# yell/boltzmann-machines

Measured on AMD Instinct MI355X. Metric: Gibbs-steps/sec (CD-k, 784x1024 RBM, batch 512), higher is better.
Workload: dtype f32

## Files before the change

boltzmann_machines_amd/csrc/bm_kernels.h:

```cpp
#pragma once
#include <stdio.h>
#include <stdlib.h>
#include <string.h>
#include <type_traits>
#include "bm_gemm.h"
#include "bm_bf3.h"
#include "bm_numerics.h"
#include "bm_rng.h"

namespace bm {

struct MfCtl { unsigned maxdiff; int done; int steps; float resid; };

struct ActArgs {
    Operand P1, Q1; int K1;
    int p_xm;
    Operand P2, Q2; int K2;
    int I, J;
    const float *bias;
    const float *sigma;
    float mult;
    float bmult;
    int kind;
    int sample;
    int lit;
    float *means;
    float *states;
    float *negmeans;
    int ldo;
    PhiloxKey key;
    long long row0;
    const float *prev;
    unsigned *maxdiff;
    float *maxdiff_blk;
    float *rowacc;
    float beta_a, beta_b;
    int rowacc_single;
    float *rowdot_out;
    int ld_part;
    const float *dot_vec;
    const float *dot_mat;
    int ld_dot;
    const float *acc_init;
    int ld_init;
    const int *skip;
    MfCtl *chk_ctl;
    const float *chk_slots; int chk_n; float chk_tol;
    Bf3Range b3;
    uint16_t *states16; int ld16;
    int geo_hint;
    int map_xi;
    float *fe_rowacc2;
    PhiloxKey fe_key;
    double *fe_zero;
    int fe_rm;
    const int *fe_flip;
    const float *fe_x; int fe_ldx;
    const float *fe_w; int fe_ldw;
    const float *clamp_val, *clamp_mask;
    int ld_clamp;
    const float *row_mult;
    float *rowen_out;
    float *sel_out;
    int sel_ld, sel_R, sel_rows;
    float *cr_part;
    const float *cr_U;
    int cr_ldu, cr_C, cr_nslots;
    const int *cb_y;
    const float *cb_U;
    int cb_ldu, cb_C;
    int *cb_bad;
    int bp;
    const float *bp_act;
    int bp_ld;
    int nrelu;
    int sm_k;
#ifdef BM_PROBE
    long long *dbg;
#endif
};
#ifdef BM_PROBE
#define BM_STAMP(n) do { if (a.dbg && threadIdx.x == 0) a.dbg[blockIdx.x * 4 + (n)] = (long long)__builtin_readcyclecounter(); } while (0)
#else
#define BM_STAMP(n) do {} while (0)
#endif

__device__ __forceinline__ int pll_flip_col(const PhiloxKey &key, unsigned long long idx, int V) {
    uint32_t w[4];
    philox_block(key, idx >> 2, w);
    return (int)(w[idx & 3] % (uint32_t)V);
}
#define FE_FLIP_FROM_KEY (reinterpret_cast<const int *>(uintptr_t(1)))
constexpr int BM_MF_SLOTS = 1024;

__device__ __forceinline__ void draw4(const ActArgs &a, const PhiloxKey &key, unsigned long long flat, int ib, int nvalid,
                                      const float *m, float *s, bool aligned) {
    if (aligned) {
        uint32_t wds[4];
        philox_block(key, flat >> 2, wds);
        if (a.kind == 0) {
#pragma unroll
            for (int r = 0; r < 4; ++r) s[r] = (u32_to_uniform(wds[r]) < m[r]) ? 1.f : 0.f;
        } else {
            float n[4];
            box_muller(wds[0], wds[1], n[0], n[1]);
            box_muller(wds[2], wds[3], n[2], n[3]);
#pragma unroll
            for (int r = 0; r < 4; ++r) s[r] = n[r] * a.sigma[ib + r] + m[r];
        }
    } else {
#pragma unroll
        for (int r = 0; r < 4; ++r) {
            if (r >= nvalid) break;
            const unsigned long long idx = flat + r;
            uint32_t wds[4];
            philox_block(key, idx >> 2, wds);
            if (a.kind == 0) {
                s[r] = (u32_to_uniform(wds[idx & 3]) < m[r]) ? 1.f : 0.f;
            } else {
                float n0, n1;
                const int pr = (int)(idx & 3) >> 1;
                box_muller(wds[2 * pr], wds[2 * pr + 1], n0, n1);
                s[r] = ((idx & 1) ? n1 : n0) * a.sigma[ib + r] + m[r];
            }
        }
    }
}

__device__ __forceinline__ float nrelu_state(float t, float n) {
    const float sd = sqrtf(sigmoid(t));
    const float u = __fadd_rn(t, __fmul_rn(n, sd));
    return (u > 0.0f) ? u : 0.0f;
}
__device__ __forceinline__ void nrelu_normals(const PhiloxKey &key, unsigned long long flat, int nvalid, float *n) {
#pragma unroll
    for (int r = 0; r < 4; ++r) {
        n[r] = 0.f;
        if (r >= nvalid) continue;
        const unsigned long long idx = flat + r;
        uint32_t wds[4];
        philox_block(key, idx >> 2, wds);
        float n0, n1;
        const int pr = (int)(idx & 3) >> 1;
        box_muller(wds[2 * pr], wds[2 * pr + 1], n0, n1);
        n[r] = (idx & 1) ? n1 : n0;
    }
}

#ifndef BM_NT_STORES
#define BM_NT_STORES 1
#endif
typedef float f32x2 __attribute__((ext_vector_type(2)));
__device__ __forceinline__ void stream_store4(float *p, float x, float y, float z, float w) {
    if (BM_NT_STORES) __builtin_nontemporal_store((f32x4){x, y, z, w}, reinterpret_cast<f32x4 *>(p));
    else *reinterpret_cast<float4 *>(p) = make_float4(x, y, z, w);
}
__device__ __forceinline__ void stream_store2(float *p, float x, float y) {
    if (BM_NT_STORES) __builtin_nontemporal_store((f32x2){x, y}, reinterpret_cast<f32x2 *>(p));
    else *reinterpret_cast<float2 *>(p) = make_float2(x, y);
}

template <bool CACHED = false>
__device__ __forceinline__ void store4(float *dst, size_t o, const float *v, int nvalid, bool v4) {
    if (v4) {
        if (CACHED) *reinterpret_cast<float4 *>(dst + o) = make_float4(v[0], v[1], v[2], v[3]);
        else stream_store4(dst + o, v[0], v[1], v[2], v[3]);
    } else {
#pragma unroll
        for (int r = 0; r < 4; ++r) if (r < nvalid) dst[o + r] = v[r];
    }
}

template <int MI> struct PhiloxFor { typedef PhiloxPair type; };
template <> struct PhiloxFor<1> { typedef PhiloxOne type; };

__device__ __forceinline__ float wave_max_lane63(float v) {
#define BM_DPP_MAX(ctrl, rmask) v = fmaxf(v, __int_as_float(__builtin_amdgcn_update_dpp(__float_as_int(v), __float_as_int(v), ctrl, rmask, 0xf, false)))
    BM_DPP_MAX(0xb1, 0xf);
    BM_DPP_MAX(0x4e, 0xf);
    BM_DPP_MAX(0x124, 0xf);
    BM_DPP_MAX(0x128, 0xf);
    BM_DPP_MAX(0x142, 0xa);
    BM_DPP_MAX(0x143, 0xc);
#undef BM_DPP_MAX
    return v;
}

template <int E, class Rng, bool MF = false, int NTH = 256> struct ActSide {
    static constexpr bool kFinalSync = false;
    static constexpr bool kSplitFill = false, kCohQ = false, kCanAbort = MF;
    static constexpr bool kMF = MF;
    const float *bias, *sigma;
    const float *prev_row;
    int ib0, I, with_rng;
    float bs[E], sg[E], pv[E];
    Rng rng;
    MfCtl *chk_ctl; const float *chk_slots; int chk_n; float chk_tol; const int *skip; float *s_chk; int aborted, nthreads;

    __device__ __forceinline__ void load_inputs() {
        const float *sp = sigma ? sigma : bias;
        const bool has_sigma = sigma != nullptr;
        if (MF && prev_row) {
            if (E == 4 && ib0 + 3 < I && (((uintptr_t)prev_row & 15u) == 0)) {
                const float4 t = *reinterpret_cast<const float4 *>(prev_row);
                pv[0] = t.x; pv[1] = t.y; pv[2] = t.z; pv[E - 1] = t.w;
            } else {
#pragma unroll
                for (int e = 0; e < E; ++e) pv[e] = (ib0 + e < I) ? prev_row[e] : 0.f;
            }
        }
        if (MF && E == 4 && ib0 + 3 < I && (((uintptr_t)(bias + ib0) & 15u) == 0) && (((uintptr_t)(sp + ib0) & 15u) == 0)) {
            const float4 b = *reinterpret_cast<const float4 *>(bias + ib0), v = *reinterpret_cast<const float4 *>(sp + ib0);
            bs[0] = b.x; bs[1] = b.y; bs[2] = b.z; bs[E - 1] = b.w;
            sg[0] = has_sigma ? v.x : 1.0f; sg[1] = has_sigma ? v.y : 1.0f; sg[2] = has_sigma ? v.z : 1.0f; sg[E - 1] = has_sigma ? v.w : 1.0f;
            return;
        }
#pragma unroll
        for (int e = 0; e < E; ++e) {
            const int i = (ib0 + e < I) ? ib0 + e : I - 1;
            bs[e] = bias[i];
            const float sv = sp[i];
            sg[e] = has_sigma ? sv : 1.0f;
        }
    }
    static constexpr int CHK_MAX = 4096;
    float *s_slots;
    static __device__ __forceinline__ void dma4_lane0(const void *src, float *lds_dst) {
        if ((threadIdx.x & 63) == 0) {
            unsigned keep;
            const unsigned lds_addr = (unsigned)(uintptr_t)(__attribute__((address_space(3))) void *)lds_dst;
            asm volatile("s_mov_b32 %0, m0\n\ts_mov_b32 m0, %2\n\ts_nop 0\n\tglobal_load_lds_dword %1, off\n\ts_mov_b32 m0, %0"
                         : "=&s"(keep) : "v"(src), "s"(__builtin_amdgcn_readfirstlane(lds_addr)) : "memory");
        }
    }
    __device__ __forceinline__ void preload() {
        if constexpr (MF) {
            load_inputs();
            aborted = 0;
            const int w = threadIdx.x >> 6, lane = threadIdx.x & 63;
            if (chk_ctl) {
                for (int p = w; p * 256 < chk_n && p * 256 < CHK_MAX; p += nthreads / 64)
                    dma16(reinterpret_cast<const char *>(chk_slots + 256 * p) + 16 * lane, s_slots + 256 * p);
                if (w == 0) dma4_lane0(&chk_ctl->done, s_slots + CHK_MAX);
            } else if (skip) {
                if (w == 0) dma4_lane0(skip, s_slots + CHK_MAX);
            }
        }
    }
    __device__ __forceinline__ void fill() {
        if (!MF) load_inputs();
        if (with_rng) rng.fill();
    }
    __device__ __forceinline__ void post_fill() {
        if constexpr (MF) {
            if (chk_ctl) {
                constexpr int NR = CHK_MAX / (4 * NTH);
                f32x4 v[NR];
#pragma unroll
                for (int q = 0; q < NR; ++q) {
                    const int e = 4 * ((int)threadIdx.x + q * NTH);
                    v[q] = *reinterpret_cast<const f32x4 *>(s_slots + (e < chk_n ? e : 0));
                }
                float m = 0.f;
#pragma unroll
                for (int q = 0; q < NR; ++q) {
                    const bool in = 4 * ((int)threadIdx.x + q * NTH) < chk_n;
                    m = fmaxf(m, in ? fmaxf(fmaxf(v[q][0], v[q][1]), fmaxf(v[q][2], v[q][3])) : 0.f);
                }
                m = wave_max_lane63(m);
                if ((threadIdx.x & 63) == 63) s_chk[threadIdx.x >> 6] = m;
                wg_barrier();
                m = 0.f;
#pragma unroll
                for (int q = 0; q < NTH / 64; ++q) m = fmaxf(m, s_chk[q]);
                const int was = __float_as_int(s_slots[CHK_MAX]);
                const int done = was || !(m > chk_tol);
                if (blockIdx.x == 0 && threadIdx.x == 0 && !was) { chk_ctl->steps += 1; chk_ctl->done = done; }
                aborted = __builtin_amdgcn_readfirstlane(done);
            } else if (skip) {
                aborted = __builtin_amdgcn_readfirstlane(__float_as_int(s_slots[CHK_MAX]) != 0);
            }
        }
    }
    __device__ __forceinline__ void drain() {}
};

template <class G, int ABL, class SideT, bool HWMATH = false, bool FE = false, bool LIT = false, bool CL = false, bool RT = false,
          bool CR = false, bool CB = false, bool BP = false, bool NR = false, bool SM = false>
__device__ __forceinline__ float act_epilogue(const ActArgs &a, const PhiloxKey &key, const f32x4 (&acc)[G::MI][1], const SideT &side,
                                              int i0, int j0) {
    constexpr int E = G::E, NH = G::MI;
    const int tid = threadIdx.x, lane = tid & 63, w = tid >> 6;
    const int wi = w % G::WI, wj = w / G::WI;
    const int g = lane >> 4, l15 = lane & 15;
    const int ib0 = i0 + wi * (16 * G::MI) + g * E;
    const int j = j0 + wj * 16 + l15;
    const bool rng_fast = ((a.I & 3) == 0);
    const float (&bs)[E] = side.bs;
    const float (&sg)[E] = side.sg;
    const typename PhiloxFor<G::MI>::type &rng = side.rng;

    float cv[NH][4], cm[NH][4];
    (void)cv; (void)cm;
    if constexpr (CL) {
        const bool al_cl = ((a.ld_clamp & 3) == 0) && (((uintptr_t)a.clamp_val & 15u) == 0) && (((uintptr_t)a.clamp_mask & 15u) == 0);
#pragma unroll
        for (int hlf = 0; hlf < NH; ++hlf) {
            const int ib = ib0 + 4 * hlf;
#pragma unroll
            for (int r = 0; r < 4; ++r) { cv[hlf][r] = 0.f; cm[hlf][r] = 0.f; }
            if (j < a.J && ib < a.I) {
                const size_t oc = (size_t)j * a.ld_clamp + ib;
                if (al_cl && ib + 3 < a.I) {
                    const float4 tv = *reinterpret_cast<const float4 *>(a.clamp_val + oc), tm = *reinterpret_cast<const float4 *>(a.clamp_mask + oc);
                    cv[hlf][0] = tv.x; cv[hlf][1] = tv.y; cv[hlf][2] = tv.z; cv[hlf][3] = tv.w;
                    cm[hlf][0] = tm.x; cm[hlf][1] = tm.y; cm[hlf][2] = tm.z; cm[hlf][3] = tm.w;
                } else {
#pragma unroll
                    for (int r = 0; r < 4; ++r)
                        if (ib + r < a.I) { cv[hlf][r] = a.clamp_val[oc + r]; cm[hlf][r] = a.clamp_mask[oc + r]; }
                }
            }
        }
    }
    float rm = 1.f, sv[E];
    (void)rm; (void)sv;
    if constexpr (RT) {
        rm = (j < a.J) ? a.row_mult[j] : 0.f;
#pragma unroll
        for (int e = 0; e < E; ++e) sv[e] = 0.f;
    }
    float cu[NH][4];
    bool cb_ok = false;
    (void)cu; (void)cb_ok;
    if constexpr (CB) {
        const int yj = (j < a.J) ? a.cb_y[j] : -1;
        cb_ok = (unsigned)yj < (unsigned)a.cb_C;
        if (j < a.J && !cb_ok && ib0 == 0) *a.cb_bad = 1;
        const bool al_cb = ((a.cb_ldu & 3) == 0) && (((uintptr_t)a.cb_U & 15u) == 0);
#pragma unroll
        for (int hlf = 0; hlf < NH; ++hlf) {
            const int ib = ib0 + 4 * hlf;
#pragma unroll
            for (int r = 0; r < 4; ++r) cu[hlf][r] = 0.f;
            if (cb_ok && ib < a.I) {
                const float *u = a.cb_U + (size_t)yj * a.cb_ldu + ib;
                if (al_cb && ib + 3 < a.I && (ib & 3) == 0) {
                    const float4 tu = *reinterpret_cast<const float4 *>(u);
                    cu[hlf][0] = tu.x; cu[hlf][1] = tu.y; cu[hlf][2] = tu.z; cu[hlf][3] = tu.w;
                } else {
#pragma unroll
                    for (int r = 0; r < 4; ++r)
                        if (ib + r < a.I) cu[hlf][r] = u[r];
                }
            }
        }
    }
    float ba[NH][4];
    (void)ba;
    if constexpr (BP) {
        const bool al_bp = ((a.bp_ld & 3) == 0) && (((uintptr_t)a.bp_act & 15u) == 0);
#pragma unroll
        for (int hlf = 0; hlf < NH; ++hlf) {
            const int ib = ib0 + 4 * hlf;
#pragma unroll
            for (int r = 0; r < 4; ++r) ba[hlf][r] = 0.f;
            if (a.bp_act && j < a.J && ib < a.I) {
                const float *p = a.bp_act + (size_t)j * a.bp_ld + ib;
                if (al_bp && ib + 3 < a.I) {
                    const float4 t = *reinterpret_cast<const float4 *>(p);
                    ba[hlf][0] = t.x; ba[hlf][1] = t.y; ba[hlf][2] = t.z; ba[hlf][3] = t.w;
                } else {
#pragma unroll
                    for (int r = 0; r < 4; ++r)
                        if (ib + r < a.I) ba[hlf][r] = p[r];
                }
            }
        }
    }
    float z[E];
    lane_outputs<G>(acc, 0, z);
    float dmax = 0.f;
    if (BM_ABL(4)) {
        float zs = 0.f;
#pragma unroll
        for (int e = 0; e < E; ++e) zs += z[e];
        if (j < a.J && ib0 < a.I && a.states) a.states[(size_t)j * a.ldo + ib0] = zs;
    } else if (j < a.J && ib0 < a.I) {
        const bool al_out = ((a.ldo & 3) == 0);
#pragma unroll
        for (int hlf = 0; hlf < NH; ++hlf) {
            const int ib = ib0 + 4 * hlf;
            if (ib >= a.I) break;
            const int nvalid = (a.I - ib < 4) ? a.I - ib : 4;
            float m[4], s[4], nt[4];
            (void)nt;
#pragma unroll
            for (int r = 0; r < 4; ++r) {
                if constexpr (BP) {
                    const float zv = z[4 * hlf + r], av = ba[hlf][r];
                    m[r] = a.bp_act ? __fmul_rn(__fmul_rn(zv, av), __fsub_rn(1.0f, av)) : zv;
                    s[r] = m[r];
                    continue;
                }
                const float x = (RT ? rm : a.mult) * z[4 * hlf + r];
                float bv = bs[4 * hlf + r];
                if constexpr (CB) { if (cb_ok) bv = __fadd_rn(bv, cu[hlf][r]); }
                const float b = (RT ? rm : a.bmult) * bv;
                if constexpr (NR) {
                    nt[r] = x + b;
                    m[r] = (nt[r] > 0.0f) ? nt[r] : 0.0f;
                    s[r] = m[r];
                    continue;
                }
                if constexpr (SM) {
                    nt[r] = x + b;
                    continue;
                }
                m[r] = (a.kind == 0) ? (LIT ? sigmoid_literal(x + b) : (HWMATH ? sigmoid_hw(x + b) : sigmoid(x + b)))
                                     : (a.kind == 1 ? (x * sg[4 * hlf + r] + b) : (a.kind == 3 ? x + b : x));
                s[r] = m[r];
            }
            if constexpr (SM) {
                static_assert(G::MI == 1, "the SM flavour exists for the geometries with one quad per lane");
                const int Ks = a.sm_k, nl = (Ks >= 8) ? (Ks >> 2) : 1, pos = g & (nl - 1);
                float mxa = fmaxf(nt[0], nt[1]), mxb = fmaxf(nt[2], nt[3]);
                if (Ks > 2) {
                    mxa = fmaxf(mxa, mxb);
                    if (Ks >= 8) mxa = fmaxf(mxa, __shfl_xor(mxa, 16));
                    if (Ks == 16) mxa = fmaxf(mxa, __shfl_xor(mxa, 32));
                    mxb = mxa;
                }
                float ev[4], cc[4], cpv[4];
#pragma unroll
                for (int r = 0; r < 4; ++r) {
                    float d = ((r < 2) ? mxa : mxb) - nt[r];
                    if (d > 80.0f) d = 80.0f;
                    ev[r] = exp_neg(d);
                }
                float start = 0.0f;
                for (int step = 0; step < nl; ++step) {
                    if (step > 0) {
                        const float recv = __shfl(cc[3], (lane + 48) & 63);
                        if (pos == step) start = recv;
                    }
                    cpv[0] = start;          cc[0] = start + ev[0];
                    cpv[1] = cc[0];          cc[1] = cc[0] + ev[1];
                    cpv[2] = (Ks == 2) ? 0.0f : cc[1];
                    cc[2] = cpv[2] + ev[2];
                    cpv[3] = cc[2];          cc[3] = cc[2] + ev[3];
                }
                float Sa = cc[3], Sb = cc[3];
                if (Ks == 2) Sa = cc[1];
                if (Ks >= 8) { Sa = __shfl(cc[3], l15 + 16 * (g | (nl - 1))); Sb = Sa; }
#pragma unroll
                for (int r = 0; r < 4; ++r) { m[r] = ev[r] / ((r < 2) ? Sa : Sb); s[r] = m[r]; }
                if (a.sample) {
                    const uint32_t *wds = rng.words(hlf);
                    float ua = u32_to_uniform(wds[0]), ub = (Ks == 2) ? u32_to_uniform(wds[2]) : ua;
                    if (Ks >= 8) { ua = __shfl(ua, l15 + 16 * (g & ~(nl - 1))); ub = ua; }
                    const float ta = ua * Sa, tb = ub * Sb;
#pragma unroll
                    for (int r = 0; r < 4; ++r) {
                        const float t = (r < 2) ? ta : tb;
                        s[r] = (cc[r] > t && !(cpv[r] > t)) ? 1.f : 0.f;
                    }
                }
            }
            if (!BP && !SM && a.sample) {
                if constexpr (NR) {
                    float n[4];
                    if (rng_fast) {
                        const uint32_t *wds = rng.words(hlf);
                        box_muller(wds[0], wds[1], n[0], n[1]);
                        box_muller(wds[2], wds[3], n[2], n[3]);
                    } else {
                        nrelu_normals(key, (unsigned long long)(a.row0 + j) * (unsigned long long)a.I + ib, nvalid, n);
                    }
#pragma unroll
                    for (int r = 0; r < 4; ++r) s[r] = nrelu_state(nt[r], n[r]);
                } else if (rng_fast) {
                    const uint32_t *wds = rng.words(hlf);
                    if (a.kind == 0) {
#pragma unroll
                        for (int r = 0; r < 4; ++r) s[r] = (u32_to_uniform(wds[r]) < m[r]) ? 1.f : 0.f;
                    } else {
                        float n[4];
                        box_muller(wds[0], wds[1], n[0], n[1]);
                        box_muller(wds[2], wds[3], n[2], n[3]);
#pragma unroll
                        for (int r = 0; r < 4; ++r) s[r] = n[r] * sg[4 * hlf + r] + m[r];
                    }
                } else {
                    const unsigned long long flat = (unsigned long long)(a.row0 + j) * (unsigned long long)a.I + ib;
                    draw4(a, key, flat, ib, nvalid, m, s, false);
                }
            }
            if constexpr (CL) {
#pragma unroll
                for (int r = 0; r < 4; ++r)
                    if (cm[hlf][r] != 0.f) { m[r] = cv[hlf][r]; s[r] = cv[hlf][r]; }
            }
            if constexpr (RT) {
#pragma unroll
                for (int r = 0; r < 4; ++r) sv[4 * hlf + r] = s[r];
            }
            const size_t o = (size_t)j * a.ldo + ib;
            if constexpr (SideT::kMF) {
                if (a.prev) {
#pragma unroll
                    for (int r = 0; r < 4; ++r)
                        if (r < nvalid) dmax = fmaxf(dmax, fabsf(m[r] - side.pv[4 * hlf + r]));
                }
            }
            const bool v4 = al_out && nvalid == 4;
            if (a.means) store4<HWMATH>(a.means, o, m, nvalid, v4 && (((uintptr_t)a.means & 15u) == 0));
            if (a.negmeans) {
                float nm[4];
#pragma unroll
                for (int r = 0; r < 4; ++r) nm[r] = -m[r];
                store4<HWMATH>(a.negmeans, o, nm, nvalid, v4 && (((uintptr_t)a.negmeans & 15u) == 0));
            }
            if (a.states) store4<HWMATH>(a.states, o, s, nvalid, v4 && (((uintptr_t)a.states & 15u) == 0));
            if constexpr (RT) {
                if (a.sel_out && rm == 1.0f) {
                    const int c = j / a.sel_R;
                    if (c < a.sel_rows)
                        store4<HWMATH>(a.sel_out, (size_t)c * a.sel_ld + ib, s, nvalid,
                                       nvalid == 4 && ((a.sel_ld & 3) == 0) && (((uintptr_t)a.sel_out & 15u) == 0));
                }
            }
            if (HWMATH && a.states16) {
                uint16_t *d = a.states16 + (size_t)j * a.ld16 + ib;
                if (nvalid == 4 && (ib & 3) == 0) {
                    uint2 pk;
                    pk.x = (__float_as_uint(s[0]) >> 16) | (__float_as_uint(s[1]) & 0xffff0000u);
                    pk.y = (__float_as_uint(s[2]) >> 16) | (__float_as_uint(s[3]) & 0xffff0000u);
                    *reinterpret_cast<uint2 *>(d) = pk;
                } else {
#pragma unroll
                    for (int r = 0; r < 4; ++r) if (r < nvalid) d[r] = (uint16_t)(__float_as_uint(s[r]) >> 16);
                }
            }
        }
    }
    if constexpr (FE) { if (a.fe_zero && i0 == 0 && j0 == 0 && tid < 6) a.fe_zero[tid] = 0.0; }
    bool row_sums = a.rowacc || a.rowdot_out;
    if constexpr (RT) row_sums = row_sums || a.rowen_out;
    if constexpr (BP) row_sums = false;
    if (row_sums) {
        float racc = 0.f, rdot = 0.f, racc2 = 0.f, ren = 0.f;
        (void)ren;
        if (j < a.J) {
            int fc = 0; float delta = 0.f;
            if constexpr (FE) {
                fc = (a.fe_flip == FE_FLIP_FROM_KEY) ? pll_flip_col(a.fe_key, (unsigned long long)(a.row0 + j), a.K1) : a.fe_flip[j];
                delta = 1.0f - 2.0f * a.fe_x[(size_t)j * a.fe_ldx + fc];
            }
#pragma unroll
            for (int hlf = 0; hlf < NH; ++hlf) {
                float qa = 0.f, qd = 0.f, qa2 = 0.f, qe = 0.f;
                (void)qe;
#pragma unroll
                for (int r = 0; r < 4; ++r) {
                    const int e = 4 * hlf + r, i = ib0 + e;
                    if (i >= a.I) break;
                    if (a.rowacc) {
                        if (a.dot_mat) {
                            qa += z[e] * a.dot_mat[(size_t)j * a.ld_dot + i];
                        } else {
                            const float t = z[e] + bs[e];
                            if constexpr (FE) qa2 += softplus(t + delta * a.fe_w[(size_t)fc * a.fe_ldw + i]);
                            if (a.rowacc_single) qa += HWMATH ? softplus_hw(a.beta_b * t) : softplus(a.beta_b * t);
                            else qa += softplus_hw(a.beta_b * t) - softplus_hw(a.beta_a * t);
                        }
                    }
                    if (a.rowdot_out) qd += a.states[(size_t)j * a.ldo + i] * a.dot_vec[i];
                    if constexpr (RT) { if (a.rowen_out) qe += sv[e] * (z[e] + bs[e]); }
                }
                if constexpr (RT) ren = (hlf == 0) ? qe : ren + qe;
                racc = (hlf == 0) ? qa : racc + qa;
                rdot = (hlf == 0) ? qd : rdot + qd;
                racc2 = (hlf == 0) ? qa2 : racc2 + qa2;
            }
        }
        racc += __shfl_xor(racc, 16);
        rdot += __shfl_xor(rdot, 16);
        if (G::MI == 1) { racc += __shfl_xor(racc, 32); rdot += __shfl_xor(rdot, 32); }
        if constexpr (FE) { racc2 += __shfl_xor(racc2, 16); if (G::MI == 1) racc2 += __shfl_xor(racc2, 32); }
        if constexpr (RT) { ren += __shfl_xor(ren, 16); if (G::MI == 1) ren += __shfl_xor(ren, 32); }
        const bool writer = (G::MI == 1) ? (g == 0) : ((g & 1) == 0);
        const int slot = (i0 + wi * (16 * G::MI)) / 16 + ((G::MI == 2) ? (g >> 1) : 0);
        if (writer && j < a.J && slot * 16 < a.I) {
            if constexpr (FE) {
                a.rowacc[(size_t)j * a.fe_rm + slot] = racc;
                a.fe_rowacc2[(size_t)j * a.fe_rm + slot] = racc2;
            } else {
                if (a.rowacc) a.rowacc[(size_t)slot * a.ld_part + j] = racc;
                if (a.rowdot_out) a.rowdot_out[(size_t)slot * a.ld_part + j] = rdot;
                if constexpr (RT) { if (a.rowen_out) a.rowen_out[(size_t)slot * a.ld_part + j] = ren; }
            }
        }
    }
    if constexpr (CR) {
        const bool writer = (G::MI == 1) ? (g == 0) : ((g & 1) == 0);
        const int slot = (i0 + wi * (16 * G::MI)) / 16 + ((G::MI == 2) ? (g >> 1) : 0);
        for (int c = 0; c < a.cr_C; ++c) {
            const float *u = a.cr_U + (size_t)c * a.cr_ldu;
            float racc = 0.f;
            if (j < a.J) {
#pragma unroll
                for (int hlf = 0; hlf < NH; ++hlf) {
                    float qa = 0.f;
#pragma unroll
                    for (int r = 0; r < 4; ++r) {
                        const int e = 4 * hlf + r, i = ib0 + e;
                        if (i >= a.I) break;
                        qa += softplus((z[e] + bs[e]) + u[i]);
                    }
                    racc = (hlf == 0) ? qa : racc + qa;
                }
            }
            racc += __shfl_xor(racc, 16);
            if (G::MI == 1) racc += __shfl_xor(racc, 32);
            if (writer && j < a.J && slot * 16 < a.I) a.cr_part[((size_t)c * a.cr_nslots + slot) * a.ld_part + j] = racc;
        }
    }
    return dmax;
}

template <class G, int MINB, bool SEG2, bool FAST, int ABL = 0, int PL = KM, int STG = STG_DMA, bool FE = false, bool LIT = false, bool MF = false,
          bool CL = false, bool RT = false, bool CR = false, bool CB = false, bool BP = false, bool NR = false, bool SM = false>
BM_KERNEL __launch_bounds__(G::NT, MINB) void act_kernel(ActArgs a, TileMap tmap) {
    __shared__ __attribute__((aligned(16))) float smem[G::SMEM_FLOATS];
    constexpr int E = G::E;
    BM_STAMP(0);
    asm volatile("" :: "s"(a.P1.ptr), "s"(a.Q1.ptr), "s"(a.P1.ld), "s"(a.Q1.ld), "s"(a.P1.nx), "s"(a.Q1.nx),
                       "s"(a.K1), "s"(a.K2), "s"(a.bias), "s"(a.sigma), "s"(a.means), "s"(a.states), "s"(a.ldo),
                       "s"(a.sample), "s"(a.kind), "s"(a.row0), "s"(a.I), "s"(a.J), "s"(a.skip));
    const int tiles_j = (a.J + G::TJ - 1) / G::TJ;
    int ti, tj;
    if (tmap.slab) {
        block_to_tile(tiles_j, ti, tj, 0, 0, a.J > 2 * a.I, (a.I + G::TI - 1) / G::TI);
    } else {
        TILE_WORDS(tmap, (int)blockIdx.x);
        TILE_OF_BLOCK(tmap, (int)blockIdx.x, (int)gridDim.x, ti, tj);
    }
    const int i0 = ti * G::TI, j0 = tj * G::TJ;
    const int tid = threadIdx.x, lane = tid & 63, w = tid >> 6;
    const int wi = w % G::WI, wj = w / G::WI;
    const int g = lane >> 4, l15 = lane & 15;
    const int ib0 = i0 + wi * (16 * G::MI) + g * E;

    KRange kr;
    kr.P1 = a.P1; kr.Q1 = a.Q1; kr.K1 = a.K1;
    kr.P2 = a.P2; kr.Q2 = a.Q2; kr.K2 = a.K2;
    static_assert(G::NJ == 1, "act_kernel: one j sub-tile per wave");
    const int j = j0 + wj * 16 + l15;
    ActSide<E, typename PhiloxFor<G::MI>::type, MF, G::NT> side;
    side.bias = a.bias; side.sigma = a.sigma; side.ib0 = ib0; side.I = a.I; side.with_rng = a.sample;
    side.prev_row = (MF && a.prev && j < a.J && ib0 < a.I) ? a.prev + (size_t)j * a.ldo + ib0 : nullptr;
    const PhiloxKey key = a.key;
    side.rng.init(key, ((unsigned long long)(a.row0 + j) * (unsigned long long)a.I + ib0) >> 2);

    f32x4 acc[G::MI][1];
#pragma unroll
    for (int t = 0; t < G::MI; ++t) acc[t][0] = (f32x4){0.f, 0.f, 0.f, 0.f};
    if constexpr (MF) {
        __shared__ float s_chk[G::NT / 64];
        __shared__ __attribute__((aligned(16))) float s_slots[ActSide<E, typename PhiloxFor<G::MI>::type, true>::CHK_MAX + 4];
        side.s_slots = s_slots;
        side.chk_ctl = a.chk_ctl; side.chk_slots = a.chk_slots; side.chk_n = a.chk_n; side.chk_tol = a.chk_tol;
        side.skip = a.skip; side.s_chk = s_chk; side.nthreads = G::NT; side.aborted = 0;
        if (a.acc_init && j < a.J) {
            const float *src = a.acc_init + (size_t)j * a.ld_init + ib0;
            if (G::MI == 1 && ib0 + 3 < a.I && (((uintptr_t)src & 15u) == 0)) {
                const float4 t4 = *reinterpret_cast<const float4 *>(src);
                acc[0][0] = (f32x4){t4.x, t4.y, t4.z, t4.w};
            } else {
#pragma unroll
                for (int r = 0; r < 4; ++r)
#pragma unroll
                    for (int t = 0; t < G::MI; ++t) {
                        const int i = ib0 + G::MI * r + t;
                        if (i < a.I) acc[t][0][r] = src[G::MI * r + t];
                    }
            }
        }
        side.preload();
    }
#ifdef BM_PROBE
    mainloop<XM, G, FAST, SEG2, ABL, PL, STG>(acc, kr, i0, j0, smem, side, a.dbg ? a.dbg + 2048 + blockIdx.x * 8 : nullptr);
#else
    mainloop<XM, G, FAST, SEG2, ABL, PL, STG>(acc, kr, i0, j0, smem, side);
#endif
    BM_STAMP(1);
    if constexpr (MF) { if (side.aborted) return; }
    float dmax = act_epilogue<G, ABL, decltype(side), false, FE, LIT, CL, RT, CR, CB, BP, NR, SM>(a, key, acc, side, i0, j0);
    if (MF && a.maxdiff) {
        __shared__ float s_wavemax[G::NT / 64];
        dmax = wave_max_lane63(dmax);
        if (lane == 63) s_wavemax[w] = dmax;
        wg_barrier();
        if (tid == 0) {
            float m = 0.f;
#pragma unroll
            for (int q = 0; q < G::NT / 64; ++q) m = fmaxf(m, s_wavemax[q]);
            if (a.maxdiff_blk && gridDim.x <= BM_MF_SLOTS) a.maxdiff_blk[blockIdx.x] = m;
            else if (m > 0.f) atomicMax(a.maxdiff, __float_as_uint(m));
        }
    }
    BM_STAMP(2);
}

struct Bf3Strip { int tiles_i, tiles_j, strips, abl; };

template <class G, bool SEG2, int MINW>
BM_KERNEL __launch_bounds__(G::NT, MINW) void act_bf3_kernel(ActArgs a, Bf3Strip sp) {
    __shared__ __attribute__((aligned(16))) float smem[Bf3Geo<G>::SMEM_FLOATS];
    constexpr int E = G::E;
    const int ti = (int)blockIdx.x / sp.strips, st = (int)blockIdx.x % sp.strips;
    const int per = sp.tiles_j / sp.strips, rem = sp.tiles_j % sp.strips;
    const int tj0 = st * per + (st < rem ? st : rem), tj1 = tj0 + per + (st < rem ? 1 : 0);
    const int i0 = ti * G::TI;
    const int tid = threadIdx.x, lane = tid & 63, w = tid >> 6;
    const int wi = w % G::WI, wj = w / G::WI;
    const int g = lane >> 4, l15 = lane & 15;
    const int ib0 = i0 + wi * (16 * G::MI) + g * E;
    ActSide<E, typename PhiloxFor<G::MI>::type> side;
    side.bias = a.bias; side.sigma = a.sigma; side.ib0 = ib0; side.I = a.I; side.with_rng = 0;
    side.prev_row = nullptr;
    side.fill();
    side.with_rng = a.sample;
    Bf3Pipe<G, SEG2> pipe;
    pipe.setup(a.b3, i0, smem);
    if (tj0 < tj1) { pipe.set_tile(a.b3, tj0 * G::TJ); pipe.prefetch(); }
    for (int tj = tj0; tj < tj1; ++tj) {
        const int j0 = tj * G::TJ, j = j0 + wj * 16 + l15;
        f32x4 acc[G::MI][1];
#pragma unroll
        for (int t = 0; t < G::MI; ++t) acc[t][0] = (f32x4){0.f, 0.f, 0.f, 0.f};
        side.rng.init(a.key, ((unsigned long long)(a.row0 + j) * (unsigned long long)a.I + ib0) >> 2);
        if (a.sample) side.rng.fill();
        if (!(sp.abl & 2)) pipe.run(acc);
        if (tj + 1 < tj1) { pipe.set_tile(a.b3, (tj + 1) * G::TJ); pipe.prefetch(); }
        if (!(sp.abl & 1)) (void)act_epilogue<G, 0, decltype(side), true>(a, a.key, acc, side, i0, j0);
    }
}

struct ColSumJob {
    const float *A, *Bm;
    int lda, ldb, ncols, nrows;
    float *out;
};
constexpr int MAX_COLJOBS = 12;
struct ColSumArgs {
    ColSumJob job[MAX_COLJOBS];
    int first_wave[MAX_COLJOBS + 1];
    int njobs;
};

constexpr int CS_ROWS = 128;
constexpr int CS_LD = 80;
constexpr int CS_SMEM_FLOATS = 2 * CS_ROWS * CS_LD;

constexpr int CS_NV = CS_ROWS * 16 / NT;
struct ColRegs { float4 a[CS_NV], b[CS_NV]; };

__device__ __forceinline__ void cs_fetch(ColRegs &r, const float *A, int lda, const float *Bm, int ldb,
                                         int c0, int ncols, int nrows, int r0, int tid) {
    const int c4 = tid & 15;
    const int cc = min(c0 + 4 * c4, ncols - 4);
#pragma unroll
    for (int n = 0; n < CS_NV; ++n) {
        const int rc = min(r0 + (tid >> 4) + 16 * n, nrows - 1);
        r.a[n] = *reinterpret_cast<const float4 *>(A + (size_t)rc * lda + cc);
        r.b[n] = Bm ? *reinterpret_cast<const float4 *>(Bm + (size_t)rc * ldb + cc) : make_float4(0.f, 0.f, 0.f, 0.f);
    }
}

__device__ __forceinline__ void cs_stash(const ColRegs &r, float *sA, float *sB, int c0, int ncols, int nrows,
                                         int r0, int tid) {
    const int c4 = tid & 15;
#pragma unroll
    for (int n = 0; n < CS_NV; ++n) {
        const int row = (tid >> 4) + 16 * n;
        const bool ok = (r0 + row < nrows) && (c0 + 4 * c4 < ncols);
        float4 va = r.a[n], vb = r.b[n];
        if (!ok) { va = make_float4(0.f, 0.f, 0.f, 0.f); vb = va; }
        *reinterpret_cast<float4 *>(sA + row * CS_LD + 4 * c4) = va;
        *reinterpret_cast<float4 *>(sB + row * CS_LD + 4 * c4) = vb;
    }
}

__device__ __forceinline__ void block_colsum(const float *A, int lda, const float *Bm, int ldb,
                                             int c0, int ncols, int nrows, bool want2,
                                             float *smem, f32x4 &sum1, f32x4 &sum2, bool negB = false) {
    const int tid = threadIdx.x, lane = tid & 63, w = tid >> 6;
    const int g = lane >> 4, l15 = lane & 15;
    float *sA = smem, *sB = smem + CS_ROWS * CS_LD;
    sum1 = (f32x4){0.f, 0.f, 0.f, 0.f};
    sum2 = (f32x4){0.f, 0.f, 0.f, 0.f};
    const bool vec = (((uintptr_t)A & 15u) == 0) && ((lda & 3) == 0) && ((ncols & 3) == 0) &&
                     (!Bm || ((((uintptr_t)Bm & 15u) == 0) && ((ldb & 3) == 0)));
    ColRegs regs;
    if (vec) cs_fetch(regs, A, lda, Bm, ldb, c0, ncols, nrows, 0, tid);
    for (int r0 = 0; r0 < nrows; r0 += CS_ROWS) {
        const int nr = (nrows - r0 < CS_ROWS) ? nrows - r0 : CS_ROWS;
        if (vec) {
            cs_stash(regs, sA, sB, c0, ncols, nrows, r0, tid);
        } else {
            for (int e = tid; e < CS_ROWS * 64; e += NT) {
                const int row = e >> 6, cc = e & 63, c = c0 + cc;
                const bool ok = row < nr && c < ncols;
                sA[row * CS_LD + cc] = ok ? A[(size_t)(r0 + row) * lda + c] : 0.f;
                sB[row * CS_LD + cc] = (ok && Bm) ? Bm[(size_t)(r0 + row) * ldb + c] : 0.f;
            }
        }
        wg_barrier();
        if (vec) cs_fetch(regs, A, lda, Bm, ldb, c0, ncols, nrows, r0 + CS_ROWS, tid);
        const int nsteps = (((nr + 3) / 4) + 7) & ~7;
        const int co = w * 16 + l15;
        for (int s = 0; s < nsteps; s += 8) {
            float d[8], e[8];
#pragma unroll
            for (int u = 0; u < 8; ++u) {
                const int o = (4 * (s + u) + g) * CS_LD + co;
                e[u] = sB[o];
                d[u] = negB ? sA[o] + e[u] : sA[o] - e[u];
            }
#pragma unroll
            for (int u = 0; u < 8; ++u) {
                sum1 = __builtin_amdgcn_mfma_f32_16x16x4f32(d[u], 1.0f, sum1, 0, 0, 0);
                if (want2) sum2 = __builtin_amdgcn_mfma_f32_16x16x4f32(e[u], 1.0f, sum2, 0, 0, 0);
            }
        }
        wg_barrier();
    }
    if (negB) sum2 = -sum2;
}

BM_KERNEL __launch_bounds__(NT) void colsum_kernel(ColSumArgs a) {
    __shared__ __attribute__((aligned(16))) float smem[CS_SMEM_FLOATS];
    const int wv = blockIdx.x, lane = threadIdx.x & 63, w = threadIdx.x >> 6;
    int jb = 0;
    while (jb + 1 < a.njobs && wv >= a.first_wave[jb + 1]) ++jb;
    const ColSumJob J = a.job[jb];
    const int c0 = (wv - a.first_wave[jb]) * 64;
    f32x4 s1, s2;
    block_colsum(J.A, J.lda, J.Bm, J.ldb, c0, J.ncols, J.nrows, false, smem, s1, s2);
    if ((lane & 15) == 0) {
        const int g = lane >> 4;
#pragma unroll
        for (int r = 0; r < 4; ++r) {
            const int cc = c0 + w * 16 + g * 4 + r;
            if (cc < J.ncols) J.out[cc] = s1[r];
        }
    }
}

struct RbmBiasArgs {
    const float *sv, *sh, *sq;
    float *vb, *dvb, *hb, *dhb, *q, *pen;
    int V, H;
    float N, lr, mom, damping, cost, target;
};
BM_KERNEL void rbm_bias_kernel(RbmBiasArgs a) {
    const int c = blockIdx.x * blockDim.x + threadIdx.x;
    if (c < a.V) {
        const float g = a.sv[c] / a.N;
        const float d = a.lr * (a.mom * a.dvb[c] + g);
        a.dvb[c] = d;
        a.vb[c] = a.vb[c] + d;
    } else if (c < a.V + a.H) {
        const int h = c - a.V;
        const float qn = a.damping * a.q[h] + (1.0f - a.damping) * a.sq[h];
        a.q[h] = qn;
        const float pen = a.cost * (qn - a.target);
        a.pen[h] = pen;
        float g = a.sh[h] / a.N;
        g = g - pen;
        const float d = a.lr * (a.mom * a.dhb[h] + g);
        a.dhb[h] = d;
        a.hb[h] = a.hb[h] + d;
    }
}

struct RbmBiasFusedArgs {
    const float *X, *vs, *h0m, *hm;
    int ldx, ldv, ldh0, ldh, B;
    int hm_negated;
    float *raw_tail;
    int raw_only;
    RbmBiasArgs u;
};
__device__ __forceinline__ void rbm_bias_fused_block(const RbmBiasFusedArgs &a, int wv, float *smem) {
    const int lane = threadIdx.x & 63, w = threadIdx.x >> 6, g = lane >> 4;
    const int nv = (a.u.V + 63) / 64;
    f32x4 s1, s2;
    if (wv < nv) {
        const int c0 = wv * 64;
        block_colsum(a.X, a.ldx, a.vs, a.ldv, c0, a.u.V, a.B, false, smem, s1, s2);
        if ((lane & 15) == 0) {
#pragma unroll
            for (int r = 0; r < 4; ++r) {
                const int c = c0 + w * 16 + g * 4 + r;
                if (c < a.u.V) {
                    a.raw_tail[c] = s1[r];
                    if (a.raw_only) continue;
                    const float gr = s1[r] / a.u.N;
                    const float d = a.u.lr * (a.u.mom * a.u.dvb[c] + gr);
                    a.u.dvb[c] = d;
                    a.u.vb[c] = a.u.vb[c] + d;
                }
            }
        }
    } else {
        const int c0 = (wv - nv) * 64;
        block_colsum(a.h0m, a.ldh0, a.hm, a.ldh, c0, a.u.H, a.B, true, smem, s1, s2, a.hm_negated != 0);
        if ((lane & 15) == 0) {
#pragma unroll
            for (int r = 0; r < 4; ++r) {
                const int h = c0 + w * 16 + g * 4 + r;
                if (h < a.u.H) {
                    const float sq = s2[r];
                    a.raw_tail[a.u.V + h] = s1[r];
                    a.raw_tail[a.u.V + a.u.H + h] = sq;
                    if (a.raw_only) continue;
                    const float qn = a.u.damping * a.u.q[h] + (1.0f - a.u.damping) * sq;
                    a.u.q[h] = qn;
                    const float pen = a.u.cost * (qn - a.u.target);
                    a.u.pen[h] = pen;
                    float gr = s1[r] / a.u.N;
                    gr = gr - pen;
                    const float d = a.u.lr * (a.u.mom * a.u.dhb[h] + gr);
                    a.u.dhb[h] = d;
                    a.u.hb[h] = a.u.hb[h] + d;
                }
            }
        }
    }
}

BM_KERNEL __launch_bounds__(NT) void rbm_bias_fused_kernel(RbmBiasFusedArgs a) {
    __shared__ __attribute__((aligned(16))) float smem[CS_SMEM_FLOATS];
    rbm_bias_fused_block(a, blockIdx.x, smem);
}

struct GradArgs {
    Operand Ppos, Qpos; int Kpos;
    Operand Pneg, Qneg; int Kneg;
    int I, J;
    int form;
    int fused;
    float *raw;
    float *raw2;
    float *W, *dW;
    float *Wt;
    int ldw, ldwt;
    const float *pen;
    float N, M, l2, lr, mom;
    int nbias;
    RbmBiasFusedArgs bias;
    int fetch_at_fill;
    int map_xi;
#ifdef BM_PROBE
    long long *dbg;
#endif
};

__device__ __forceinline__ void apply_w_update(float g, float pen, float l2, float lr, float mom,
                                               float &w, float &dw) {
    g = __fsub_rn(g, __fmul_rn(l2, w));
    g = __fsub_rn(g, pen);
    const float d = __fmul_rn(lr, __fadd_rn(__fmul_rn(mom, dw), g));
    dw = d;
    w = __fadd_rn(w, d);
}
__device__ __forceinline__ bool grad_pow2(float N) { return ((__float_as_uint(N) & 0x007fffffu) == 0u) && N >= 1.0f; }
__device__ __forceinline__ float grad_norm1(float r, float N, float invN, bool pow2) {
    return pow2 ? __fmul_rn(r, invN) : __fdiv_rn(r, N);
}
__device__ __forceinline__ float grad_norm2(float r, float r2, float N, float M, float invN, float invM, bool pow2) {
    return pow2 ? __fsub_rn(__fmul_rn(r, invN), __fmul_rn(r2, invM)) : __fsub_rn(__fdiv_rn(r, N), __fdiv_rn(r2, M));
}

struct DivBy {
    float n, inv; bool pow2;
    __device__ __forceinline__ explicit DivBy(float N) : n(N), inv(1.0f / N),
        pow2(grad_pow2(N)) {}
};

template <int NJ> struct GradSide {
    static constexpr bool kFinalSync = true;
    static constexpr bool kSplitFill = false, kCohQ = false, kCanAbort = false;
    const float *W, *dW; int ldw, I, J, ib0, jb[NJ]; bool on, vec8;
    float4 w[NJ][2], d[NJ][2];
    bool at_fill;
    __device__ __forceinline__ void fill() { if (at_fill) fetch(); }
    __device__ __forceinline__ void drain() { if (!at_fill) fetch(); }
    __device__ __forceinline__ void fetch() {
        if (!on || ib0 >= I) return;
#pragma unroll
        for (int n = 0; n < NJ; ++n) {
            if (jb[n] >= J) continue;
            const size_t o = (size_t)jb[n] * ldw + ib0;
            if (vec8) {
                w[n][0] = *reinterpret_cast<const float4 *>(W + o);  w[n][1] = *reinterpret_cast<const float4 *>(W + o + 4);
                d[n][0] = *reinterpret_cast<const float4 *>(dW + o); d[n][1] = *reinterpret_cast<const float4 *>(dW + o + 4);
            } else {
                float tw[8], td[8];
#pragma unroll
                for (int e = 0; e < 8; ++e) {
                    const bool ok = ib0 + e < I;
                    tw[e] = ok ? W[o + e] : 0.f;
                    td[e] = ok ? dW[o + e] : 0.f;
                }
                w[n][0] = make_float4(tw[0], tw[1], tw[2], tw[3]); w[n][1] = make_float4(tw[4], tw[5], tw[6], tw[7]);
                d[n][0] = make_float4(td[0], td[1], td[2], td[3]); d[n][1] = make_float4(td[4], td[5], td[6], td[7]);
            }
        }
    }
};

struct GradCen { const float *oj, *gj, *oi, *gi; };
__device__ __forceinline__ const GradCen &grad_cen_of(const GradCen &c) { return c; }
struct GradFast { float *Wf, *We, *Wet; int ldf, ldet; float fast_lr, fast_decay; };
__device__ __forceinline__ const GradFast &grad_fast_of(const GradFast &f) { return f; }
template <class T, class... P> struct grad_has { static constexpr int value = 0; };
template <class T, class P0, class... P> struct grad_has<T, P0, P...> { static constexpr int value = (std::is_same<T, P0>::value ? 1 : 0) + grad_has<T, P...>::value; };
template <class G, bool FAST, int ABL = 0, int STG = STG_DMA, int MINB = 1, class... CENP>
BM_KERNEL __launch_bounds__(G::NT, MINB) void grad_kernel(GradArgs a, TileMap tmap, CENP... cenp) {
    constexpr int CEN = grad_has<GradCen, CENP...>::value, FW = grad_has<GradFast, CENP...>::value;
    static_assert(sizeof...(CENP) <= 1 && CEN + FW == (int)sizeof...(CENP), "grad_kernel: at most one GradCen or one GradFast");
    constexpr int TI = G::TI, NJ = G::NJ;
    static_assert(G::MI == 2 && G::TI == 64 && G::TJ == 64, "grad_kernel: 64 x 64 tiles, 8 consecutive outputs per lane");
    __shared__ __attribute__((aligned(16))) float smem[G::SMEM_FLOATS];
    constexpr bool kBias = G::SMEM_FLOATS >= CS_SMEM_FLOATS;
    static_assert(G::NT >= NT, "bias path");
    const int ntile_blocks = (int)gridDim.x - a.nbias;
    if ((int)blockIdx.x >= ntile_blocks) {
        if constexpr (kBias) {
            if (G::NT > NT && threadIdx.x >= NT) return;
            rbm_bias_fused_block(a.bias, (int)blockIdx.x - ntile_blocks, smem);
        }
        return;
    }
    asm volatile("" :: "s"(a.Ppos.ptr), "s"(a.Qpos.ptr), "s"(a.Ppos.ld), "s"(a.Qpos.ld), "s"(a.Ppos.nx), "s"(a.Qpos.nx),
                       "s"(a.Pneg.ptr), "s"(a.Qneg.ptr), "s"(a.Pneg.ld), "s"(a.Qneg.ld), "s"(a.Kpos), "s"(a.Kneg),
                       "s"(a.I), "s"(a.J), "s"(a.W), "s"(a.dW), "s"(a.ldw), "s"(a.form), "s"(a.fused));
    constexpr int TJ2 = G::TJ;
    int ti, tj;
    if (tmap.slab) {
        block_to_tile((a.J + TJ2 - 1) / TJ2, ti, tj, 0, a.nbias);
    } else {
        TILE_WORDS(tmap, (int)blockIdx.x);
        TILE_OF_BLOCK(tmap, (int)blockIdx.x, ntile_blocks, ti, tj);
    }
    const int i0 = ti * TI, j0 = tj * TJ2;
    const int tid = threadIdx.x, lane = tid & 63, w = tid >> 6;
    const int wi = w % G::WI, wj = w / G::WI;
    const int g = lane >> 4, l15 = lane & 15;
    const int ib0 = i0 + wi * 32 + g * 8;

#ifdef BM_PROBE
#define BM_GSTAMP(n) do { if (a.dbg && threadIdx.x == 0) a.dbg[blockIdx.x * 4 + (n)] = (long long)__builtin_readcyclecounter(); } while (0)
#else
#define BM_GSTAMP(n) do {} while (0)
#endif
    BM_GSTAMP(0);
    f32x4 pos[2][NJ], neg[2][NJ];
#pragma unroll
    for (int t = 0; t < 2; ++t)
#pragma unroll
        for (int n = 0; n < NJ; ++n) pos[t][n] = neg[t][n] = (f32x4){0.f, 0.f, 0.f, 0.f};
    GradSide<NJ> side;
    side.W = a.W; side.dW = a.dW; side.ldw = a.ldw; side.I = a.I; side.J = a.J; side.ib0 = ib0;
#pragma unroll
    for (int n = 0; n < NJ; ++n) side.jb[n] = j0 + wj * (16 * NJ) + lane_j<KM, G>(l15, n);
    side.vec8 = (ib0 + 7 < a.I) && ((a.ldw & 3) == 0);
    side.at_fill = true;
    side.on = a.fused != 0 && a.fetch_at_fill != 0;
    KRange kr;
    kr.P1 = a.Ppos; kr.Q1 = a.Qpos; kr.K1 = a.Kpos;
    if (a.form == 0) {
        kr.P2 = a.Pneg; kr.Q2 = a.Qneg; kr.K2 = a.Kneg;
        mainloop<KM, G, FAST, true, ABL, KM, STG>(pos, kr, i0, j0, smem, side);
    } else {
        kr.P2 = a.Ppos; kr.Q2 = a.Qpos; kr.K2 = 0;
        mainloop<KM, G, FAST, false, 0, KM, STG>(pos, kr, i0, j0, smem, side);
        kr.P1 = a.Pneg; kr.Q1 = a.Qneg; kr.K1 = a.Kneg;
        mainloop<KM, G, FAST, false, 0, KM, STG>(neg, kr, i0, j0, smem, side);
    }

    BM_GSTAMP(1);
    if (ib0 >= a.I) return;
    if (!a.fetch_at_fill) { side.on = a.fused != 0; side.fetch(); }
    const DivBy divN(a.N), divM(a.M);
    float wt[NJ][8];
    float et[FW ? NJ : 1][FW ? 8 : 1];
    bool jok[NJ];
    float coi[CEN ? 8 : 1], cgi[CEN ? 8 : 1];
    if constexpr (CEN != 0) {
#pragma unroll
        for (int e = 0; e < 8; ++e) {
            const bool ok = ib0 + e < a.I;
            coi[e] = ok ? grad_cen_of(cenp...).oi[ib0 + e] : 0.f;
            cgi[e] = ok ? grad_cen_of(cenp...).gi[ib0 + e] : 0.f;
        }
    }
#pragma unroll
    for (int n = 0; n < NJ; ++n) {
        const int j = side.jb[n];
        jok[n] = j < a.J;
        if (!jok[n]) continue;
        float pv[8], nv[8];
        lane_outputs<G>(pos, n, pv);
        lane_outputs<G>(neg, n, nv);
        const size_t o = (size_t)j * a.ldw + ib0;
        if (!a.fused) {
#pragma unroll
            for (int e = 0; e < 8; ++e) {
                if (ib0 + e >= a.I) break;
                a.raw[o + e] = pv[e];
                if (a.form != 0) a.raw2[o + e] = nv[e];
            }
            continue;
        }
        float wv[8] = {side.w[n][0].x, side.w[n][0].y, side.w[n][0].z, side.w[n][0].w, side.w[n][1].x, side.w[n][1].y, side.w[n][1].z, side.w[n][1].w};
        float dv[8] = {side.d[n][0].x, side.d[n][0].y, side.d[n][0].z, side.d[n][0].w, side.d[n][1].x, side.d[n][1].y, side.d[n][1].z, side.d[n][1].w};
        float pe[8];
#pragma unroll
        for (int e = 0; e < 8; ++e) pe[e] = (a.pen && ib0 + e < a.I) ? a.pen[ib0 + e] : 0.f;
        float gr[8];
        if (divN.pow2 && divM.pow2) {
#pragma unroll
            for (int e = 0; e < 8; ++e) gr[e] = (a.form == 0) ? grad_norm1(pv[e], a.N, divN.inv, true)
                                                              : grad_norm2(pv[e], nv[e], a.N, a.M, divN.inv, divM.inv, true);
        } else {
#pragma unroll
            for (int e = 0; e < 8; ++e) gr[e] = (a.form == 0) ? grad_norm1(pv[e], a.N, 0.f, false)
                                                              : grad_norm2(pv[e], nv[e], a.N, a.M, 0.f, 0.f, false);
        }
        if constexpr (CEN != 0) {
            const float oj = grad_cen_of(cenp...).oj[j], gj = grad_cen_of(cenp...).gj[j];
#pragma unroll
            for (int e = 0; e < 8; ++e) gr[e] = __fsub_rn(gr[e], __fadd_rn(__fmul_rn(oj, cgi[e]), __fmul_rn(gj, coi[e])));
        }
        float fv[FW ? 8 : 1];
        if constexpr (FW != 0) {
            const GradFast &f = grad_fast_of(cenp...);
            const size_t of = (size_t)j * f.ldf + ib0;
            if (side.vec8 && (f.ldf & 3) == 0) {
                const float4 f0 = *reinterpret_cast<const float4 *>(f.Wf + of), f1 = *reinterpret_cast<const float4 *>(f.Wf + of + 4);
                fv[0] = f0.x; fv[1] = f0.y; fv[2] = f0.z; fv[3] = f0.w; fv[4] = f1.x; fv[5] = f1.y; fv[6] = f1.z; fv[7] = f1.w;
            } else {
#pragma unroll
                for (int e = 0; e < 8; ++e) fv[e] = (ib0 + e < a.I) ? f.Wf[of + e] : 0.f;
            }
#pragma unroll
            for (int e = 0; e < 8; ++e) fv[e] = __fadd_rn(__fmul_rn(f.fast_decay, fv[e]), __fmul_rn(f.fast_lr, gr[e]));
        }
#pragma unroll
        for (int e = 0; e < 8; ++e) {
            apply_w_update(gr[e], pe[e], a.l2, a.lr, a.mom, wv[e], dv[e]);
            wt[n][e] = wv[e];
        }
        if (side.vec8) {
            stream_store4(a.W + o, wv[0], wv[1], wv[2], wv[3]);
            stream_store4(a.W + o + 4, wv[4], wv[5], wv[6], wv[7]);
            stream_store4(a.dW + o, dv[0], dv[1], dv[2], dv[3]);
            stream_store4(a.dW + o + 4, dv[4], dv[5], dv[6], dv[7]);
        } else {
#pragma unroll
            for (int e = 0; e < 8; ++e)
                if (ib0 + e < a.I) { a.W[o + e] = wv[e]; a.dW[o + e] = dv[e]; }
        }
        if constexpr (FW != 0) {
            const GradFast &f = grad_fast_of(cenp...);
            const size_t of = (size_t)j * f.ldf + ib0;
#pragma unroll
            for (int e = 0; e < 8; ++e) et[n][e] = __fadd_rn(wv[e], fv[e]);
            if (side.vec8 && (f.ldf & 3) == 0) {
                stream_store4(f.Wf + of, fv[0], fv[1], fv[2], fv[3]);
                stream_store4(f.Wf + of + 4, fv[4], fv[5], fv[6], fv[7]);
                stream_store4(f.We + of, et[n][0], et[n][1], et[n][2], et[n][3]);
                stream_store4(f.We + of + 4, et[n][4], et[n][5], et[n][6], et[n][7]);
            } else {
#pragma unroll
                for (int e = 0; e < 8; ++e)
                    if (ib0 + e < a.I) { f.Wf[of + e] = fv[e]; f.We[of + e] = et[n][e]; }
            }
        }
    }
    if constexpr (FW != 0) {
        const GradFast &f = grad_fast_of(cenp...);
        if (a.fused && f.Wet) {
            const int ja = side.jb[0];
            const bool pair = NJ == 2 && jok[0] && jok[NJ - 1] && ((f.ldet & 1) == 0);
#pragma unroll
            for (int e = 0; e < 8; ++e) {
                if (ib0 + e >= a.I) break;
                float *dst = f.Wet + (size_t)(ib0 + e) * f.ldet + ja;
                if (pair) {
                    stream_store2(dst, et[0][e], et[NJ - 1][e]);
                } else {
                    if (jok[0]) dst[0] = et[0][e];
                    if (NJ == 2 && jok[NJ - 1]) dst[1] = et[NJ - 1][e];
                }
            }
        }
    }
    if (a.fused && a.Wt) {
        const int ja = side.jb[0];
        const bool pair = NJ == 2 && jok[0] && jok[NJ - 1] && ((a.ldwt & 1) == 0);
#pragma unroll
        for (int e = 0; e < 8; ++e) {
            if (ib0 + e >= a.I) break;
            float *dst = a.Wt + (size_t)(ib0 + e) * a.ldwt + ja;
            if (pair) {
                stream_store2(dst, wt[0][e], wt[NJ - 1][e]);
            } else {
                if (jok[0]) dst[0] = wt[0][e];
                if (NJ == 2 && jok[NJ - 1]) dst[1] = wt[NJ - 1][e];
            }
        }
    }
    BM_GSTAMP(2);
}

struct ApplyWArgs {
    const float *raw, *raw2;
    float *W, *dW, *Wt;
    const float *pen;
    int I, J, ldw, ldwt;
    int form;
    float N, M, l2, lr, mom;
};
BM_KERNEL void apply_w_kernel(ApplyWArgs a) {
    const size_t n = (size_t)a.I * a.J;
    for (size_t e = (size_t)blockIdx.x * blockDim.x + threadIdx.x; e < n; e += (size_t)gridDim.x * blockDim.x) {
        const int i = (int)(e % (size_t)a.I), j = (int)(e / (size_t)a.I);
        const size_t o = (size_t)j * a.ldw + i;
        const float gr = (a.form == 0) ? grad_norm1(a.raw[o], a.N, 0.f, false) : grad_norm2(a.raw[o], a.raw2[o], a.N, a.M, 0.f, 0.f, false);
        float wv = a.W[o], dv = a.dW[o];
        apply_w_update(gr, a.pen ? a.pen[i] : 0.f, a.l2, a.lr, a.mom, wv, dv);
        a.W[o] = wv;
        a.dW[o] = dv;
        if (a.Wt) a.Wt[(size_t)i * a.ldwt + j] = wv;
    }
}

__device__ __forceinline__ void rbm_bias_apply(const RbmBiasArgs &a, bool hidden, int c, float g) {
    if (!hidden) {
        const float d = a.lr * (a.mom * a.dvb[c] + g);
        a.dvb[c] = d;
        a.vb[c] = a.vb[c] + d;
    } else {
        const float qn = a.damping * a.q[c] + (1.0f - a.damping) * a.sq[c];
        a.q[c] = qn;
        const float pen = a.cost * (qn - a.target);
        a.pen[c] = pen;
        g = g - pen;
        const float d = a.lr * (a.mom * a.dhb[c] + g);
        a.dhb[c] = d;
        a.hb[c] = a.hb[c] + d;
    }
}
__device__ __forceinline__ void rbm_bias_update(const RbmBiasArgs &a, int c) {
    if (c < a.V) rbm_bias_apply(a, false, c, a.sv[c] / a.N);
    else if (c < a.V + a.H) rbm_bias_apply(a, true, c - a.V, a.sh[c - a.V] / a.N);
}
BM_KERNEL __launch_bounds__(256) void apply_w_tiled_kernel(ApplyWArgs a, RbmBiasArgs b, int nbias) {
    __shared__ float tile[64][65];
    const int ntile = (int)gridDim.x - nbias;
    if ((int)blockIdx.x >= ntile) {
        rbm_bias_update(b, ((int)blockIdx.x - ntile) * 256 + (int)threadIdx.x);
        return;
    }
    const int tiles_i = (a.I + 63) / 64;
    const int i0 = ((int)blockIdx.x % tiles_i) * 64, j0 = ((int)blockIdx.x / tiles_i) * 64;
    const int tid = threadIdx.x, c4 = tid & 15, r0 = tid >> 4;
    const bool pow2 = grad_pow2(a.N) && grad_pow2(a.M);
    const float invN = 1.0f / a.N, invM = 1.0f / a.M;
    const int i = i0 + 4 * c4;
    float4 pe = make_float4(0.f, 0.f, 0.f, 0.f);
    if (a.pen && i < a.I) pe = *reinterpret_cast<const float4 *>(a.pen + i);
#pragma unroll
    for (int p = 0; p < 4; ++p) {
        const int jl = r0 + 16 * p, j = j0 + jl;
        if (j < a.J && i < a.I) {
            const size_t o = (size_t)j * a.ldw + i;
            const float4 r = *reinterpret_cast<const float4 *>(a.raw + o);
            float4 wv = *reinterpret_cast<const float4 *>(a.W + o), dv = *reinterpret_cast<const float4 *>(a.dW + o);
            float4 g;
            if (a.form == 0) {
                g = make_float4(grad_norm1(r.x, a.N, invN, pow2), grad_norm1(r.y, a.N, invN, pow2),
                                grad_norm1(r.z, a.N, invN, pow2), grad_norm1(r.w, a.N, invN, pow2));
            } else {
                const float4 r2 = *reinterpret_cast<const float4 *>(a.raw2 + o);
                g = make_float4(grad_norm2(r.x, r2.x, a.N, a.M, invN, invM, pow2), grad_norm2(r.y, r2.y, a.N, a.M, invN, invM, pow2),
                                grad_norm2(r.z, r2.z, a.N, a.M, invN, invM, pow2), grad_norm2(r.w, r2.w, a.N, a.M, invN, invM, pow2));
            }
            apply_w_update(g.x, pe.x, a.l2, a.lr, a.mom, wv.x, dv.x);
            apply_w_update(g.y, pe.y, a.l2, a.lr, a.mom, wv.y, dv.y);
            apply_w_update(g.z, pe.z, a.l2, a.lr, a.mom, wv.z, dv.z);
            apply_w_update(g.w, pe.w, a.l2, a.lr, a.mom, wv.w, dv.w);
            *reinterpret_cast<float4 *>(a.W + o) = wv;
            *reinterpret_cast<float4 *>(a.dW + o) = dv;
            tile[jl][4 * c4] = wv.x; tile[jl][4 * c4 + 1] = wv.y; tile[jl][4 * c4 + 2] = wv.z; tile[jl][4 * c4 + 3] = wv.w;
        }
    }
    if (!a.Wt) return;
    __syncthreads();
    const int jq = j0 + 4 * c4;
#pragma unroll
    for (int p = 0; p < 4; ++p) {
        const int il = r0 + 16 * p, ii = i0 + il;
        if (ii >= a.I || jq >= a.J) continue;
        float *dst = a.Wt + (size_t)ii * a.ldwt + jq;
        if (jq + 3 < a.J) {
            *reinterpret_cast<float4 *>(dst) = make_float4(tile[4 * c4][il], tile[4 * c4 + 1][il], tile[4 * c4 + 2][il], tile[4 * c4 + 3][il]);
        } else {
            for (int e = 0; e < 4; ++e) if (jq + e < a.J) dst[e] = tile[4 * c4 + e][il];
        }
    }
}
struct SmArgs {
    float *L; int ld, I, J, M, sample;
    float *states, *negmeans;
    int ld_states;
    PhiloxKey key; long long row0;
    const float *prev; int ld_prev; unsigned *maxdiff;
    const int *skip;
};
BM_KERNEL __launch_bounds__(64) void softmax_multinomial_kernel(SmArgs a) {
    extern __shared__ float sm_dyn[];
    float *c = sm_dyn, *e = sm_dyn + a.I;
    const int row = blockIdx.x, lane = threadIdx.x;
    if (a.skip && *a.skip) return;
    float *l = a.L + (size_t)row * a.ld;
    const int lds = a.ld_states ? a.ld_states : a.ld;
    float mx = -3.402823466e38f;
    for (int i = lane; i < a.I; i += 64) mx = fmaxf(mx, l[i]);
#pragma unroll
    for (int off = 32; off > 0; off >>= 1) mx = fmaxf(mx, __shfl_xor(mx, off));
    for (int i = lane; i < a.I; i += 64) {
        float d = mx - l[i];
        if (d > 80.0f) d = 80.0f;
        e[i] = exp_neg(d);
    }
    __syncthreads();
    if (lane == 0) {
        float run = 0.0f;
        int i = 0;
        for (; i + 8 <= a.I; i += 8) {
            float t[8];
#pragma unroll
            for (int u = 0; u < 8; ++u) t[u] = e[i + u];
#pragma unroll
            for (int u = 0; u < 8; ++u) { run = run + t[u]; c[i + u] = run; }
        }
        for (; i < a.I; ++i) { run = run + e[i]; c[i] = run; }
    }
    __syncthreads();
    const float S = c[a.I - 1], Mf = (float)a.M;
    float dmax = 0.f;
    for (int i = lane; i < a.I; i += 64) {
        const float m = Mf * (e[i] / S);
        if (a.prev) dmax = fmaxf(dmax, fabsf(m - a.prev[(size_t)row * a.ld_prev + i]));
        l[i] = m;
        if (a.negmeans) a.negmeans[(size_t)row * lds + i] = -m;
        if (a.states && !a.sample) a.states[(size_t)row * lds + i] = m;
    }
    if (a.maxdiff) {
#pragma unroll
        for (int off = 32; off > 0; off >>= 1) dmax = fmaxf(dmax, __shfl_xor(dmax, off));
        if (lane == 0 && dmax > 0.f) atomicMax(a.maxdiff, __float_as_uint(dmax));
    }
    if (!a.states || !a.sample) return;
    __syncthreads();
    int *cnt = reinterpret_cast<int *>(e);
    for (int i = lane; i < a.I; i += 64) cnt[i] = 0;
    __syncthreads();
    for (int d = lane; d < a.M; d += 64) {
        const float u = philox_uniform_at(a.key, (unsigned long long)(a.row0 + row) * (unsigned long long)a.M + (unsigned long long)d);
        const float t = u * S;
        int lo = 0, hi = a.I - 1;
        while (lo < hi) {
            const int mid = (lo + hi) >> 1;
            if (c[mid] > t) hi = mid; else lo = mid + 1;
        }
        atomicAdd(cnt + lo, 1);
    }
    __syncthreads();
    for (int i = lane; i < a.I; i += 64) a.states[(size_t)row * lds + i] = (float)cnt[i];
}

BM_KERNEL void mn_hhat_kernel(float *hhat, int K, int M, PhiloxKey k0, PhiloxKey k1, PhiloxKey k2) {
    const int d = blockIdx.x * blockDim.x + threadIdx.x;
    if (d >= M) return;
    const PhiloxKey keys[3] = {k0, k1, k2};
#pragma unroll
    for (int t = 0; t < 3; ++t) {
        int idx = (int)(philox_uniform_at(keys[t], (unsigned long long)d) * (float)K);
        if (idx > K - 1) idx = K - 1;
        atomicAdd(hhat + (size_t)t * K + idx, 1.0f);
    }
}

BM_KERNEL void dropout_kernel(const float *X, int ldx, float *Y, int ldy, int rows, int cols, float keep,
                               PhiloxKey key, unsigned long long flat0) {
    const size_t n = (size_t)rows * cols;
    for (size_t e = (size_t)blockIdx.x * blockDim.x + threadIdx.x; e < n; e += (size_t)gridDim.x * blockDim.x) {
        const size_t r = e / (size_t)cols, c = e % (size_t)cols;
        const float u = philox_uniform_at(key, flat0 + e);
        Y[r * ldy + c] = (X[r * ldx + c] / keep) * floorf(keep + u);
    }
}

BM_KERNEL void div_cols_kernel(const float *X, int ldx, const float *sigma, float *Y, int ldy, int rows, int cols) {
    const size_t n = (size_t)rows * cols;
    for (size_t e = (size_t)blockIdx.x * blockDim.x + threadIdx.x; e < n; e += (size_t)gridDim.x * blockDim.x) {
        const size_t r = e / (size_t)cols, c = e % (size_t)cols;
        Y[r * ldy + c] = X[r * ldx + c] / sigma[c];
    }
}

BM_KERNEL void copy2d_kernel(const float *X, int ldx, float *Y, int ldy, int rows, int cols) {
    const size_t n = (size_t)rows * cols;
    for (size_t e = (size_t)blockIdx.x * blockDim.x + threadIdx.x; e < n; e += (size_t)gridDim.x * blockDim.x) {
        const size_t r = e / (size_t)cols, c = e % (size_t)cols;
        Y[r * ldy + c] = X[r * ldx + c];
    }
}

BM_KERNEL void clamp_apply_kernel(float *X, int ldx, const float *val, const float *mask, int ldc, int rows, int cols) {
    const size_t n = (size_t)rows * cols;
    for (size_t e = (size_t)blockIdx.x * blockDim.x + threadIdx.x; e < n; e += (size_t)gridDim.x * blockDim.x) {
        const size_t r = e / (size_t)cols, c = e % (size_t)cols;
        if (mask[r * ldc + c] != 0.f) X[r * ldx + c] = val[r * ldc + c];
    }
}

BM_KERNEL __launch_bounds__(256) void transpose_kernel(const float *A, int lda, float *T, int ldt, int rows, int cols) {
    __shared__ float t[32][33];
    const int tiles_c = (cols + 31) / 32;
    const int r0 = ((int)blockIdx.x / tiles_c) * 32, c0 = ((int)blockIdx.x % tiles_c) * 32;
    const int tx = threadIdx.x & 31, ty = threadIdx.x >> 5;
    for (int r = ty; r < 32; r += 8)
        if (r0 + r < rows && c0 + tx < cols) t[r][tx] = A[(size_t)(r0 + r) * lda + c0 + tx];
    __syncthreads();
    for (int c = ty; c < 32; c += 8)
        if (c0 + c < cols && r0 + tx < rows) T[(size_t)(c0 + c) * ldt + r0 + tx] = t[tx][c];
}

__device__ __forceinline__ double wave_sum(double v) {
#pragma unroll
    for (int off = 32; off > 0; off >>= 1) v += __shfl_xor(v, off);
    return v;
}

BM_KERNEL void sqdiff_kernel(const float *A, int lda, const float *B, int ldb, int rows, int cols, double *out) {
    const size_t n = (size_t)rows * cols;
    double s = 0.0;
    for (size_t e = (size_t)blockIdx.x * blockDim.x + threadIdx.x; e < n; e += (size_t)gridDim.x * blockDim.x) {
        const size_t r = e / (size_t)cols, c = e % (size_t)cols;
        const float d = B ? (A[r * lda + c] - B[r * ldb + c]) : A[r * lda + c];
        s += (double)d * (double)d;
    }
    s = wave_sum(s);
    if ((threadIdx.x & 63) == 0) atomicAdd(out, s);
}

struct MetricsPrepArgs {
    double *scal; float *rowacc; int n_rowacc; int *flip; int B, V; PhiloxKey key; unsigned long long row0;
};
BM_KERNEL __launch_bounds__(256) void metrics_prep_kernel(MetricsPrepArgs a) {
    const int t = blockIdx.x * blockDim.x + threadIdx.x, nt = gridDim.x * blockDim.x;
    if (t < 6) a.scal[t] = 0.0;
    for (int e = t; e < a.n_rowacc; e += nt) a.rowacc[e] = 0.f;
    for (int b = t; b < a.B; b += nt) {
        a.flip[b] = pll_flip_col(a.key, a.row0 + b, a.V);
    }
}
struct SqJob { const float *A; int lda; const float *B; int ldb; int rows, cols; double *out; };
__device__ __forceinline__ void sqdiff2_body(const SqJob &j0, const SqJob &j1, int blk, int nblk) {
    const int half = nblk >> 1;
    const bool second = blk >= half;
    const SqJob &j = second ? j1 : j0;
    const int nb = second ? nblk - half : half, b = second ? blk - half : blk;
    const int lane = threadIdx.x & 63, wv = b * (blockDim.x >> 6) + (threadIdx.x >> 6), nwv = nb * (blockDim.x >> 6);
    double s = 0.0;
    const bool vec = (j.lda & 3) == 0 && (((uintptr_t)j.A) & 15u) == 0 && (!j.B || ((j.ldb & 3) == 0 && (((uintptr_t)j.B) & 15u) == 0));
    for (int r = wv; r < j.rows; r += nwv) {
        const float *pa = j.A + (size_t)r * j.lda, *pb = j.B ? j.B + (size_t)r * j.ldb : nullptr;
        int c = 0;
        if (vec) {
            const int c4n = j.cols >> 2;
            for (int g0 = 0; g0 < c4n; g0 += 256) {
                float4 x[4], y[4];
#pragma unroll
                for (int u = 0; u < 4; ++u) {
                    const int g = g0 + u * 64 + lane;
                    const int gc = g < c4n ? g : c4n - 1;
                    x[u] = *reinterpret_cast<const float4 *>(pa + 4 * gc);
                    y[u] = pb ? *reinterpret_cast<const float4 *>(pb + 4 * gc) : make_float4(0.f, 0.f, 0.f, 0.f);
                }
#pragma unroll
                for (int u = 0; u < 4; ++u) {
                    if (g0 + u * 64 + lane < c4n) {
                        const float d0 = x[u].x - y[u].x, d1 = x[u].y - y[u].y, d2 = x[u].z - y[u].z, d3 = x[u].w - y[u].w;
                        s += (double)d0 * (double)d0 + (double)d1 * (double)d1 + (double)d2 * (double)d2 + (double)d3 * (double)d3;
                    }
                }
            }
            c = 4 * c4n;
        }
        for (c += lane; c < j.cols; c += 64) {
            const float d = pb ? (pa[c] - pb[c]) : pa[c];
            s += (double)d * (double)d;
        }
    }
    __shared__ double s_part[4];
    s = wave_sum(s);
    if (lane == 0) s_part[threadIdx.x >> 6] = s;
    __syncthreads();
    if (threadIdx.x == 0 && j.rows > 0) atomicAdd(j.out, (s_part[0] + s_part[1]) + (s_part[2] + s_part[3]));
}
BM_KERNEL __launch_bounds__(256) void sqdiff2_kernel(SqJob j0, SqJob j1) { sqdiff2_body(j0, j1, (int)blockIdx.x, (int)gridDim.x); }
BM_KERNEL void scal_to_host_kernel(const double *scal, double *dst) {
    if (threadIdx.x < 6) dst[threadIdx.x] = scal[threadIdx.x];
}

struct FeArgs {
    Operand P, Q; int K;
    int I, J;
    const float *hb;
    float *rowacc;
    float *rowacc2;
    const int *flip_col;
    const float *hvec;
    float *rowacc3;
};
template <bool FAST>
BM_KERNEL __launch_bounds__(NT, 1) void fe_hidden_kernel(FeArgs a) {
    using G = GeoAct;
    constexpr int TI = G::TI, TJ = G::TJ;
    __shared__ __attribute__((aligned(16))) float smem[G::SMEM_FLOATS];
    const int tiles_j = (a.J + TJ - 1) / TJ;
    int ti, tj;
    block_to_tile(tiles_j, ti, tj);
    const int i0 = ti * TI, j0 = tj * TJ;
    f32x4 acc[2][1];
    acc[0][0] = acc[1][0] = (f32x4){0.f, 0.f, 0.f, 0.f};
    NoSide none;
    KRange kr;
    kr.P1 = a.P; kr.Q1 = a.Q; kr.K1 = a.K;
    kr.P2 = a.P; kr.Q2 = a.Q; kr.K2 = 0;
    mainloop<XM, G, FAST, false>(acc, kr, i0, j0, smem, none);
    const int tid = threadIdx.x, lane = tid & 63, w = tid >> 6;
    const int wi = w & 1, wj = w >> 1;
    const int g = lane >> 4, l15 = lane & 15;
    const int j = j0 + wj * 16 + l15;
    float s = 0.f, s2 = 0.f, s3 = 0.f;
    if (j < a.J) {
        float delta = 0.f; int fc = -1;
        if (a.flip_col) {
            fc = a.flip_col[j];
            delta = 1.0f - 2.0f * a.Q.ptr[(size_t)j * a.Q.ld + fc];
        }
        float zz[8];
        lane_outputs<G>(acc, 0, zz);
#pragma unroll
        for (int e = 0; e < 8; ++e) {
            const int i = i0 + wi * 32 + g * 8 + e;
            if (i < a.I) {
                if (a.hvec) {
                    s += zz[e] * a.hvec[i];
                    s3 += zz[e] * a.hvec[a.I + i];
                    if (fc >= 0) s2 += (zz[e] + delta * a.P.ptr[(size_t)fc * a.P.ld + i]) * a.hvec[2 * (size_t)a.I + i];
                } else {
                    const float z = zz[e] + a.hb[i];
                    s += softplus(z);
                    if (fc >= 0) s2 += softplus(z + delta * a.P.ptr[(size_t)fc * a.P.ld + i]);
                }
            }
        }
    }
    s += __shfl_xor(s, 16);  s += __shfl_xor(s, 32);
    s2 += __shfl_xor(s2, 16); s2 += __shfl_xor(s2, 32);
    s3 += __shfl_xor(s3, 16); s3 += __shfl_xor(s3, 32);
    if (g == 0 && j < a.J) {
        atomicAdd(a.rowacc + j, s);
        if (a.rowacc2) atomicAdd(a.rowacc2 + j, s2);
        if (a.rowacc3) atomicAdd(a.rowacc3 + j, s3);
    }
}

struct FeRowArgs {
    const float *X; int ld, V, B;
    const float *vb, *sigma;
    const float *rowacc, *rowacc2, *rowacc3;
    const int *flip_col;
    double *out;
    int nslot, ld_part;
    int has_key; PhiloxKey key; unsigned long long row0;
};
constexpr int FE_ROWS_PER_WG = 8;
__device__ __forceinline__ void fe_row_body(const FeRowArgs &a, int blk) {
    const int lane = threadIdx.x & 63, wv = threadIdx.x >> 6;
    double s0 = 0.0, s1 = 0.0, s2 = 0.0;
    for (int q = 0; q < FE_ROWS_PER_WG / 4; ++q) {
        const int row = blk * FE_ROWS_PER_WG + q * 4 + wv;
        if (row >= a.B) break;
        const float *x = a.X + (size_t)row * a.ld;
        const int fc = a.flip_col ? a.flip_col[row] : (a.has_key ? pll_flip_col(a.key, a.row0 + row, a.V) : -1);
        double t = 0.0, t2 = 0.0;
        int c = lane;
        if (!a.sigma && (a.ld & 3) == 0 && (((uintptr_t)a.X | (uintptr_t)a.vb) & 15u) == 0) {
            const int c4n = a.V >> 2;
            for (int g0 = 0; g0 < c4n; g0 += 256) {
                float4 xv[4], bv[4];
#pragma unroll
                for (int u = 0; u < 4; ++u) {
                    const int g = g0 + u * 64 + lane, gc = g < c4n ? g : c4n - 1;
                    xv[u] = *reinterpret_cast<const float4 *>(x + 4 * gc);
                    bv[u] = *reinterpret_cast<const float4 *>(a.vb + 4 * gc);
                }
#pragma unroll
                for (int u = 0; u < 4; ++u) {
                    const int g = g0 + u * 64 + lane;
                    if (g < c4n) {
                        const float xs[4] = {xv[u].x, xv[u].y, xv[u].z, xv[u].w}, bs4[4] = {bv[u].x, bv[u].y, bv[u].z, bv[u].w};
#pragma unroll
                        for (int r = 0; r < 4; ++r) {
                            const float xf = (4 * g + r == fc) ? 1.0f - xs[r] : xs[r];
                            t -= (double)(xs[r] * bs4[r]);
                            t2 -= (double)(xf * bs4[r]);
                        }
                    }
                }
            }
            c = 4 * c4n + lane;
        }
        for (; c < a.V; c += 64) {
            const float xv = x[c];
            const float xf = (c == fc) ? 1.0f - xv : xv;
            if (a.sigma) {
                const float mu = a.vb[c] / a.sigma[c];
                t += 0.5 * (double)((xv - mu) * (xv - mu));
                t2 += 0.5 * (double)((xf - mu) * (xf - mu));
            } else {
                t -= (double)(xv * a.vb[c]);
                t2 -= (double)(xf * a.vb[c]);
            }
        }
        t = wave_sum(t);
        t2 = wave_sum(t2);
        double h1 = 0.0, h2 = 0.0;
        if (a.nslot > 0) {
            for (int q = lane; q < a.nslot; q += 64) {
                h1 += (double)a.rowacc[(size_t)row * a.ld_part + q];
                h2 += (double)a.rowacc2[(size_t)row * a.ld_part + q];
            }
            h1 = wave_sum(h1); h2 = wave_sum(h2);
        } else {
            h1 = (double)a.rowacc[row];
            if (a.rowacc2) h2 = (double)a.rowacc2[row];
        }
        s0 += t - h1;
        if (a.rowacc2) s1 += t2 - h2;
        if (a.rowacc3) s2 += t - (double)a.rowacc3[row];
    }
    __shared__ double s_part[3][4];
    if (lane == 0) { s_part[0][wv] = s0; s_part[1][wv] = s1; s_part[2][wv] = s2; }
    __syncthreads();
    if (threadIdx.x < 3) {
        const double v = (s_part[threadIdx.x][0] + s_part[threadIdx.x][1]) + (s_part[threadIdx.x][2] + s_part[threadIdx.x][3]);
        if (threadIdx.x == 0 || (threadIdx.x == 1 && a.rowacc2) || (threadIdx.x == 2 && a.rowacc3)) atomicAdd(a.out + threadIdx.x, v);
    }
}
BM_KERNEL __launch_bounds__(256) void fe_row_kernel(FeRowArgs a) { fe_row_body(a, (int)blockIdx.x); }
BM_KERNEL __launch_bounds__(256) void metrics_tail_kernel(SqJob j0, SqJob j1, FeRowArgs r, int nb_sq) {
    if ((int)blockIdx.x < nb_sq) sqdiff2_body(j0, j1, (int)blockIdx.x, nb_sq);
    else fe_row_body(r, (int)blockIdx.x - nb_sq);
}

BM_KERNEL void pll_index_kernel(int *out, int B, int V, PhiloxKey key, unsigned long long row0) {
    const int b = blockIdx.x * blockDim.x + threadIdx.x;
    if (b >= B) return;
    const unsigned long long idx = row0 + b;
    uint32_t w[4];
    philox_block(key, idx >> 2, w);
    out[b] = (int)(w[idx & 3] % (uint32_t)V);
}

struct DbmBiasArgs {
    const float *s_pos, *s_neg;
    float *b, *db;
    float *q, *mm, *pen;
    int n, layer;
    float N, M, lr, mom, damping, cost, target;
};
__device__ __forceinline__ void dbm_bias_apply(const DbmBiasArgs &a, int c, float g) {
    if (a.q) {
        const float qn = a.damping * a.q[c] + (1.0f - a.damping) * a.s_neg[a.layer];
        const float mn = a.damping * a.mm[c] + (1.0f - a.damping) * a.s_pos[a.layer];
        a.q[c] = qn;
        a.mm[c] = mn;
        const float p1 = a.cost * (qn - a.target);
        const float p2 = a.cost * (mn - a.target);
        const float pen = p1 + p2;
        a.pen[c] = pen;
        g = g - pen;
    }
    const float d = a.lr * (a.mom * a.db[c] + g);
    a.db[c] = d;
    a.b[c] = a.b[c] + d;
}
__device__ __forceinline__ void dbm_bias_update(const DbmBiasArgs &a, int c) {
    dbm_bias_apply(a, c, a.s_pos[c] / a.N - a.s_neg[c] / a.M);
}
BM_KERNEL void dbm_bias_kernel(DbmBiasArgs a) {
    const int c = blockIdx.x * blockDim.x + threadIdx.x;
    if (c < a.n) dbm_bias_update(a, c);
}
constexpr int DBM_BIAS_JOBS = 1 + 4;
struct DbmBiasMulti { DbmBiasArgs job[DBM_BIAS_JOBS]; };
BM_KERNEL void dbm_bias_multi_kernel(DbmBiasMulti m) {
    const DbmBiasArgs &a = m.job[blockIdx.y];
    const int c = blockIdx.x * blockDim.x + threadIdx.x;
    if (c < a.n) dbm_bias_update(a, c);
}

struct MaxNormArgs {
    float *W, *Wt;
    int I, J, ldw, ldwt;
    float max_norm;
    float *norm_out;
    float *num, *den;
    int c_first, c_end;
};
constexpr int MN_CH = 256;
constexpr int MN_COLS = 16;
constexpr int MN_NV = MN_CH * (MN_COLS / 4) / NT;
struct MnRegs { float4 v[MN_NV]; };
__device__ __forceinline__ void maxnorm_load(const MaxNormArgs &a, int c0, int r0, bool full, MnRegs &r) {
    const int tid = threadIdx.x;
    if (full) {
#pragma unroll
        for (int n = 0; n < MN_NV; ++n) {
            const int f = tid + n * NT, row = r0 + (f >> 2), c = c0 + 4 * (f & 3);
            const int rc = row < a.J ? row : a.J - 1;
            r.v[n] = *reinterpret_cast<const float4 *>(a.W + (size_t)rc * a.ldw + c);
        }
    } else {
#pragma unroll
        for (int n = 0; n < MN_NV; ++n) {
            const int f = tid + n * NT, row = r0 + (f >> 2), c = c0 + 4 * (f & 3);
            const int rc = row < a.J ? row : a.J - 1;
            const float *src = a.W + (size_t)rc * a.ldw;
            const int last = a.I - 1;
            r.v[n] = make_float4(src[c < last ? c : last], src[c + 1 < last ? c + 1 : last], src[c + 2 < last ? c + 2 : last],
                                 src[c + 3 < last ? c + 3 : last]);
        }
    }
}
__device__ __forceinline__ void maxnorm_store(const MaxNormArgs &a, int c0, int r0, float *buf, MnRegs &r) {
    const int tid = threadIdx.x;
#pragma unroll
    for (int n = 0; n < MN_NV; ++n) {
        const int f = tid + n * NT, row = f >> 2, c4 = f & 3, c = c0 + 4 * c4;
        const bool rok = r0 + row < a.J;
        float4 v = r.v[n];
        v.x = (rok && c < a.I) ? v.x : 0.f;
        v.y = (rok && c + 1 < a.I) ? v.y : 0.f;
        v.z = (rok && c + 2 < a.I) ? v.z : 0.f;
        v.w = (rok && c + 3 < a.I) ? v.w : 0.f;
        *reinterpret_cast<float4 *>(buf + row * 16 + 4 * c4) = v;
    }
}
BM_KERNEL __launch_bounds__(NT) void maxnorm_kernel(MaxNormArgs a) {
    static_assert(NT == 256 && MN_NV >= 1 && MN_NV * NT == MN_CH * (MN_COLS / 4), "loader split");
    __shared__ __attribute__((aligned(16))) float sA[2][MN_CH * 16];
    const int tid = threadIdx.x, lane = tid & 63, w = tid >> 6;
    const int g = lane >> 4, l15 = lane & 15;
    const int c0 = a.c_first + blockIdx.x * MN_COLS;
    const bool full = (a.ldw & 3) == 0 && (((uintptr_t)a.W) & 15u) == 0 && c0 + MN_COLS <= a.I;
    f32x4 acc = (f32x4){0.f, 0.f, 0.f, 0.f};
    const int nch = (a.J + MN_CH - 1) / MN_CH;
    MnRegs R0, R1, R2;
    maxnorm_load(a, c0, 0, full, R0);
    if (nch > 1) maxnorm_load(a, c0, MN_CH, full, R1);
    if (nch > 2) maxnorm_load(a, c0, 2 * MN_CH, full, R2);
#define BM_MN_STEP(R, CH)                                                                         \
    if ((CH) < nch) {                                                                             \
        maxnorm_store(a, c0, (CH) * MN_CH, sA[(CH) & 1], R);                                      \
        if ((CH) + 3 < nch) maxnorm_load(a, c0, ((CH) + 3) * MN_CH, full, R);                     \
        wg_barrier();           \
        if (w == 0) {                                                                             \
            const float *img = sA[(CH) & 1];                                                      \
            _Pragma("unroll 2")                                                                   \
            for (int s = 0; s < MN_CH / 4; s += 8) {       \
                float d[8];                                                                       \
                _Pragma("unroll")                                                                 \
                for (int u = 0; u < 8; ++u) d[u] = img[(4 * (s + u) + g) * 16 + l15];             \
                _Pragma("unroll")                                                                 \
                for (int u = 0; u < 8; ++u) acc = __builtin_amdgcn_mfma_f32_16x16x4f32(d[u], d[u], acc, 0, 0, 0); \
            }                                                                                     \
        }                                                                                         \
    }
    for (int ch = 0; ch < nch; ch += 3) {
        BM_MN_STEP(R0, ch)
        BM_MN_STEP(R1, ch + 1)
        BM_MN_STEP(R2, ch + 2)
    }
#undef BM_MN_STEP
    const int c = c0 + l15;
    if (w == 0 && (l15 >> 2) == g && c < a.I) {
        const float nrm = sqrtf(acc[l15 & 3]);
        a.num[c] = fminf(nrm, a.max_norm);
        a.den[c] = fmaxf(nrm, 1e-8f);
        if (a.norm_out) a.norm_out[c] = nrm;
    }
}
BM_KERNEL __launch_bounds__(256) void maxnorm_scale_kernel(MaxNormArgs a) {
    __shared__ float t[32][33];
    const int tx = threadIdx.x & 31, ty = threadIdx.x >> 5;
    const int tiles_c = (a.c_end - a.c_first + 31) / 32;
    const int c0 = a.c_first + (blockIdx.x % tiles_c) * 32, j0 = (blockIdx.x / tiles_c) * 32;
    const int c = c0 + tx;
    const float num = c < a.I ? a.num[c] : 0.f, den = c < a.I ? a.den[c] : 1.f;
#pragma unroll
    for (int r = ty; r < 32; r += 8) {
        const int j = j0 + r;
        float wn = 0.f;
        if (j < a.J && c < a.I) {
            const size_t o = (size_t)j * a.ldw + c;
            wn = (a.W[o] * num) / den;
            a.W[o] = wn;
        }
        t[r][tx] = wn;
    }
    if (!a.Wt) return;
    __syncthreads();
#pragma unroll
    for (int r = ty; r < 32; r += 8) {
        const int cc = c0 + r, j = j0 + tx;
        if (cc < a.I && j < a.J) a.Wt[(size_t)cc * a.ldwt + j] = t[tx][r];
    }
}

BM_KERNEL __launch_bounds__(256) void mf_ctl_kernel(MfCtl *c, float tol, int init, float *blk, int nblk) {
    __shared__ float s_m[4];
    float m = 0.f;
    for (int e = threadIdx.x; e < nblk; e += 256) { m = fmaxf(m, blk[e]); blk[e] = 0.f; }
#pragma unroll
    for (int off = 32; off > 0; off >>= 1) m = fmaxf(m, __shfl_xor(m, off));
    if ((threadIdx.x & 63) == 0) s_m[threadIdx.x >> 6] = m;
    __syncthreads();
    if (threadIdx.x != 0) return;
    const float resid = fmaxf(fmaxf(fmaxf(s_m[0], s_m[1]), fmaxf(s_m[2], s_m[3])), __uint_as_float(c->maxdiff));
    if (init) {
        c->steps = 0;
        c->done = !(resid > tol);
    } else if (!c->done) {
        c->steps += 1;
        c->done = !(resid > tol);
    }
    c->maxdiff = 0u;
}

BM_KERNEL __launch_bounds__(256) void mf_resid_kernel(MfCtl *c, float *blk, int nblk) {
    __shared__ float s_m[4];
    float m = 0.f;
    for (int e = threadIdx.x; e < nblk; e += 256) { m = fmaxf(m, blk[e]); blk[e] = 0.f; }
#pragma unroll
    for (int off = 32; off > 0; off >>= 1) m = fmaxf(m, __shfl_xor(m, off));
    if ((threadIdx.x & 63) == 0) s_m[threadIdx.x >> 6] = m;
    __syncthreads();
    if (threadIdx.x != 0) return;
    c->resid = fmaxf(fmaxf(fmaxf(s_m[0], s_m[1]), fmaxf(s_m[2], s_m[3])), __uint_as_float(c->maxdiff));
    c->maxdiff = 0u;
}
BM_KERNEL void mf_latch_kernel(MfCtl *c, float tol, int init) {
    if (threadIdx.x != 0 || blockIdx.x != 0) return;
    if (init) {
        c->steps = 0;
        c->done = !(c->resid > tol);
    } else if (!c->done) {
        c->steps += 1;
        c->done = !(c->resid > tol);
    }
}

BM_KERNEL __launch_bounds__(256) void maxabsdiff_kernel(const float *A, int lda, const float *B, int ldb, int rows, int cols, unsigned *out) {
    __shared__ float s_m[4];
    float m = 0.f;
    const bool vec = ((lda | ldb) & 3) == 0 && ((((uintptr_t)A) | ((uintptr_t)B)) & 15u) == 0;
    if (vec) {
        const int c4n = cols >> 2;
        const long long n = (long long)rows * c4n;
        const long long stride = (long long)gridDim.x * 256;
        long long e = (long long)blockIdx.x * 256 + threadIdx.x;
        for (; e + 3 * stride < n; e += 4 * stride) {
            float4 x[4], y[4];
#pragma unroll
            for (int u = 0; u < 4; ++u) {
                const long long f = e + u * stride;
                const int r = (int)(f / c4n), c = 4 * (int)(f % c4n);
                x[u] = *reinterpret_cast<const float4 *>(A + (size_t)r * lda + c);
                y[u] = *reinterpret_cast<const float4 *>(B + (size_t)r * ldb + c);
            }
#pragma unroll
            for (int u = 0; u < 4; ++u)
                m = fmaxf(m, fmaxf(fmaxf(fabsf(x[u].x - y[u].x), fabsf(x[u].y - y[u].y)), fmaxf(fabsf(x[u].z - y[u].z), fabsf(x[u].w - y[u].w))));
        }
        for (; e < n; e += stride) {
            const int r = (int)(e / c4n), c = 4 * (int)(e % c4n);
            const float4 x = *reinterpret_cast<const float4 *>(A + (size_t)r * lda + c), y = *reinterpret_cast<const float4 *>(B + (size_t)r * ldb + c);
            m = fmaxf(m, fmaxf(fmaxf(fabsf(x.x - y.x), fabsf(x.y - y.y)), fmaxf(fabsf(x.z - y.z), fabsf(x.w - y.w))));
        }
        for (int r = blockIdx.x; r < rows; r += gridDim.x)
            for (int c = 4 * c4n + threadIdx.x; c < cols; c += 256) m = fmaxf(m, fabsf(A[(size_t)r * lda + c] - B[(size_t)r * ldb + c]));
    } else {
        for (int r = blockIdx.x; r < rows; r += gridDim.x) {
            const float *pa = A + (size_t)r * lda, *pb = B + (size_t)r * ldb;
            for (int c = threadIdx.x; c < cols; c += 256) m = fmaxf(m, fabsf(pa[c] - pb[c]));
        }
    }
#pragma unroll
    for (int off = 32; off > 0; off >>= 1) m = fmaxf(m, __shfl_xor(m, off));
    if ((threadIdx.x & 63) == 0) s_m[threadIdx.x >> 6] = m;
    __syncthreads();
    if (threadIdx.x == 0) {
        m = fmaxf(fmaxf(s_m[0], s_m[1]), fmaxf(s_m[2], s_m[3]));
        if (m > 0.f) atomicMax(out, __float_as_uint(m));
    }
}

BM_KERNEL __launch_bounds__(256) void mf_init0_kernel(const float *Z, int ldz, const float *bias, const float *prev, int ldp,
                                                       float *out, int ldo, int rows, int cols, float mult, float bmult, int lit,
                                                       unsigned *maxdiff, float *blk) {
    __shared__ float s_m[4];
    float dm = 0.f;
    for (int r = blockIdx.x; r < rows; r += gridDim.x) {
        const float *z = Z + (size_t)r * ldz, *p = prev + (size_t)r * ldp;
        float *o = out + (size_t)r * ldo;
        for (int c = threadIdx.x; c < cols; c += 256) {
            const float x = mult * z[c];
            const float b = bmult * bias[c];
            const float m = lit ? sigmoid_literal(x + b) : sigmoid(x + b);
            dm = fmaxf(dm, fabsf(m - p[c]));
            o[c] = m;
        }
    }
#pragma unroll
    for (int off = 32; off > 0; off >>= 1) dm = fmaxf(dm, __shfl_xor(dm, off));
    if ((threadIdx.x & 63) == 0) s_m[threadIdx.x >> 6] = dm;
    __syncthreads();
    if (threadIdx.x == 0) {
        dm = fmaxf(fmaxf(s_m[0], s_m[1]), fmaxf(s_m[2], s_m[3]));
        if (blk && gridDim.x <= BM_MF_SLOTS) blk[blockIdx.x] = dm;
        else if (dm > 0.f) atomicMax(maxdiff, __float_as_uint(dm));
    }
}

struct AisScoreArgs {
    const float *pe[3]; int ne_slots[3]; int ne;
    const float *po[2]; int no_slots[2]; int no;
};

BM_KERNEL __launch_bounds__(256) void ais_score_kernel(double *logw, int J, int ld, AisScoreArgs p, float dbeta) {
    __shared__ double s_s[8][32], s_d[8][32];
    const int c = threadIdx.x & 31, t = threadIdx.x >> 5;
    const int j = blockIdx.x * 32 + c;
    double s = 0.0, d = 0.0;
    if (j < J) {
#pragma unroll
        for (int e = 0; e < 3; ++e)
            if (e < p.ne) for (int q = t; q < p.ne_slots[e]; q += 8) s += (double)p.pe[e][(size_t)q * ld + j];
#pragma unroll
        for (int o = 0; o < 2; ++o)
            if (o < p.no) for (int q = t; q < p.no_slots[o]; q += 8) d += (double)p.po[o][(size_t)q * ld + j];
    }
    s_s[t][c] = s; s_d[t][c] = d;
    __syncthreads();
    if (t == 0 && j < J) {
        const double ss = ((s_s[0][c] + s_s[1][c]) + (s_s[2][c] + s_s[3][c])) + ((s_s[4][c] + s_s[5][c]) + (s_s[6][c] + s_s[7][c]));
        const double dd = ((s_d[0][c] + s_d[1][c]) + (s_d[2][c] + s_d[3][c])) + ((s_d[4][c] + s_d[5][c]) + (s_d[6][c] + s_d[7][c]));
        logw[j] += ss + (double)dbeta * dd;
    }
}


}

#include "bm_launch.h"
```

boltzmann_machines_amd/csrc/bm_xchg.hip:

```cpp
#include "../../include/bm355.h"
#include "bm_common.h"

#include <unistd.h>

namespace bmx {

constexpr int MAXR = 8;
constexpr int NTX = 256;
enum : int { F_READY = 0, F_DONE = MAXR, F_STATUS = 2 * MAXR, F_WORDS = 2 * MAXR + 8 };

typedef float f32x4 __attribute__((ext_vector_type(4)));
typedef unsigned u32x4 __attribute__((ext_vector_type(4)));

struct Blob {
    hipIpcMemHandle_t h_buf, h_red, h_flags;
    uint64_t off_buf;
    int32_t pid, device, rank, pad;
    uint64_t count;
    char fill[256 - 3 * 64 - 8 - 16 - 8];
};
static_assert(sizeof(Blob) == 256, "blob layout");

struct Args {
    float *buf, *red;
    unsigned long long count, chunk;
    unsigned long long red_cap;
    int rank, n;
    unsigned epoch;
    const float *pbuf[MAXR], *pred[MAXR];
    unsigned *pflags[MAXR];
    unsigned *flags;
    unsigned *ctr;
    int grid;
    long long timeout_ticks;
};

__device__ __forceinline__ __amdgpu_buffer_rsrc_t rsrc(const void *p, unsigned long long bytes) {
    const unsigned n = bytes > 0xfffffff0ull ? 0xfffffff0u : (unsigned)bytes;
    return __builtin_amdgcn_make_buffer_rsrc(const_cast<void *>(p), 0, (int)n, 0x00020000);
}
__device__ __forceinline__ f32x4 load_sys(__amdgpu_buffer_rsrc_t r, unsigned byte_off) {
    return __builtin_bit_cast(f32x4, __builtin_amdgcn_raw_buffer_load_b128(r, (int)byte_off, 0, 17));
}
__device__ __forceinline__ void store_sys(__amdgpu_buffer_rsrc_t r, unsigned byte_off, f32x4 v) {
    __builtin_amdgcn_raw_buffer_store_b128(__builtin_bit_cast(u32x4, v), r, (int)byte_off, 0, 17);
}

__device__ __forceinline__ bool wait_all(const Args &a, int base, int code) {
    const int tid = threadIdx.x;
    int bad = 0;
    if (tid < a.n) {
        const long long t0 = wall_clock64();
        while ((int)(__hip_atomic_load(a.flags + base + tid, __ATOMIC_RELAXED, __HIP_MEMORY_SCOPE_SYSTEM) - a.epoch) < 0) {
            __builtin_amdgcn_s_sleep(4);
            if (wall_clock64() - t0 > a.timeout_ticks) { bad = 1; break; }
        }
        if (bad) __hip_atomic_store(a.flags + F_STATUS, (unsigned)(code * 16 + tid + 1), __ATOMIC_RELAXED, __HIP_MEMORY_SCOPE_SYSTEM);
    }
    bad = __syncthreads_or(bad);
    if (!bad && __hip_atomic_load(a.flags + F_STATUS, __ATOMIC_RELAXED, __HIP_MEMORY_SCOPE_SYSTEM) != 0u) bad = 1;
    __atomic_thread_fence(__ATOMIC_ACQUIRE);
    return !bad;
}

__global__ __launch_bounds__(NTX) void allreduce_kernel(Args a) {
    const int tid = threadIdx.x, me = a.rank, n = a.n;
    if (blockIdx.x == 0 && tid < n)
        __hip_atomic_store(a.pflags[tid] + F_READY + me, a.epoch, __ATOMIC_RELEASE, __HIP_MEMORY_SCOPE_SYSTEM);
    const bool ok1 = wait_all(a, F_READY, 1);
    const float qnan = __builtin_nanf("");
    const unsigned long long base = (unsigned long long)me * a.chunk;
    const unsigned long long len = base < a.count ? (a.count - base < a.chunk ? a.count - base : a.chunk) : 0ull;
    const unsigned long long len4 = (len + 3) / 4;
    {
        __amdgpu_buffer_rsrc_t rs[MAXR];
#pragma unroll
        for (int r = 0; r < MAXR; ++r) rs[r] = rsrc(r < n ? a.pbuf[r] + base : a.buf, r < n ? len4 * 16 : 0);
        __amdgpu_buffer_rsrc_t rred = rsrc(a.red, len4 * 16);
        for (unsigned long long e = (unsigned long long)blockIdx.x * NTX + tid; e < len4; e += (unsigned long long)a.grid * NTX) {
            const unsigned off = (unsigned)(e * 16);
            f32x4 v[MAXR];
#pragma unroll
            for (int r = 0; r < MAXR; ++r) if (r < n) v[r] = load_sys(rs[r], off);
            f32x4 s = v[0];
#pragma unroll
            for (int r = 1; r < MAXR; ++r) if (r < n) s = s + v[r];
            if (!ok1) s = (f32x4){qnan, qnan, qnan, qnan};
            *reinterpret_cast<f32x4 *>(a.buf + base + e * 4) = s;
            store_sys(rred, off, s);
        }
    }
    __threadfence_system();
    __syncthreads();
    if (tid == 0) {
        const unsigned old = __hip_atomic_fetch_add(a.ctr, 1u, __ATOMIC_ACQ_REL, __HIP_MEMORY_SCOPE_AGENT);
        if (old + 1u == (unsigned)a.grid * a.epoch) {
            __threadfence_system();
            for (int r = 0; r < n; ++r)
                __hip_atomic_store(a.pflags[r] + F_DONE + me, a.epoch, __ATOMIC_RELEASE, __HIP_MEMORY_SCOPE_SYSTEM);
        }
    }
    if (n == 1) return;
    const bool ok2 = wait_all(a, F_DONE, 2);
    for (int d = 1; d < n; ++d) {
        if (!ok2) {
            const unsigned long long bq = (unsigned long long)((me + d) % n) * a.chunk;
            const unsigned long long lq = bq < a.count ? (a.count - bq < a.chunk ? a.count - bq : a.chunk) : 0ull;
            for (unsigned long long e = (unsigned long long)blockIdx.x * NTX + tid; e < (lq + 3) / 4; e += (unsigned long long)a.grid * NTX)
                *reinterpret_cast<f32x4 *>(a.buf + bq + e * 4) = (f32x4){qnan, qnan, qnan, qnan};
            continue;
        }
        const int q = (me + d) % n;
        const unsigned long long bq = (unsigned long long)q * a.chunk;
        const unsigned long long lq = bq < a.count ? (a.count - bq < a.chunk ? a.count - bq : a.chunk) : 0ull;
        const unsigned long long lq4 = (lq + 3) / 4;
        __amdgpu_buffer_rsrc_t rq = rsrc(a.pred[q], lq4 * 16);
        unsigned long long e = (unsigned long long)blockIdx.x * NTX + tid;
        const unsigned long long st = (unsigned long long)a.grid * NTX;
        for (; e + st < lq4; e += 2 * st) {
            const f32x4 v0 = load_sys(rq, (unsigned)(e * 16)), v1 = load_sys(rq, (unsigned)((e + st) * 16));
            *reinterpret_cast<f32x4 *>(a.buf + bq + e * 4) = v0;
            *reinterpret_cast<f32x4 *>(a.buf + bq + (e + st) * 4) = v1;
        }
        if (e < lq4) *reinterpret_cast<f32x4 *>(a.buf + bq + e * 4) = load_sys(rq, (unsigned)(e * 16));
    }
}

struct RbmApply {
    float *W, *dW;
    unsigned long long countW, chunkW;
    int I, ldw, V, H;
    float N, l2, lr, mom, damping, cost, target;
    float *vb, *dvb, *hb, *dhb, *q, *pen;
    float *tail_red;
    unsigned *tail_flag;
    int dw_only;
};

__global__ __launch_bounds__(NTX) void exchange_apply_kernel(Args a, RbmApply p) {
    const int tid = threadIdx.x, me = a.rank, n = a.n;
    const float qnan = __builtin_nanf("");
    if (blockIdx.x == 0 && tid < n)
        __hip_atomic_store(a.pflags[tid] + F_READY + me, a.epoch, __ATOMIC_RELEASE, __HIP_MEMORY_SCOPE_SYSTEM);
    const bool ok1 = wait_all(a, F_READY, 1);
    const unsigned long long base = (unsigned long long)me * p.chunkW;
    const unsigned long long len = base < p.countW ? (p.countW - base < p.chunkW ? p.countW - base : p.chunkW) : 0ull;
    const unsigned long long len4 = len / 4;
    __amdgpu_buffer_rsrc_t rred = rsrc(a.red, len4 * 16);
    if (!p.dw_only) {
        if (blockIdx.x == gridDim.x - 1) {
            const int T = p.V + 2 * p.H, T4 = (T + 3) / 4;
            __amdgpu_buffer_rsrc_t rt[MAXR];
#pragma unroll
            for (int r = 0; r < MAXR; ++r) rt[r] = rsrc(r < n ? a.pbuf[r] + p.countW : a.buf, r < n ? (unsigned long long)T4 * 16 : 0);
            for (int c4 = tid; c4 < T4; c4 += NTX) {
                f32x4 v[MAXR];
#pragma unroll
                for (int r = 0; r < MAXR; ++r) if (r < n) v[r] = load_sys(rt[r], (unsigned)c4 * 16u);
                f32x4 s = v[0];
#pragma unroll
                for (int r = 1; r < MAXR; ++r) if (r < n) s = s + v[r];
                if (!ok1) s = (f32x4){qnan, qnan, qnan, qnan};
                *reinterpret_cast<f32x4 *>(p.tail_red + 4 * c4) = s;
            }
            __syncthreads();
            const float *sv = p.tail_red, *sh = p.tail_red + p.V, *sq = p.tail_red + p.V + p.H;
            for (int c = tid; c < p.V + p.H; c += NTX) {
                if (c < p.V) {
                    const float g = sv[c] / p.N;
                    const float d = p.lr * (p.mom * p.dvb[c] + g);
                    p.dvb[c] = d;
                    p.vb[c] = p.vb[c] + d;
                } else {
                    const int h = c - p.V;
                    const float qn = p.damping * p.q[h] + (1.0f - p.damping) * sq[h];
                    p.q[h] = qn;
                    const float pen = p.cost * (qn - p.target);
                    p.pen[h] = pen;
                    float g = sh[h] / p.N;
                    g = g - pen;
                    const float d = p.lr * (p.mom * p.dhb[h] + g);
                    p.dhb[h] = d;
                    p.hb[h] = p.hb[h] + d;
                }
            }
            __threadfence();
            __syncthreads();
            if (tid == 0) __hip_atomic_store(p.tail_flag, a.epoch, __ATOMIC_RELEASE, __HIP_MEMORY_SCOPE_AGENT);
        }
        bool okp = true;
        if (p.cost != 0.f) {
            int bad = 0;
            if (tid == 0) {
                const long long t0 = wall_clock64();
                while ((int)(__hip_atomic_load(p.tail_flag, __ATOMIC_ACQUIRE, __HIP_MEMORY_SCOPE_AGENT) - a.epoch) < 0) {
                    __builtin_amdgcn_s_sleep(2);
                    if (wall_clock64() - t0 > a.timeout_ticks) { bad = 1; break; }
                }
                if (bad) __hip_atomic_store(a.flags + F_STATUS, (unsigned)(4 * 16 + me + 1), __ATOMIC_RELAXED, __HIP_MEMORY_SCOPE_SYSTEM);
            }
            okp = !__syncthreads_or(bad);
        }
        const bool pow2 = bm::grad_pow2(p.N);
        const float invN = 1.0f / p.N;
        __amdgpu_buffer_rsrc_t rs[MAXR];
#pragma unroll
        for (int r = 0; r < MAXR; ++r) rs[r] = rsrc(r < n ? a.pbuf[r] + base : a.buf, r < n ? len4 * 16 : 0);
        for (unsigned long long e = (unsigned long long)blockIdx.x * NTX + tid; e < len4; e += (unsigned long long)a.grid * NTX) {
            const unsigned off = (unsigned)(e * 16);
            f32x4 v[MAXR];
#pragma unroll
            for (int r = 0; r < MAXR; ++r) if (r < n) v[r] = load_sys(rs[r], off);
            f32x4 s = v[0];
#pragma unroll
            for (int r = 1; r < MAXR; ++r) if (r < n) s = s + v[r];
            const unsigned long long flat = base + e * 4;
            const int i = (int)(flat % (unsigned long long)p.ldw);
            f32x4 wv = *reinterpret_cast<const f32x4 *>(p.W + flat), dv = *reinterpret_cast<const f32x4 *>(p.dW + flat);
            if (i < p.I) {
                f32x4 pe = (f32x4){0.f, 0.f, 0.f, 0.f};
                if (p.cost != 0.f) pe = *reinterpret_cast<const f32x4 *>(p.pen + i);
#pragma unroll
                for (int c = 0; c < 4; ++c) {
                    const float g = bm::grad_norm1(s[c], p.N, invN, pow2);
                    float w = wv[c], d = dv[c];
                    bm::apply_w_update(g, pe[c], p.l2, p.lr, p.mom, w, d);
                    wv[c] = w; dv[c] = d;
                }
                if (!ok1 || !okp) wv = dv = (f32x4){qnan, qnan, qnan, qnan};
                *reinterpret_cast<f32x4 *>(p.W + flat) = wv;
                *reinterpret_cast<f32x4 *>(p.dW + flat) = dv;
            }
            store_sys(rred, off, wv);
        }
    } else {
        for (unsigned long long e = (unsigned long long)blockIdx.x * NTX + tid; e < len4; e += (unsigned long long)a.grid * NTX)
            store_sys(rred, (unsigned)(e * 16), *reinterpret_cast<const f32x4 *>(p.dW + base + e * 4));
    }
    __threadfence_system();
    __syncthreads();
    if (tid == 0) {
        const unsigned old = __hip_atomic_fetch_add(a.ctr, 1u, __ATOMIC_ACQ_REL, __HIP_MEMORY_SCOPE_AGENT);
        if (old + 1u == (unsigned)a.grid * a.epoch) {
            __threadfence_system();
            for (int r = 0; r < n; ++r)
                __hip_atomic_store(a.pflags[r] + F_DONE + me, a.epoch, __ATOMIC_RELEASE, __HIP_MEMORY_SCOPE_SYSTEM);
        }
    }
    if (n == 1) return;
    const bool ok2 = wait_all(a, F_DONE, 2);
    float *dst = p.dw_only ? p.dW : p.W;
    for (int d = 1; d < n; ++d) {
        const int q = (me + d) % n;
        const unsigned long long bq = (unsigned long long)q * p.chunkW;
        const unsigned long long lq = bq < p.countW ? (p.countW - bq < p.chunkW ? p.countW - bq : p.chunkW) : 0ull;
        const unsigned long long lq4 = lq / 4;
        __amdgpu_buffer_rsrc_t rq = rsrc(a.pred[q], lq4 * 16);
        const unsigned long long st = (unsigned long long)a.grid * NTX;
        unsigned long long e = (unsigned long long)blockIdx.x * NTX + tid;
        if (!ok2) {
            for (; e < lq4; e += st) *reinterpret_cast<f32x4 *>(dst + bq + e * 4) = (f32x4){qnan, qnan, qnan, qnan};
            continue;
        }
        for (; e + st < lq4; e += 2 * st) {
            const f32x4 v0 = load_sys(rq, (unsigned)(e * 16)), v1 = load_sys(rq, (unsigned)((e + st) * 16));
            *reinterpret_cast<f32x4 *>(dst + bq + e * 4) = v0;
            *reinterpret_cast<f32x4 *>(dst + bq + (e + st) * 4) = v1;
        }
        if (e < lq4) *reinterpret_cast<f32x4 *>(dst + bq + e * 4) = load_sys(rq, (unsigned)(e * 16));
    }
}

struct DbmLayerX {
    float *W, *dW, *Wt, *wnorm;
    const float *pen;
    unsigned long long off_pos, off_neg;
    unsigned long long red_off;
    int I, J, ldw, ldwt, sw;
};
struct DbmApply {
    int L, mode, do_ready;
    DbmLayerX lay[BM_DBM_MAX_LAYERS];
    bm::DbmBiasArgs bias[BM_DBM_MAX_LAYERS + 1];
    unsigned long long off_sums; int n_sums;
    float N, M, l2, lr, mom;
    float *tail_red; unsigned *tail_flag;
};

__global__ __launch_bounds__(NTX) void dbm_exchange_apply_kernel(Args a, DbmApply p) {
    const int tid = threadIdx.x, me = a.rank, n = a.n;
    const float qnan = __builtin_nanf("");
    if (blockIdx.x == 0 && tid < n)
        __hip_atomic_store(a.pflags[tid] + F_READY + me, a.epoch, __ATOMIC_RELEASE, __HIP_MEMORY_SCOPE_SYSTEM);
    const bool ok1 = wait_all(a, F_READY, 1);
    __amdgpu_buffer_rsrc_t rs[MAXR];
#pragma unroll
    for (int r = 0; r < MAXR; ++r) rs[r] = rsrc(r < n ? a.pbuf[r] : a.buf, r < n ? ((a.count + 3) & ~3ull) * 4 : 0);
    if (blockIdx.x == gridDim.x - 1) {
        const int T4 = (p.n_sums + 3) / 4;
        for (int c4 = tid; c4 < T4; c4 += NTX) {
            const unsigned off = (unsigned)((p.off_sums + 4ull * c4) * 4);
            f32x4 v[MAXR];
#pragma unroll
            for (int r = 0; r < MAXR; ++r) if (r < n) v[r] = load_sys(rs[r], off);
            f32x4 s = v[0];
#pragma unroll
            for (int r = 1; r < MAXR; ++r) if (r < n) s = s + v[r];
            if (!ok1) s = (f32x4){qnan, qnan, qnan, qnan};
            *reinterpret_cast<f32x4 *>(p.tail_red + 4 * c4) = s;
        }
        __syncthreads();
        for (int v = 0; v <= p.L; ++v)
            for (int c = tid; c < p.bias[v].n; c += NTX) bm::dbm_bias_update(p.bias[v], c);
        __threadfence();
        __syncthreads();
        if (tid == 0) __hip_atomic_store(p.tail_flag, a.epoch, __ATOMIC_RELEASE, __HIP_MEMORY_SCOPE_AGENT);
    }
    bool okp = true;
    {
        int bad = 0;
        if (tid == 0) {
            const long long t0 = wall_clock64();
            while ((int)(__hip_atomic_load(p.tail_flag, __ATOMIC_ACQUIRE, __HIP_MEMORY_SCOPE_AGENT) - a.epoch) < 0) {
                __builtin_amdgcn_s_sleep(2);
                if (wall_clock64() - t0 > a.timeout_ticks) { bad = 1; break; }
            }
            if (bad) __hip_atomic_store(a.flags + F_STATUS, (unsigned)(4 * 16 + me + 1), __ATOMIC_RELAXED, __HIP_MEMORY_SCOPE_SYSTEM);
        }
        okp = !__syncthreads_or(bad);
    }
    const bool pow2 = bm::grad_pow2(p.N) && bm::grad_pow2(p.M);
    const float invN = 1.0f / p.N, invM = 1.0f / p.M;
    for (int i = 0; i < p.L; ++i) {
        const DbmLayerX &y = p.lay[i];
        const int c0 = me * y.sw, c1 = (c0 + y.sw < y.I) ? c0 + y.sw : y.I;
        if (c1 <= c0) continue;
        const unsigned w4 = (unsigned)(c1 - c0) / 4u;
        const unsigned long long n4 = (unsigned long long)y.J * w4;
        for (unsigned long long e = (unsigned long long)blockIdx.x * NTX + tid; e < n4; e += (unsigned long long)a.grid * NTX) {
            const int j = (int)(e / w4), c = c0 + 4 * (int)(e % w4);
            const unsigned long long o = (unsigned long long)j * y.ldw + c;
            const unsigned bp = (unsigned)((y.off_pos + o) * 4), bn = (unsigned)((y.off_neg + o) * 4);
            f32x4 vp[MAXR], vn[MAXR];
#pragma unroll
            for (int r = 0; r < MAXR; ++r) if (r < n) { vp[r] = load_sys(rs[r], bp); vn[r] = load_sys(rs[r], bn); }
            f32x4 sp = vp[0], sn = vn[0];
#pragma unroll
            for (int r = 1; r < MAXR; ++r) if (r < n) { sp = sp + vp[r]; sn = sn + vn[r]; }
            f32x4 wv = *reinterpret_cast<const f32x4 *>(y.W + o), dv = *reinterpret_cast<const f32x4 *>(y.dW + o);
            const f32x4 pe = *reinterpret_cast<const f32x4 *>(y.pen + c);
#pragma unroll
            for (int q = 0; q < 4; ++q) {
                const float g = bm::grad_norm2(sp[q], sn[q], p.N, p.M, invN, invM, pow2);
                float w = wv[q], d = dv[q];
                bm::apply_w_update(g, pe[q], p.l2, p.lr, p.mom, w, d);
                wv[q] = w; dv[q] = d;
            }
            if (!ok1 || !okp) wv = dv = (f32x4){qnan, qnan, qnan, qnan};
            *reinterpret_cast<f32x4 *>(y.W + o) = wv;
            *reinterpret_cast<f32x4 *>(y.dW + o) = dv;
        }
    }
}

__global__ __launch_bounds__(NTX) void dbm_exchange_gather_kernel(Args a, DbmApply p) {
    __shared__ float t[32][33];
    const int tid = threadIdx.x, me = a.rank, n = a.n;
    const float qnan = __builtin_nanf("");
    if (p.do_ready) {
        if (blockIdx.x == 0 && tid < n)
            __hip_atomic_store(a.pflags[tid] + F_READY + me, a.epoch, __ATOMIC_RELEASE, __HIP_MEMORY_SCOPE_SYSTEM);
        (void)wait_all(a, F_READY, 1);
    }
    __amdgpu_buffer_rsrc_t rred = rsrc(a.red, a.red_cap * 4);
    for (int i = 0; i < p.L; ++i) {
        const DbmLayerX &y = p.lay[i];
        const int c0 = me * y.sw, c1 = (c0 + y.sw < y.I) ? c0 + y.sw : y.I;
        if (c1 <= c0) continue;
        const float *src = p.mode ? y.dW : y.W;
        const unsigned w4 = (unsigned)(c1 - c0) / 4u;
        const unsigned long long n4 = (unsigned long long)y.J * w4;
        for (unsigned long long e = (unsigned long long)blockIdx.x * NTX + tid; e < n4; e += (unsigned long long)a.grid * NTX) {
            const int j = (int)(e / w4), cc = 4 * (int)(e % w4);
            store_sys(rred, (unsigned)((y.red_off + (unsigned long long)j * y.sw + cc) * 4),
                      *reinterpret_cast<const f32x4 *>(src + (unsigned long long)j * y.ldw + c0 + cc));
        }
        if (!p.mode && blockIdx.x == 0)
            for (unsigned e = tid; e < w4; e += NTX)
                store_sys(rred, (unsigned)((y.red_off + (unsigned long long)y.J * y.sw + 4 * e) * 4),
                          *reinterpret_cast<const f32x4 *>(y.wnorm + c0 + 4 * e));
    }
    __threadfence_system();
    __syncthreads();
    if (tid == 0) {
        const unsigned old = __hip_atomic_fetch_add(a.ctr, 1u, __ATOMIC_ACQ_REL, __HIP_MEMORY_SCOPE_AGENT);
        if (old + 1u == (unsigned)a.grid * a.epoch) {
            __threadfence_system();
            for (int r = 0; r < n; ++r)
                __hip_atomic_store(a.pflags[r] + F_DONE + me, a.epoch, __ATOMIC_RELEASE, __HIP_MEMORY_SCOPE_SYSTEM);
        }
    }
    if (n == 1) return;
    const bool ok2 = wait_all(a, F_DONE, 2);
    for (int i = 0; i < p.L; ++i) {
        const DbmLayerX &y = p.lay[i];
        float *dst = p.mode ? y.dW : y.W;
        for (int d = 1; d < n; ++d) {
            const int q = (me + d) % n;
            const int q0 = q * y.sw, q1 = (q0 + y.sw < y.I) ? q0 + y.sw : y.I;
            if (q1 <= q0) continue;
            __amdgpu_buffer_rsrc_t rq = rsrc(a.pred[q], a.red_cap * 4);
            const int tiles_c = (q1 - q0 + 31) / 32, tiles_j = (y.J + 31) / 32;
            for (int tile = blockIdx.x; tile < tiles_c * tiles_j; tile += a.grid) {
                const int cb = (tile % tiles_c) * 32, j0 = (tile / tiles_c) * 32;
                const int r = tid >> 3, c4 = tid & 7;
                const int j = j0 + r, c = q0 + cb + 4 * c4;
                f32x4 v = (f32x4){0.f, 0.f, 0.f, 0.f};
                if (j < y.J && c < q1) {
                    v = ok2 ? load_sys(rq, (unsigned)((y.red_off + (unsigned long long)j * y.sw + cb + 4 * c4) * 4))
                            : (f32x4){qnan, qnan, qnan, qnan};
                    *reinterpret_cast<f32x4 *>(dst + (unsigned long long)j * y.ldw + c) = v;
                }
                if (!p.mode) {
                    t[r][4 * c4] = v[0]; t[r][4 * c4 + 1] = v[1]; t[r][4 * c4 + 2] = v[2]; t[r][4 * c4 + 3] = v[3];
                    __syncthreads();
                    const int cc = q0 + cb + r, jq = j0 + 4 * c4;
                    if (cc < q1 && jq < y.J) {
                        float *wt = y.Wt + (unsigned long long)cc * y.ldwt + jq;
                        if (jq + 3 < y.J) *reinterpret_cast<f32x4 *>(wt) = (f32x4){t[4 * c4][r], t[4 * c4 + 1][r], t[4 * c4 + 2][r], t[4 * c4 + 3][r]};
                        else for (int e = 0; e < 4; ++e) if (jq + e < y.J) wt[e] = t[4 * c4 + e][r];
                    }
                    __syncthreads();
                }
            }
            if (!p.mode && blockIdx.x == 0)
                for (int e = tid; e < (q1 - q0) / 4; e += NTX)
                    *reinterpret_cast<f32x4 *>(y.wnorm + q0 + 4 * e) =
                        ok2 ? load_sys(rq, (unsigned)((y.red_off + (unsigned long long)y.J * y.sw + 4 * e) * 4)) : (f32x4){qnan, qnan, qnan, qnan};
        }
    }
}

struct MaxArgs {
    float *val;
    unsigned long long *slots;
    unsigned long long *pslots[MAXR];
    unsigned *flags;
    int rank, n;
    unsigned epoch;
    long long timeout_ticks;
};
__global__ __launch_bounds__(64) void max1_kernel(MaxArgs a) {
    const int tid = threadIdx.x;
    const unsigned par = a.epoch & 1u;
    const float mine = *a.val;
    float got = 0.f;
    if (tid < a.n) {
        const unsigned long long word = ((unsigned long long)a.epoch << 32) | (unsigned long long)__float_as_uint(mine);
        __hip_atomic_store(a.pslots[tid] + par * MAXR + a.rank, word, __ATOMIC_RELAXED, __HIP_MEMORY_SCOPE_SYSTEM);
        const long long t0 = wall_clock64();
        unsigned long long w;
        bool ok = true;
        while ((unsigned)((w = __hip_atomic_load(a.slots + par * MAXR + tid, __ATOMIC_RELAXED, __HIP_MEMORY_SCOPE_SYSTEM)) >> 32) != a.epoch) {
            __builtin_amdgcn_s_sleep(2);
            if (wall_clock64() - t0 > a.timeout_ticks) { ok = false; break; }
        }
        if (ok) got = __uint_as_float((unsigned)w);
        else __hip_atomic_store(a.flags + F_STATUS, (unsigned)(3 * 16 + tid + 1), __ATOMIC_RELAXED, __HIP_MEMORY_SCOPE_SYSTEM);
    }
#pragma unroll
    for (int off = 32; off > 0; off >>= 1) got = fmaxf(got, __shfl_xor(got, off));
    if (tid == 0) *a.val = got;
}

__global__ __launch_bounds__(256) void mf_ctl_max1_kernel(MaxArgs a, bm::MfCtl *c, float *blk, int nblk, float tol, int init) {
    __shared__ float s_m[4];
    __shared__ float s_resid;
    const int tid = threadIdx.x;
    float m = 0.f;
    for (int e = tid; e < nblk; e += 256) { m = fmaxf(m, blk[e]); blk[e] = 0.f; }
#pragma unroll
    for (int off = 32; off > 0; off >>= 1) m = fmaxf(m, __shfl_xor(m, off));
    if ((tid & 63) == 0) s_m[tid >> 6] = m;
    __syncthreads();
    if (tid == 0) {
        s_resid = fmaxf(fmaxf(fmaxf(s_m[0], s_m[1]), fmaxf(s_m[2], s_m[3])), __uint_as_float(c->maxdiff));
        c->maxdiff = 0u;
    }
    __syncthreads();
    if (tid >= 64) return;
    const unsigned par = a.epoch & 1u;
    const float mine = s_resid;
    float got = 0.f;
    if (tid < a.n) {
        const unsigned long long word = ((unsigned long long)a.epoch << 32) | (unsigned long long)__float_as_uint(mine);
        __hip_atomic_store(a.pslots[tid] + par * MAXR + a.rank, word, __ATOMIC_RELAXED, __HIP_MEMORY_SCOPE_SYSTEM);
        const long long t0 = wall_clock64();
        unsigned long long w;
        bool ok = true;
        while ((unsigned)((w = __hip_atomic_load(a.slots + par * MAXR + tid, __ATOMIC_RELAXED, __HIP_MEMORY_SCOPE_SYSTEM)) >> 32) != a.epoch) {
            __builtin_amdgcn_s_sleep(2);
            if (wall_clock64() - t0 > a.timeout_ticks) { ok = false; break; }
        }
        if (ok) got = __uint_as_float((unsigned)w);
        else __hip_atomic_store(a.flags + F_STATUS, (unsigned)(3 * 16 + tid + 1), __ATOMIC_RELAXED, __HIP_MEMORY_SCOPE_SYSTEM);
    }
#pragma unroll
    for (int off = 32; off > 0; off >>= 1) got = fmaxf(got, __shfl_xor(got, off));
    if (tid != 0) return;
    c->resid = got;
    if (init) {
        c->steps = 0;
        c->done = !(got > tol);
    } else if (!c->done) {
        c->steps += 1;
        c->done = !(got > tol);
    }
}

}

struct bm_xchg {
    int rank = 0, nranks = 1, device = 0;
    float *buf = nullptr, *red = nullptr;
    size_t count = 0, chunk = 0, red_cap = 0;
    unsigned *flags = nullptr, *ctr = nullptr;
    unsigned long long *slots = nullptr;
    const float *pbuf[bmx::MAXR], *pred[bmx::MAXR];
    unsigned *pflags[bmx::MAXR];
    void *opened[3 * bmx::MAXR];
    int n_opened = 0;
    bool attached = false;
    unsigned epoch = 0, epoch_max = 0;
    int grid = 1;
    long long timeout_ticks = 0;
    float *tail_red = nullptr;
    unsigned *tail_flag = nullptr;
    size_t tail_n = 0;
    bool dw_stale = false;
    bm_xchg **user = nullptr;
};

static int xchg_alloc_flags(bm_xchg *x) {
    const size_t bytes = bmx::F_WORDS * sizeof(unsigned) + 2 * bmx::MAXR * sizeof(unsigned long long);
    void *p = nullptr;
    hipError_t e = hipExtMallocWithFlags(&p, bytes, hipDeviceMallocUncached);
    if (e != hipSuccess) { (void)hipGetLastError(); e = hipExtMallocWithFlags(&p, bytes, hipDeviceMallocFinegrained); }
    BM_HIP(e);
    BM_HIP(hipMemset(p, 0, bytes));
    x->flags = (unsigned *)p;
    x->slots = (unsigned long long *)((char *)p + bmx::F_WORDS * sizeof(unsigned));
    return 0;
}

static int xchg_check_status(bm_xchg *x) {
    if (!x) return 0;
    unsigned s = 0;
    BM_HIP(hipMemcpy(&s, x->flags + bmx::F_STATUS, sizeof(s), hipMemcpyDeviceToHost));
    BM_CHECK(s == 0, "bm_xchg: a wait for rank %u expired in phase %u (1 READY, 2 DONE, 3 max, 4 penalty): the results of "
                     "this exchange are NaN-poisoned, the job is lost", (s & 15u) - 1u, s >> 4);
    return 0;
}

static void xchg_bind_user(bm_xchg *x, bm_xchg **slot) { if (x) x->user = slot; }
static void xchg_dw_replaced(bm_xchg *x) { if (x) x->dw_stale = false; }

static int xchg_mf_ctl_step(bm_xchg *x, bm::MfCtl *ctl, float *blk, int nblk, float tol, int init, hipStream_t stream) {
    BM_CHECK(x && x->attached && ctl, "exchange not attached / null argument");
    bmx::MaxArgs a;
    memset(&a, 0, sizeof(a));
    a.val = &ctl->resid; a.slots = x->slots; a.flags = x->flags; a.rank = x->rank; a.n = x->nranks;
    a.epoch = ++x->epoch_max; a.timeout_ticks = x->timeout_ticks;
    for (int r = 0; r < bmx::MAXR; ++r)
        a.pslots[r] = (unsigned long long *)((char *)x->pflags[r] + bmx::F_WORDS * sizeof(unsigned));
    hipLaunchKernelGGL(bmx::mf_ctl_max1_kernel, dim3(1), dim3(256), 0, stream, a, ctl, blk, nblk, tol, init);
    BM_HIP(hipGetLastError());
    return 0;
}

extern "C" {

static int xchg_create(int32_t rank, int32_t nranks, float *buf_dev, size_t count, size_t min_red, bm_xchg **out) {
    BM_CHECK(out && buf_dev, "null argument");
    BM_CHECK(nranks >= 1 && nranks <= bmx::MAXR && rank >= 0 && rank < nranks, "bad rank %d of %d (at most %d ranks)", rank, nranks, bmx::MAXR);
    BM_CHECK(((uintptr_t)buf_dev & 15u) == 0, "the exchanged buffer must be 16-byte aligned");
    bm_xchg *x = new bm_xchg();
    x->rank = rank; x->nranks = nranks; x->buf = buf_dev; x->count = count;
    x->chunk = (((count + nranks - 1) / nranks) + 3) & ~(size_t)3;
    x->red_cap = ((x->chunk > min_red ? x->chunk : min_red) + 3) & ~(size_t)3;
    auto fail = [&]() { if (x->red) (void)hipFree(x->red); if (x->ctr) (void)hipFree(x->ctr); if (x->flags) (void)hipFree(x->flags); delete x; return 1; };
    if (hipGetDevice(&x->device) != hipSuccess ||
        hipMalloc((void **)&x->red, (x->red_cap ? x->red_cap : 4) * sizeof(float)) != hipSuccess ||
        hipMalloc((void **)&x->ctr, 64) != hipSuccess || hipMemset(x->ctr, 0, 64) != hipSuccess) {
        bm::set_error("bm_xchg_create: device allocation failed: %s", hipGetErrorString(hipGetLastError()));
        return fail();
    }
    if (xchg_alloc_flags(x)) return fail();
    int ncu = 0, per_cu = 0;
    {
        hipDeviceProp_t pr;
        if (hipGetDeviceProperties(&pr, x->device) == hipSuccess) ncu = pr.multiProcessorCount;
        if (hipOccupancyMaxActiveBlocksPerMultiprocessor(&per_cu, bmx::dbm_exchange_gather_kernel, bmx::NTX, 0) != hipSuccess) { (void)hipGetLastError(); per_cu = 0; }
    }
    if (ncu < 1 || per_cu < 1) { bm::set_error("bm_xchg_create: cannot establish a co-resident launch width (CUs %d, workgroups per CU %d)", ncu, per_cu); return fail(); }
    const size_t f4 = (x->chunk / 4 + bmx::NTX - 1) / bmx::NTX;
    x->grid = (int)(f4 < 1 ? 1 : (f4 > (size_t)ncu ? (size_t)ncu : f4));
    const char *t = getenv("BM_XCHG_TIMEOUT_S");
    x->timeout_ticks = (long long)((t ? atof(t) : 20.0) * 1e8);
    for (int r = 0; r < bmx::MAXR; ++r) { x->pbuf[r] = x->buf; x->pred[r] = x->red; x->pflags[r] = x->flags; }
    x->attached = nranks == 1;
    *out = x;
    return 0;
}

int bm_xchg_create(int32_t rank, int32_t nranks, float *buf_dev, size_t count, bm_xchg **out) {
    return xchg_create(rank, nranks, buf_dev, count, 0, out);
}

int bm_xchg_blob_bytes(void) { return (int)sizeof(bmx::Blob); }

int bm_xchg_export(bm_xchg *x, void *out_blob256) {
    BM_CHECK(x && out_blob256, "null argument");
    bmx::Blob b;
    memset(&b, 0, sizeof(b));
    void *base = nullptr; size_t sz = 0;
    BM_HIP(hipMemGetAddressRange((hipDeviceptr_t *)&base, &sz, (hipDeviceptr_t)x->buf));
    BM_CHECK((char *)x->buf + ((x->count + 3) & ~(size_t)3) * sizeof(float) <= (char *)base + sz,
             "the exchanged buffer's allocation must cover its length rounded up to 16 bytes");
    b.off_buf = (uint64_t)((char *)x->buf - (char *)base);
    BM_HIP(hipIpcGetMemHandle(&b.h_buf, base));
    BM_HIP(hipIpcGetMemHandle(&b.h_red, x->red));
    BM_HIP(hipIpcGetMemHandle(&b.h_flags, x->flags));
    b.pid = (int32_t)getpid(); b.device = x->device; b.rank = x->rank; b.count = x->count;
    memcpy(out_blob256, &b, sizeof(b));
    return 0;
}

int bm_xchg_attach(bm_xchg *x, const void *all_blobs) {
    BM_CHECK(x && all_blobs, "null argument");
    BM_CHECK(!x->attached || x->nranks == 1, "already attached");
    const bmx::Blob *bl = (const bmx::Blob *)all_blobs;
    for (int r = 0; r < x->nranks; ++r) {
        BM_CHECK(bl[r].rank == r, "blob %d carries rank %d: the blobs must be ordered by rank", r, bl[r].rank);
        BM_CHECK(bl[r].count == x->count, "rank %d exchanges %llu floats, this rank %zu", r, (unsigned long long)bl[r].count, x->count);
        if (r == x->rank) continue;
        BM_CHECK(bl[r].pid != (int32_t)getpid(), "rank %d lives in this process: one process per rank", r);
        void *pb = nullptr, *pr = nullptr, *pf = nullptr;
        BM_HIP(hipIpcOpenMemHandle(&pb, bl[r].h_buf, hipIpcMemLazyEnablePeerAccess));
        x->opened[x->n_opened++] = pb;
        BM_HIP(hipIpcOpenMemHandle(&pr, bl[r].h_red, hipIpcMemLazyEnablePeerAccess));
        x->opened[x->n_opened++] = pr;
        BM_HIP(hipIpcOpenMemHandle(&pf, bl[r].h_flags, hipIpcMemLazyEnablePeerAccess));
        x->opened[x->n_opened++] = pf;
        x->pbuf[r] = (const float *)((char *)pb + bl[r].off_buf);
        x->pred[r] = (const float *)pr;
        x->pflags[r] = (unsigned *)pf;
    }
    x->attached = true;
    return 0;
}

int bm_xchg_destroy(bm_xchg *x) {
    if (!x) return 0;
    (void)hipDeviceSynchronize();
    if (x->user) *x->user = nullptr;
    for (int i = 0; i < x->n_opened; ++i) (void)hipIpcCloseMemHandle(x->opened[i]);
    if (x->red) (void)hipFree(x->red);
    if (x->tail_red) (void)hipFree(x->tail_red);
    if (x->tail_flag) (void)hipFree(x->tail_flag);
    if (x->ctr) (void)hipFree(x->ctr);
    if (x->flags) (void)hipFree(x->flags);
    delete x;
    return 0;
}

int bm_xchg_allreduce_sum(bm_xchg *x, void *stream) {
    BM_CHECK(x && x->attached, "exchange not attached (bm_xchg_export -> gather the blobs -> bm_xchg_attach)");
    bmx::Args a;
    memset(&a, 0, sizeof(a));
    a.buf = x->buf; a.red = x->red; a.count = x->count; a.chunk = x->chunk;
    a.rank = x->rank; a.n = x->nranks; a.epoch = ++x->epoch;
    for (int r = 0; r < bmx::MAXR; ++r) { a.pbuf[r] = x->pbuf[r]; a.pred[r] = x->pred[r]; a.pflags[r] = x->pflags[r]; }
    a.flags = x->flags; a.ctr = x->ctr; a.grid = x->grid; a.timeout_ticks = x->timeout_ticks;
    hipLaunchKernelGGL(bmx::allreduce_kernel, dim3(x->grid), dim3(bmx::NTX), 0, (hipStream_t)stream, a);
    BM_HIP(hipGetLastError());
    return 0;
}

int bm_xchg_allreduce_max1(bm_xchg *x, float *val_dev, void *stream) {
    BM_CHECK(x && x->attached && val_dev, "exchange not attached / null argument");
    bmx::MaxArgs a;
    memset(&a, 0, sizeof(a));
    a.val = val_dev; a.slots = x->slots; a.flags = x->flags; a.rank = x->rank; a.n = x->nranks;
    a.epoch = ++x->epoch_max; a.timeout_ticks = x->timeout_ticks;
    for (int r = 0; r < bmx::MAXR; ++r)
        a.pslots[r] = (unsigned long long *)((char *)x->pflags[r] + bmx::F_WORDS * sizeof(unsigned));
    hipLaunchKernelGGL(bmx::max1_kernel, dim3(1), dim3(64), 0, (hipStream_t)stream, a);
    BM_HIP(hipGetLastError());
    return 0;
}

int bm_xchg_status(bm_xchg *x, int32_t *out_status) {
    BM_CHECK(x && out_status, "null argument");
    BM_HIP(hipDeviceSynchronize());
    unsigned s = 0;
    BM_HIP(hipMemcpy(&s, x->flags + bmx::F_STATUS, sizeof(s), hipMemcpyDeviceToHost));
    *out_status = (int32_t)s;
    if (s) bm::set_error("bm_xchg: wait for rank %u timed out in phase %u (1 READY, 2 DONE, 3 max)", (s & 15u) - 1u, s >> 4);
    return 0;
}

int bm_xchg_set_timeout(bm_xchg *x, double seconds) {
    BM_CHECK(x && seconds > 0.0, "bad argument");
    x->timeout_ticks = (long long)(seconds * 1e8);
    return 0;
}

int bm_xchg_set_max_workgroups(bm_xchg *x, int32_t n) {
    BM_CHECK(x && n >= 1, "bad argument");
    BM_CHECK(x->epoch == 0, "bm_xchg_set_max_workgroups: call it before the first exchange");
    if (x->grid > n) x->grid = n;
    return 0;
}

int bm_xchg_info(bm_xchg *x, int32_t *out_rank, int32_t *out_nranks, size_t *out_count) {
    BM_CHECK(x, "null argument");
    if (out_rank) *out_rank = x->rank;
    if (out_nranks) *out_nranks = x->nranks;
    if (out_count) *out_count = x->count;
    return 0;
}

static int xchg_launch_apply(bm_rbm *h, bm_xchg *x, float N_global, float lr, float mom, int dw_only) {
    void *p = nullptr; size_t n = 0;
    BM_TRY(bm_rbm_dev_ptr(h, "grad", &p, &n));
    BM_CHECK(x->attached && p == (void *)x->buf && n == x->count, "the exchange was created for another buffer (gradient slots are not supported)");
    BM_CHECK(h->H % 4 == 0 && h->W.ld % 4 == 0 && h->W.ld == h->dW.ld, "the fused exchange needs n_hidden % 4 == 0");
    const size_t tail = (size_t)h->V + 2 * (size_t)h->H;
    if (!x->tail_red || x->tail_n < tail) {
        if (x->tail_red) (void)hipFree(x->tail_red);
        BM_HIP(hipMalloc((void **)&x->tail_red, (tail + 4) * sizeof(float)));
        x->tail_n = tail;
    }
    if (!x->tail_flag) {
        BM_HIP(hipMalloc((void **)&x->tail_flag, 64));
        BM_HIP(hipMemsetAsync(x->tail_flag, 0, 64, h->stream));
    }
    bmx::Args a;
    memset(&a, 0, sizeof(a));
    a.buf = x->buf; a.red = x->red; a.count = x->count; a.chunk = x->chunk;
    a.rank = x->rank; a.n = x->nranks; a.epoch = ++x->epoch;
    for (int r = 0; r < bmx::MAXR; ++r) { a.pbuf[r] = x->pbuf[r]; a.pred[r] = x->pred[r]; a.pflags[r] = x->pflags[r]; }
    a.flags = x->flags; a.ctr = x->ctr; a.grid = x->grid; a.timeout_ticks = x->timeout_ticks;
    bmx::RbmApply q;
    memset(&q, 0, sizeof(q));
    q.W = h->W.p; q.dW = h->dW.p;
    h->wt_valid = false;
    h->eff_valid = false;
    q.countW = (unsigned long long)h->V * h->W.ld;
    q.chunkW = (((q.countW + x->nranks - 1) / x->nranks) + 3) & ~3ull;
    BM_CHECK(q.chunkW <= x->chunk, "staging slice too small");
    q.I = h->H; q.ldw = h->W.ld; q.V = h->V; q.H = h->H;
    q.N = N_global; q.l2 = h->cfg.l2; q.lr = lr; q.mom = mom;
    q.damping = h->cfg.sparsity_damping; q.cost = h->cfg.sparsity_cost; q.target = h->cfg.sparsity_target;
    q.vb = h->vb.p; q.dvb = h->dvb.p; q.hb = h->hb.p; q.dhb = h->dhb.p; q.q = h->q.p; q.pen = h->pen.p;
    q.tail_red = x->tail_red; q.tail_flag = x->tail_flag; q.dw_only = dw_only;
    hipLaunchKernelGGL(bmx::exchange_apply_kernel, dim3(x->grid), dim3(bmx::NTX), 0, h->stream, a, q);
    BM_HIP(hipGetLastError());
    h->xchg_used = x; x->user = &h->xchg_used;
    return 0;
}

int bm_rbm_exchange_apply_direct(bm_rbm *h, bm_xchg *x, int32_t B_global, float lr, float mom) {
    BM_CHECK(!h || !h->cen_on, "bm_rbm_exchange_apply_direct: the exchange's fused apply has no centred form; switch centering off");
    BM_TRY(refuse_nrelu(h, "bm_rbm_exchange_apply_direct"));
    BM_CHECK(h && x, "null argument");
    BM_CHECK(B_global > 0, "bm_rbm_exchange_apply_direct: B_global = %d must be positive", B_global);
    BM_TRY(xchg_launch_apply(h, x, (float)B_global, lr, mom, 0));
    x->dw_stale = x->nranks > 1;
    h->dw_sharded = x->dw_stale;
    return 0;
}
int bm_rbm_exchange_gather_dw(bm_rbm *h, bm_xchg *x) {
    BM_CHECK(h && x, "null argument");
    BM_TRY(refuse_nrelu(h, "bm_rbm_exchange_gather_dw"));
    if (x->nranks == 1 || (!x->dw_stale && !(h->H % 4 == 0 && h->W.ld % 4 == 0 && h->W.ld == h->dW.ld))) {
        x->dw_stale = false; h->dw_sharded = false; return 0;
    }
    BM_TRY(xchg_launch_apply(h, x, 1.f, 0.f, 0.f, 1));
    x->dw_stale = false;
    h->dw_sharded = false;
    return 0;
}

int bm_rbm_xchg_create(bm_rbm *h, int32_t rank, int32_t nranks, bm_xchg **out) {
    BM_CHECK(h && out, "null argument");
    BM_TRY(refuse_nrelu(h, "bm_rbm_xchg_create"));
    void *p = nullptr; size_t n = 0;
    BM_TRY(bm_rbm_dev_ptr(h, "grad", &p, &n));
    return bm_xchg_create(rank, nranks, (float *)p, n, out);
}
static int dbm_slice_width(int I, int nranks) { return 32 * ((I + 32 * nranks - 1) / (32 * nranks)); }
static size_t dbm_staging_floats(const bm_dbm *h, int nranks) {
    size_t need = 0;
    for (int i = 0; i < h->L; ++i) need += ((size_t)h->n[i] + 1) * (size_t)dbm_slice_width(h->n[i + 1], nranks);
    return need;
}
int bm_dbm_xchg_create(bm_dbm *h, int32_t rank, int32_t nranks, bm_xchg **out) {
    BM_CHECK(h && out, "null argument");
    void *p = nullptr; size_t n = 0;
    BM_TRY(bm_dbm_dev_ptr(h, "grad", &p, &n));
    return xchg_create(rank, nranks, (float *)p, n, nranks >= 1 ? dbm_staging_floats(h, nranks) : 0, out);
}

static bool dbm_fused_ok(const bm_dbm *h, const bm_xchg *x) {
    if (!x->attached || x->buf != h->grad.p || x->count != h->grad.n) return false;
    if (((x->count + 3) & ~(size_t)3) * sizeof(float) >= 0xfffffff0ull || x->red_cap * sizeof(float) >= 0xfffffff0ull) return false;
    if (dbm_staging_floats(h, x->nranks) > x->red_cap) return false;
    for (int i = 0; i < h->L; ++i)
        if (h->n[i + 1] % 4 != 0 || h->W[i].ld % 4 != 0 || h->Wt[i].ld % 4 != 0 || h->W[i].ld != h->dW[i].ld) return false;
    return true;
}
int bm_dbm_exchange_apply_ok(bm_dbm *h, bm_xchg *x, int32_t *out_ok) {
    BM_CHECK(h && x && out_ok, "null argument");
    *out_ok = dbm_fused_ok(h, x) ? 1 : 0;
    return 0;
}

static int dbm_fill_exchange(bm_dbm *h, bm_xchg *x, bmx::Args &a, bmx::DbmApply &q, bool new_epoch) {
    memset(&a, 0, sizeof(a));
    a.buf = x->buf; a.red = x->red; a.count = x->count; a.chunk = x->chunk; a.red_cap = x->red_cap;
    a.rank = x->rank; a.n = x->nranks; a.epoch = new_epoch ? ++x->epoch : x->epoch;
    for (int r = 0; r < bmx::MAXR; ++r) { a.pbuf[r] = x->pbuf[r]; a.pred[r] = x->pred[r]; a.pflags[r] = x->pflags[r]; }
    a.flags = x->flags; a.ctr = x->ctr; a.grid = x->grid; a.timeout_ticks = x->timeout_ticks;
    memset(&q, 0, sizeof(q));
    q.L = h->L;
    size_t roff = 0;
    for (int i = 0; i < h->L; ++i) {
        bmx::DbmLayerX &y = q.lay[i];
        y.W = h->W[i].p; y.dW = h->dW[i].p; y.Wt = h->Wt[i].p; y.wnorm = h->wnorm[i].p; y.pen = h->pen[i].p;
        y.off_pos = h->raw_off[i][0]; y.off_neg = h->raw_off[i][1];
        y.I = h->n[i + 1]; y.J = h->n[i]; y.ldw = h->W[i].ld; y.ldwt = h->Wt[i].ld;
        y.sw = dbm_slice_width(y.I, x->nranks);
        y.red_off = roff;
        roff += ((size_t)y.J + 1) * (size_t)y.sw;
    }
    return 0;
}

int bm_dbm_exchange_apply_direct(bm_dbm *h, bm_xchg *x, int32_t N_global, int32_t M_global, float lr, float mom) {
    BM_CHECK(!h || !h->cen_on, "bm_dbm_exchange_apply_direct: the exchange's fused apply has no centred form; switch centering off");
    BM_CHECK(h && x, "null argument");
    BM_CHECK(N_global > 0 && M_global > 0, "bm_dbm_exchange_apply_direct: N_global = %d and M_global = %d must be positive", N_global, M_global);
    BM_CHECK(!h->failed, "an earlier launch of this engine failed");
    BM_CHECK(dbm_fused_ok(h, x), "the fused DBM exchange needs an attached exchange created by bm_dbm_xchg_create for this "
                                 "engine and layer widths that are multiples of 4 (bm_dbm_exchange_apply_ok)");
    const size_t nsums = h->grad.n - (size_t)(h->sums_p - h->grad.p);
    if (!x->tail_red || x->tail_n < nsums) {
        if (x->tail_red) (void)hipFree(x->tail_red);
        BM_HIP(hipMalloc((void **)&x->tail_red, (nsums + 4) * sizeof(float)));
        x->tail_n = nsums;
    }
    if (!x->tail_flag) {
        BM_HIP(hipMalloc((void **)&x->tail_flag, 64));
        BM_HIP(hipMemsetAsync(x->tail_flag, 0, 64, h->stream));
    }
    bmx::Args a; bmx::DbmApply q;
    BM_TRY(dbm_fill_exchange(h, x, a, q, true));
    q.off_sums = (unsigned long long)(h->sums_p - h->grad.p); q.n_sums = (int)nsums;
    q.N = (float)N_global; q.M = (float)M_global; q.l2 = h->cfg.l2; q.lr = lr; q.mom = mom;
    q.tail_red = x->tail_red; q.tail_flag = x->tail_flag;
    {
        DbmBiasArgs &b = q.bias[0];
        b.s_pos = x->tail_red + sums_off(h, 0); b.s_neg = x->tail_red + sums_off(h, 1);
        b.b = h->vb.p; b.db = h->dvb.p; b.n = h->V; b.N = q.N; b.M = q.M; b.lr = lr; b.mom = mom;
        for (int i = 0; i < h->L; ++i) {
            DbmBiasArgs &c = q.bias[1 + i];
            c.s_pos = x->tail_red + sums_off(h, 2 + 2 * i); c.s_neg = x->tail_red + sums_off(h, 3 + 2 * i);
            c.b = h->hb[i].p; c.db = h->dhb[i].p; c.q = h->q[i].p; c.mm = h->mm[i].p; c.pen = h->pen[i].p;
            c.n = h->n[i + 1]; c.layer = i; c.N = q.N; c.M = q.M; c.lr = lr; c.mom = mom;
            c.damping = h->cfg.sparsity_damping; c.cost = h->cfg.sparsity_cost[i]; c.target = h->cfg.sparsity_target[i];
        }
    }
    hipLaunchKernelGGL(bmx::dbm_exchange_apply_kernel, dim3(x->grid), dim3(bmx::NTX), 0, h->stream, a, q);
    for (int i = 0; i < h->L; ++i) {
        const int c0 = x->rank * q.lay[i].sw;
        const int c1 = c0 + q.lay[i].sw < q.lay[i].I ? c0 + q.lay[i].sw : q.lay[i].I;
        launch_dbm_maxnorm(h, i, c0, c1 > c0 ? c1 : c0);
    }
    hipLaunchKernelGGL(bmx::dbm_exchange_gather_kernel, dim3(x->grid), dim3(bmx::NTX), 0, h->stream, a, q);
    BM_HIP(hipGetLastError());
    h->xchg_used = x; x->user = &h->xchg_used;
    x->dw_stale = x->nranks > 1;
    h->dw_sharded = x->dw_stale;
    h->dw_set_mask = 0;
    BM_CHECK(!h->failed, "a launch helper of this update could not allocate");
    return 0;
}
int bm_dbm_exchange_gather_dw(bm_dbm *h, bm_xchg *x) {
    BM_CHECK(h && x, "null argument");
    if (x->nranks == 1 || (!x->dw_stale && !dbm_fused_ok(h, x))) { x->dw_stale = false; h->dw_sharded = false; return 0; }
    BM_CHECK(dbm_fused_ok(h, x), "the exchange does not belong to this engine");
    bmx::Args a; bmx::DbmApply q;
    BM_TRY(dbm_fill_exchange(h, x, a, q, true));
    q.mode = 1; q.do_ready = 1;
    hipLaunchKernelGGL(bmx::dbm_exchange_gather_kernel, dim3(x->grid), dim3(bmx::NTX), 0, h->stream, a, q);
    BM_HIP(hipGetLastError());
    h->xchg_used = x; x->user = &h->xchg_used;
    x->dw_stale = false;
    h->dw_sharded = false;
    return 0;
}
static int xchg_allreduce_prefix(bm_xchg *x, size_t n, hipStream_t stream) {
    BM_CHECK(x && x->attached && n >= 1 && n <= x->count, "exchange not attached / bad prefix length");
    bmx::Args a;
    memset(&a, 0, sizeof(a));
    a.buf = x->buf; a.red = x->red; a.count = n;
    a.chunk = (((n + x->nranks - 1) / x->nranks) + 3) & ~(size_t)3;
    BM_CHECK(a.chunk <= x->red_cap, "staging slice too small");
    a.rank = x->rank; a.n = x->nranks; a.epoch = ++x->epoch;
    for (int r = 0; r < bmx::MAXR; ++r) { a.pbuf[r] = x->pbuf[r]; a.pred[r] = x->pred[r]; a.pflags[r] = x->pflags[r]; }
    a.flags = x->flags; a.ctr = x->ctr; a.grid = x->grid; a.timeout_ticks = x->timeout_ticks;
    hipLaunchKernelGGL(bmx::allreduce_kernel, dim3(x->grid), dim3(bmx::NTX), 0, stream, a);
    BM_HIP(hipGetLastError());
    return 0;
}

__global__ void ais_window_kernel(const double *logw, float *win, int lo, int n_win, int a, int b, double logZ0, int literal, int fail) {
    const int e = blockIdx.x * blockDim.x + threadIdx.x;
    if (e >= n_win) return;
    const int c = lo + e;
    float v = 0.f;
    if (c >= a && c < b) v = fail ? __builtin_nanf("") : (literal ? (float)logw[c - a] + (float)logZ0 : (float)(logw[c - a] + logZ0));
    win[e] = v;
}

int bm_dbm_ais_sharded_direct(bm_dbm *h, bm_xchg *x, int32_t n_betas, int32_t n_runs_total, int32_t k, uint64_t seed,
                              float *values_host) {
    BM_CHECK(h && x && values_host, "null argument");
    BM_CHECK(x->attached, "exchange not attached");
    BM_CHECK(n_runs_total >= 1, "bad AIS arguments");
    void *gp = nullptr; size_t gn = 0;
    BM_TRY(bm_dbm_dev_ptr(h, "grad", &gp, &gn));
    BM_CHECK(gp == (void *)x->buf && gn == x->count, "the exchange was created for another buffer");
    BM_CHECK(!h->dw_sharded, "the momentum buffers are sharded (bm_dbm_exchange_gather_dw first)");
    const int rank = x->rank, world = x->nranks;
    const int q = n_runs_total / world, rem = n_runs_total % world;
    const int a = rank * q + (rank < rem ? rank : rem), b = a + q + (rank < rem ? 1 : 0);
    std::string first_err;
    int rc = 0;
    if (b > a) rc = ais_core(h, n_betas, b - a, k, seed, a);
    if (rc) { first_err = bm_last_error(); (void)hipGetLastError(); }
    const double z0 = ais_log_Z0(h, h->ais_literal != 0);
    h->xchg_used = x; x->user = &h->xchg_used;
    int rc_x = 0, rc_m = 0;
    for (size_t lo = 0; lo < (size_t)n_runs_total && !rc_x && !rc_m; lo += x->count) {
        const size_t nw = (size_t)n_runs_total - lo < x->count ? (size_t)n_runs_total - lo : x->count;
        hipLaunchKernelGGL(ais_window_kernel, dim3((unsigned)((nw + 255) / 256)), dim3(256), 0, h->stream,
                           (const double *)h->alogw.p, x->buf, (int)lo, (int)nw, a, b, z0, h->ais_literal, rc ? 1 : 0);
        rc_x = xchg_allreduce_prefix(x, nw, h->stream);
        if (rc_x) { if (first_err.empty()) first_err = bm_last_error(); break; }
        if (hipMemcpyAsync(values_host + lo, x->buf, nw * sizeof(float), hipMemcpyDeviceToHost, h->stream) != hipSuccess) rc_m = 1;
        if (hipStreamSynchronize(h->stream) != hipSuccess) rc_m = 1;
    }
    if (rc || rc_x) { bm::set_error("bm_dbm_ais_sharded_direct (rank %d): %s", rank, first_err.c_str()); return rc ? rc : rc_x; }
    if (rc_m) { bm::set_error("bm_dbm_ais_sharded_direct: device copy / synchronisation failed"); return 1; }
    BM_TRY(xchg_check_status(x));
    for (int e = 0; e < n_runs_total; ++e)
        BM_CHECK(values_host[e] == values_host[e], "bm_dbm_ais_sharded_direct: another rank's AIS sweep failed (chain %d arrived as NaN)", e);
    return 0;
}

int bm_rbm_allreduce_grads_direct(bm_rbm *h, bm_xchg *x) {
    BM_CHECK(h && x, "null argument");
    BM_TRY(refuse_nrelu(h, "bm_rbm_allreduce_grads_direct"));
    void *p = nullptr, *st = nullptr; size_t n = 0;
    BM_TRY(bm_rbm_dev_ptr(h, "grad", &p, &n));
    BM_CHECK(p == (void *)x->buf && n == x->count, "the exchange was created for another buffer (gradient slots are not supported)");
    BM_TRY(bm_rbm_stream(h, &st));
    h->xchg_used = x; x->user = &h->xchg_used;
    return bm_xchg_allreduce_sum(x, st);
}
int bm_dbm_allreduce_grads_direct(bm_dbm *h, bm_xchg *x) {
    BM_CHECK(h && x, "null argument");
    void *p = nullptr, *st = nullptr; size_t n = 0;
    BM_TRY(bm_dbm_dev_ptr(h, "grad", &p, &n));
    BM_CHECK(p == (void *)x->buf && n == x->count, "the exchange was created for another buffer");
    BM_TRY(bm_dbm_stream(h, &st));
    h->xchg_used = x; x->user = &h->xchg_used;
    return bm_xchg_allreduce_sum(x, st);
}

}
```

Before: 15870.

## Relax exchange fences, unroll cross-rank loads, and template kernels on fence mode

Templates the multi-GPU exchange kernels on a FENCES flag. By default they use relaxed atomics and s_waitcnt drains in place of system-scope fences and release/acquire orderings. Loops that load from several ranks are unrolled to keep more loads in flight, the local rank is read with device-coherent rather than system-coherent loads, and the bias-update tail batches its loads. This targets synchronization and latency cost in the gradient exchange, but risks memory-ordering bugs across devices. The metric is single-device Gibbs steps/sec, where these exchange paths probably do not run at all.

```diff
diff --git a/boltzmann_machines_amd/csrc/bm_kernels.h b/boltzmann_machines_amd/csrc/bm_kernels.h
--- a/boltzmann_machines_amd/csrc/bm_kernels.h
+++ b/boltzmann_machines_amd/csrc/bm_kernels.h
@@ -1703,6 +1703,7 @@
     int n, layer;
     float N, M, lr, mom, damping, cost, target;
 };
+template <bool PEN_WT = false>
 __device__ __forceinline__ void dbm_bias_apply(const DbmBiasArgs &a, int c, float g) {
     if (a.q) {
         const float qn = a.damping * a.q[c] + (1.0f - a.damping) * a.s_neg[a.layer];
@@ -1712,15 +1713,17 @@
         const float p1 = a.cost * (qn - a.target);
         const float p2 = a.cost * (mn - a.target);
         const float pen = p1 + p2;
-        a.pen[c] = pen;
+        if (PEN_WT) __hip_atomic_store(a.pen + c, pen, __ATOMIC_RELAXED, __HIP_MEMORY_SCOPE_AGENT);
+        else a.pen[c] = pen;
         g = g - pen;
     }
     const float d = a.lr * (a.mom * a.db[c] + g);
     a.db[c] = d;
     a.b[c] = a.b[c] + d;
 }
+template <bool PEN_WT = false>
 __device__ __forceinline__ void dbm_bias_update(const DbmBiasArgs &a, int c) {
-    dbm_bias_apply(a, c, a.s_pos[c] / a.N - a.s_neg[c] / a.M);
+    dbm_bias_apply<PEN_WT>(a, c, a.s_pos[c] / a.N - a.s_neg[c] / a.M);
 }
 BM_KERNEL void dbm_bias_kernel(DbmBiasArgs a) {
     const int c = blockIdx.x * blockDim.x + threadIdx.x;
diff --git a/boltzmann_machines_amd/csrc/bm_xchg.hip b/boltzmann_machines_amd/csrc/bm_xchg.hip
--- a/boltzmann_machines_amd/csrc/bm_xchg.hip
+++ b/boltzmann_machines_amd/csrc/bm_xchg.hip
@@ -46,6 +46,22 @@
     __builtin_amdgcn_raw_buffer_store_b128(__builtin_bit_cast(u32x4, v), r, (int)byte_off, 0, 17);
 }
 
+template <bool DEV>
+__device__ __forceinline__ f32x4 load_dev(__amdgpu_buffer_rsrc_t r, unsigned byte_off) {
+    return __builtin_bit_cast(f32x4, __builtin_amdgcn_raw_buffer_load_b128(r, (int)byte_off, 0, DEV ? 16 : 0));
+}
+__device__ __forceinline__ void drain_stores() { asm volatile("s_waitcnt vmcnt(0)" ::: "memory"); }
+
+template <bool FENCES>
+__device__ __forceinline__ void post_ready(const Args &a) {
+    if (blockIdx.x == 0 && (int)threadIdx.x < a.n) {
+        unsigned *f = a.pflags[threadIdx.x] + F_READY + a.rank;
+        if (FENCES) __hip_atomic_store(f, a.epoch, __ATOMIC_RELEASE, __HIP_MEMORY_SCOPE_SYSTEM);
+        else __hip_atomic_store(f, a.epoch, __ATOMIC_RELAXED, __HIP_MEMORY_SCOPE_SYSTEM);
+    }
+}
+
+template <bool FENCES>
 __device__ __forceinline__ bool wait_all(const Args &a, int base, int code) {
     const int tid = threadIdx.x;
     int bad = 0;
@@ -56,73 +72,145 @@
             if (wall_clock64() - t0 > a.timeout_ticks) { bad = 1; break; }
         }
         if (bad) __hip_atomic_store(a.flags + F_STATUS, (unsigned)(code * 16 + tid + 1), __ATOMIC_RELAXED, __HIP_MEMORY_SCOPE_SYSTEM);
+    } else if (tid == a.n) {
+        if (__hip_atomic_load(a.flags + F_STATUS, __ATOMIC_RELAXED, __HIP_MEMORY_SCOPE_SYSTEM) != 0u) bad = 1;
     }
     bad = __syncthreads_or(bad);
-    if (!bad && __hip_atomic_load(a.flags + F_STATUS, __ATOMIC_RELAXED, __HIP_MEMORY_SCOPE_SYSTEM) != 0u) bad = 1;
-    __atomic_thread_fence(__ATOMIC_ACQUIRE);
+    if (FENCES) __atomic_thread_fence(__ATOMIC_ACQUIRE);
+    else asm volatile("" ::: "memory");
     return !bad;
 }
 
+template <bool FENCES>
+__device__ __forceinline__ void publish_done(const Args &a) {
+    if (FENCES) __threadfence_system();
+    else drain_stores();
+    __syncthreads();
+    if (threadIdx.x == 0) {
+        unsigned old;
+        if (FENCES) old = __hip_atomic_fetch_add(a.ctr, 1u, __ATOMIC_ACQ_REL, __HIP_MEMORY_SCOPE_AGENT);
+        else old = __hip_atomic_fetch_add(a.ctr, 1u, __ATOMIC_RELAXED, __HIP_MEMORY_SCOPE_AGENT);
+        if (old + 1u == (unsigned)a.grid * a.epoch) {
+            if (FENCES) __threadfence_system();
+            for (int r = 0; r < a.n; ++r) {
+                unsigned *f = a.pflags[r] + F_DONE + a.rank;
+                if (FENCES) __hip_atomic_store(f, a.epoch, __ATOMIC_RELEASE, __HIP_MEMORY_SCOPE_SYSTEM);
+                else __hip_atomic_store(f, a.epoch, __ATOMIC_RELAXED, __HIP_MEMORY_SCOPE_SYSTEM);
+            }
+        }
+    }
+}
+
+template <bool FENCES>
+__device__ __forceinline__ void post_tail(unsigned *tail_flag, unsigned epoch) {
+    if (FENCES) __threadfence();
+    else drain_stores();
+    __syncthreads();
+    if (threadIdx.x == 0) {
+        if (FENCES) __hip_atomic_store(tail_flag, epoch, __ATOMIC_RELEASE, __HIP_MEMORY_SCOPE_AGENT);
+        else __hip_atomic_store(tail_flag, epoch, __ATOMIC_RELAXED, __HIP_MEMORY_SCOPE_AGENT);
+    }
+}
+template <bool FENCES>
+__device__ __forceinline__ bool wait_tail(const Args &a, const unsigned *tail_flag) {
+    int bad = 0;
+    if (threadIdx.x == 0) {
+        const long long t0 = wall_clock64();
+        for (;;) {
+            const unsigned f = FENCES ? __hip_atomic_load(tail_flag, __ATOMIC_ACQUIRE, __HIP_MEMORY_SCOPE_AGENT)
+                                      : __hip_atomic_load(tail_flag, __ATOMIC_RELAXED, __HIP_MEMORY_SCOPE_AGENT);
+            if ((int)(f - a.epoch) >= 0) break;
+            __builtin_amdgcn_s_sleep(2);
+            if (wall_clock64() - t0 > a.timeout_ticks) { bad = 1; break; }
+        }
+        if (bad) __hip_atomic_store(a.flags + F_STATUS, (unsigned)(4 * 16 + a.rank + 1), __ATOMIC_RELAXED, __HIP_MEMORY_SCOPE_SYSTEM);
+    }
+    bad = __syncthreads_or(bad);
+    asm volatile("" ::: "memory");
+    return !bad;
+}
+constexpr unsigned OOB = 0xfffffff0u;
+constexpr int UNROLL = 2;
+constexpr int DBM_UNROLL = 2;
+constexpr int TAIL_UNROLL = 4, BIAS_UNROLL = 8;
+__device__ __forceinline__ void store_dev(__amdgpu_buffer_rsrc_t r, unsigned byte_off, f32x4 v) {
+    __builtin_amdgcn_raw_buffer_store_b128(__builtin_bit_cast(u32x4, v), r, (int)byte_off, 0, 0);
+}
+__device__ __forceinline__ void load_ranks(f32x4 (&v)[MAXR], const __amdgpu_buffer_rsrc_t (&rs)[MAXR], unsigned off, int n, int me) {
+#pragma unroll
+    for (int r = 0; r < MAXR; ++r)
+        if (r < n) v[r] = r == me ? load_dev<false>(rs[r], off) : load_sys(rs[r], off);
+}
+__device__ __forceinline__ f32x4 sum_ranks(const f32x4 (&v)[MAXR], int n) {
+    f32x4 s = v[0];
+#pragma unroll
+    for (int r = 1; r < MAXR; ++r) if (r < n) s = s + v[r];
+    return s;
+}
+__device__ __forceinline__ void pull_slice(const float *src, float *dst, unsigned long long len4, unsigned long long st, bool ok) {
+    const __amdgpu_buffer_rsrc_t rq = rsrc(src, len4 * 16), rd = rsrc(dst, len4 * 16);
+    const float qnan = __builtin_nanf("");
+    for (unsigned long long e0 = (unsigned long long)blockIdx.x * NTX + threadIdx.x; e0 < len4; e0 += 4 * st) {
+        unsigned off[4];
+        f32x4 v[4];
+#pragma unroll
+        for (int u = 0; u < 4; ++u) {
+            const unsigned long long e = e0 + u * st;
+            off[u] = e < len4 ? (unsigned)(e * 16) : OOB;
+            v[u] = ok ? load_sys(rq, off[u]) : (f32x4){qnan, qnan, qnan, qnan};
+        }
+#pragma unroll
+        for (int u = 0; u < 4; ++u) store_dev(rd, off[u], v[u]);
+    }
+}
+
+template <bool FENCES>
+__device__ __forceinline__ void store_pen(float *p, float v) {
+    if (FENCES) *p = v;
+    else __hip_atomic_store(p, v, __ATOMIC_RELAXED, __HIP_MEMORY_SCOPE_AGENT);
+}
+
+template <bool FENCES>
 __global__ __launch_bounds__(NTX) void allreduce_kernel(Args a) {
     const int tid = threadIdx.x, me = a.rank, n = a.n;
-    if (blockIdx.x == 0 && tid < n)
-        __hip_atomic_store(a.pflags[tid] + F_READY + me, a.epoch, __ATOMIC_RELEASE, __HIP_MEMORY_SCOPE_SYSTEM);
-    const bool ok1 = wait_all(a, F_READY, 1);
+    post_ready<FENCES>(a);
+    const bool ok1 = wait_all<FENCES>(a, F_READY, 1);
     const float qnan = __builtin_nanf("");
     const unsigned long long base = (unsigned long long)me * a.chunk;
     const unsigned long long len = base < a.count ? (a.count - base < a.chunk ? a.count - base : a.chunk) : 0ull;
     const unsigned long long len4 = (len + 3) / 4;
+    const unsigned long long st = (unsigned long long)a.grid * NTX;
     {
         __amdgpu_buffer_rsrc_t rs[MAXR];
 #pragma unroll
         for (int r = 0; r < MAXR; ++r) rs[r] = rsrc(r < n ? a.pbuf[r] + base : a.buf, r < n ? len4 * 16 : 0);
-        __amdgpu_buffer_rsrc_t rred = rsrc(a.red, len4 * 16);
-        for (unsigned long long e = (unsigned long long)blockIdx.x * NTX + tid; e < len4; e += (unsigned long long)a.grid * NTX) {
-            const unsigned off = (unsigned)(e * 16);
-            f32x4 v[MAXR];
-#pragma unroll
-            for (int r = 0; r < MAXR; ++r) if (r < n) v[r] = load_sys(rs[r], off);
-            f32x4 s = v[0];
-#pragma unroll
-            for (int r = 1; r < MAXR; ++r) if (r < n) s = s + v[r];
-            if (!ok1) s = (f32x4){qnan, qnan, qnan, qnan};
-            *reinterpret_cast<f32x4 *>(a.buf + base + e * 4) = s;
-            store_sys(rred, off, s);
-        }
-    }
-    __threadfence_system();
-    __syncthreads();
-    if (tid == 0) {
-        const unsigned old = __hip_atomic_fetch_add(a.ctr, 1u, __ATOMIC_ACQ_REL, __HIP_MEMORY_SCOPE_AGENT);
-        if (old + 1u == (unsigned)a.grid * a.epoch) {
-            __threadfence_system();
-            for (int r = 0; r < n; ++r)
-                __hip_atomic_store(a.pflags[r] + F_DONE + me, a.epoch, __ATOMIC_RELEASE, __HIP_MEMORY_SCOPE_SYSTEM);
-        }
-    }
+        const __amdgpu_buffer_rsrc_t rown = rsrc(a.buf + base, len4 * 16), rred = rsrc(a.red, len4 * 16);
+        for (unsigned long long e0 = (unsigned long long)blockIdx.x * NTX + tid; e0 < len4; e0 += UNROLL * st) {
+            unsigned off[UNROLL];
+            f32x4 v[UNROLL][MAXR];
+#pragma unroll
+            for (int u = 0; u < UNROLL; ++u) {
+                const unsigned long long e = e0 + u * st;
+                off[u] = e < len4 ? (unsigned)(e * 16) : OOB;
+                load_ranks(v[u], rs, off[u], n, me);
+            }
+#pragma unroll
+            for (int u = 0; u < UNROLL; ++u) {
+                f32x4 s = sum_ranks(v[u], n);
+                if (!ok1) s = (f32x4){qnan, qnan, qnan, qnan};
+                store_dev(rown, off[u], s);
+                if (n > 1) store_sys(rred, off[u], s);
+            }
+        }
+    }
+    publish_done<FENCES>(a);
     if (n == 1) return;
-    const bool ok2 = wait_all(a, F_DONE, 2);
+    const bool ok2 = wait_all<FENCES>(a, F_DONE, 2);
     for (int d = 1; d < n; ++d) {
-        if (!ok2) {
-            const unsigned long long bq = (unsigned long long)((me + d) % n) * a.chunk;
-            const unsigned long long lq = bq < a.count ? (a.count - bq < a.chunk ? a.count - bq : a.chunk) : 0ull;
-            for (unsigned long long e = (unsigned long long)blockIdx.x * NTX + tid; e < (lq + 3) / 4; e += (unsigned long long)a.grid * NTX)
-                *reinterpret_cast<f32x4 *>(a.buf + bq + e * 4) = (f32x4){qnan, qnan, qnan, qnan};
-            continue;
-        }
         const int q = (me + d) % n;
         const unsigned long long bq = (unsigned long long)q * a.chunk;
         const unsigned long long lq = bq < a.count ? (a.count - bq < a.chunk ? a.count - bq : a.chunk) : 0ull;
-        const unsigned long long lq4 = (lq + 3) / 4;
-        __amdgpu_buffer_rsrc_t rq = rsrc(a.pred[q], lq4 * 16);
-        unsigned long long e = (unsigned long long)blockIdx.x * NTX + tid;
-        const unsigned long long st = (unsigned long long)a.grid * NTX;
-        for (; e + st < lq4; e += 2 * st) {
-            const f32x4 v0 = load_sys(rq, (unsigned)(e * 16)), v1 = load_sys(rq, (unsigned)((e + st) * 16));
-            *reinterpret_cast<f32x4 *>(a.buf + bq + e * 4) = v0;
-            *reinterpret_cast<f32x4 *>(a.buf + bq + (e + st) * 4) = v1;
-        }
-        if (e < lq4) *reinterpret_cast<f32x4 *>(a.buf + bq + e * 4) = load_sys(rq, (unsigned)(e * 16));
+        pull_slice(a.pred[q], a.buf + bq, (lq + 3) / 4, st, ok2);
     }
 }
 
@@ -137,15 +225,16 @@
     int dw_only;
 };
 
+template <bool FENCES>
 __global__ __launch_bounds__(NTX) void exchange_apply_kernel(Args a, RbmApply p) {
     const int tid = threadIdx.x, me = a.rank, n = a.n;
     const float qnan = __builtin_nanf("");
-    if (blockIdx.x == 0 && tid < n)
-        __hip_atomic_store(a.pflags[tid] + F_READY + me, a.epoch, __ATOMIC_RELEASE, __HIP_MEMORY_SCOPE_SYSTEM);
-    const bool ok1 = wait_all(a, F_READY, 1);
+    post_ready<FENCES>(a);
+    const bool ok1 = wait_all<FENCES>(a, F_READY, 1);
     const unsigned long long base = (unsigned long long)me * p.chunkW;
     const unsigned long long len = base < p.countW ? (p.countW - base < p.chunkW ? p.countW - base : p.chunkW) : 0ull;
     const unsigned long long len4 = len / 4;
+    const unsigned long long st = (unsigned long long)a.grid * NTX;
     __amdgpu_buffer_rsrc_t rred = rsrc(a.red, len4 * 16);
     if (!p.dw_only) {
         if (blockIdx.x == gridDim.x - 1) {
@@ -153,121 +242,112 @@
             __amdgpu_buffer_rsrc_t rt[MAXR];
 #pragma unroll
             for (int r = 0; r < MAXR; ++r) rt[r] = rsrc(r < n ? a.pbuf[r] + p.countW : a.buf, r < n ? (unsigned long long)T4 * 16 : 0);
-            for (int c4 = tid; c4 < T4; c4 += NTX) {
-                f32x4 v[MAXR];
-#pragma unroll
-                for (int r = 0; r < MAXR; ++r) if (r < n) v[r] = load_sys(rt[r], (unsigned)c4 * 16u);
-                f32x4 s = v[0];
-#pragma unroll
-                for (int r = 1; r < MAXR; ++r) if (r < n) s = s + v[r];
-                if (!ok1) s = (f32x4){qnan, qnan, qnan, qnan};
-                *reinterpret_cast<f32x4 *>(p.tail_red + 4 * c4) = s;
+            for (int c0 = tid; c0 < T4; c0 += TAIL_UNROLL * NTX) {
+                f32x4 v[TAIL_UNROLL][MAXR];
+#pragma unroll
+                for (int u = 0; u < TAIL_UNROLL; ++u) {
+                    const int c4 = c0 + u * NTX;
+                    load_ranks(v[u], rt, c4 < T4 ? (unsigned)c4 * 16u : OOB, n, me);
+                }
+#pragma unroll
+                for (int u = 0; u < TAIL_UNROLL; ++u) {
+                    const int c4 = c0 + u * NTX;
+                    f32x4 s = sum_ranks(v[u], n);
+                    if (!ok1) s = (f32x4){qnan, qnan, qnan, qnan};
+                    if (c4 < T4) *reinterpret_cast<f32x4 *>(p.tail_red + 4 * c4) = s;
+                }
             }
             __syncthreads();
             const float *sv = p.tail_red, *sh = p.tail_red + p.V, *sq = p.tail_red + p.V + p.H;
-            for (int c = tid; c < p.V + p.H; c += NTX) {
-                if (c < p.V) {
-                    const float g = sv[c] / p.N;
-                    const float d = p.lr * (p.mom * p.dvb[c] + g);
-                    p.dvb[c] = d;
-                    p.vb[c] = p.vb[c] + d;
-                } else {
-                    const int h = c - p.V;
-                    const float qn = p.damping * p.q[h] + (1.0f - p.damping) * sq[h];
-                    p.q[h] = qn;
-                    const float pen = p.cost * (qn - p.target);
-                    p.pen[h] = pen;
-                    float g = sh[h] / p.N;
-                    g = g - pen;
-                    const float d = p.lr * (p.mom * p.dhb[h] + g);
-                    p.dhb[h] = d;
-                    p.hb[h] = p.hb[h] + d;
+            for (int c0 = tid; c0 < p.V + p.H; c0 += BIAS_UNROLL * NTX) {
+                float s0[BIAS_UNROLL], s1[BIAS_UNROLL], x0[BIAS_UNROLL], x1[BIAS_UNROLL], x2[BIAS_UNROLL];
+#pragma unroll
+                for (int u = 0; u < BIAS_UNROLL; ++u) {
+                    const int c = c0 + u * NTX, h = c - p.V;
+                    s0[u] = s1[u] = x0[u] = x1[u] = x2[u] = 0.f;
+                    if (c < p.V) { s0[u] = sv[c]; x0[u] = p.dvb[c]; x1[u] = p.vb[c]; }
+                    else if (h < p.H) { s0[u] = sh[h]; s1[u] = sq[h]; x0[u] = p.dhb[h]; x1[u] = p.hb[h]; x2[u] = p.q[h]; }
+                }
+#pragma unroll
+                for (int u = 0; u < BIAS_UNROLL; ++u) {
+                    const int c = c0 + u * NTX, h = c - p.V;
+                    if (c < p.V) {
+                        const float g = s0[u] / p.N;
+                        const float d = p.lr * (p.mom * x0[u] + g);
+                        p.dvb[c] = d;
+                        p.vb[c] = x1[u] + d;
+                    } else if (h < p.H) {
+                        const float qn = p.damping * x2[u] + (1.0f - p.damping) * s1[u];
+                        p.q[h] = qn;
+                        const float pen = p.cost * (qn - p.target);
+                        store_pen<FENCES>(p.pen + h, pen);
+                        float g = s0[u] / p.N;
+                        g = g - pen;
+                        const float d = p.lr * (p.mom * x0[u] + g);
+                        p.dhb[h] = d;
+                        p.hb[h] = x1[u] + d;
+                    }
                 }
             }
-            __threadfence();
-            __syncthreads();
-            if (tid == 0) __hip_atomic_store(p.tail_flag, a.epoch, __ATOMIC_RELEASE, __HIP_MEMORY_SCOPE_AGENT);
+            post_tail<FENCES>(p.tail_flag, a.epoch);
         }
         bool okp = true;
-        if (p.cost != 0.f) {
-            int bad = 0;
-            if (tid == 0) {
-                const long long t0 = wall_clock64();
-                while ((int)(__hip_atomic_load(p.tail_flag, __ATOMIC_ACQUIRE, __HIP_MEMORY_SCOPE_AGENT) - a.epoch) < 0) {
-                    __builtin_amdgcn_s_sleep(2);
-                    if (wall_clock64() - t0 > a.timeout_ticks) { bad = 1; break; }
-                }
-                if (bad) __hip_atomic_store(a.flags + F_STATUS, (unsigned)(4 * 16 + me + 1), __ATOMIC_RELAXED, __HIP_MEMORY_SCOPE_SYSTEM);
-            }
-            okp = !__syncthreads_or(bad);
-        }
+        if (p.cost != 0.f) okp = wait_tail<FENCES>(a, p.tail_flag);
         const bool pow2 = bm::grad_pow2(p.N);
         const float invN = 1.0f / p.N;
+        __amdgpu_buffer_rsrc_t rpen = rsrc(p.pen, (unsigned long long)p.I * 4);
         __amdgpu_buffer_rsrc_t rs[MAXR];
 #pragma unroll
         for (int r = 0; r < MAXR; ++r) rs[r] = rsrc(r < n ? a.pbuf[r] + base : a.buf, r < n ? len4 * 16 : 0);
-        for (unsigned long long e = (unsigned long long)blockIdx.x * NTX + tid; e < len4; e += (unsigned long long)a.grid * NTX) {
-            const unsigned off = (unsigned)(e * 16);
-            f32x4 v[MAXR];
-#pragma unroll
-            for (int r = 0; r < MAXR; ++r) if (r < n) v[r] = load_sys(rs[r], off);
-            f32x4 s = v[0];
-#pragma unroll
-            for (int r = 1; r < MAXR; ++r) if (r < n) s = s + v[r];
-            const unsigned long long flat = base + e * 4;
-            const int i = (int)(flat % (unsigned long long)p.ldw);
-            f32x4 wv = *reinterpret_cast<const f32x4 *>(p.W + flat), dv = *reinterpret_cast<const f32x4 *>(p.dW + flat);
-            if (i < p.I) {
-                f32x4 pe = (f32x4){0.f, 0.f, 0.f, 0.f};
-                if (p.cost != 0.f) pe = *reinterpret_cast<const f32x4 *>(p.pen + i);
-#pragma unroll
-                for (int c = 0; c < 4; ++c) {
-                    const float g = bm::grad_norm1(s[c], p.N, invN, pow2);
-                    float w = wv[c], d = dv[c];
-                    bm::apply_w_update(g, pe[c], p.l2, p.lr, p.mom, w, d);
-                    wv[c] = w; dv[c] = d;
+        const __amdgpu_buffer_rsrc_t rW = rsrc(p.W + base, len4 * 16), rdW = rsrc(p.dW + base, len4 * 16);
+        const unsigned nw = a.grid > 1 ? (unsigned)a.grid - 1u : 1u;
+        const unsigned long long sw = (unsigned long long)nw * NTX;
+        for (unsigned long long e0 = blockIdx.x < nw ? (unsigned long long)blockIdx.x * NTX + tid : len4; e0 < len4; e0 += UNROLL * sw) {
+            unsigned off[UNROLL], offu[UNROLL];
+            f32x4 v[UNROLL][MAXR], wv[UNROLL], dv[UNROLL], pe[UNROLL];
+#pragma unroll
+            for (int u = 0; u < UNROLL; ++u) {
+                const unsigned long long e = e0 + u * sw;
+                off[u] = e < len4 ? (unsigned)(e * 16) : OOB;
+                load_ranks(v[u], rs, off[u], n, me);
+                wv[u] = load_dev<false>(rW, off[u]);
+                dv[u] = load_dev<false>(rdW, off[u]);
+                const int i = (int)((base + e * 4) % (unsigned long long)p.ldw);
+                offu[u] = i < p.I ? off[u] : OOB;
+                pe[u] = (f32x4){0.f, 0.f, 0.f, 0.f};
+                if (p.cost != 0.f) pe[u] = load_dev<!FENCES>(rpen, offu[u] != OOB ? (unsigned)i * 4u : OOB);
+            }
+#pragma unroll
+            for (int u = 0; u < UNROLL; ++u) {
+                const f32x4 s = sum_ranks(v[u], n);
+                if (offu[u] != OOB) {
+#pragma unroll
+                    for (int c = 0; c < 4; ++c) {
+                        const float g = bm::grad_norm1(s[c], p.N, invN, pow2);
+                        float w = wv[u][c], d = dv[u][c];
+                        bm::apply_w_update(g, pe[u][c], p.l2, p.lr, p.mom, w, d);
+                        wv[u][c] = w; dv[u][c] = d;
+                    }
+                    if (!ok1 || !okp) wv[u] = dv[u] = (f32x4){qnan, qnan, qnan, qnan};
                 }
-                if (!ok1 || !okp) wv = dv = (f32x4){qnan, qnan, qnan, qnan};
-                *reinterpret_cast<f32x4 *>(p.W + flat) = wv;
-                *reinterpret_cast<f32x4 *>(p.dW + flat) = dv;
+                store_dev(rW, offu[u], wv[u]);
+                store_dev(rdW, offu[u], dv[u]);
+                if (n > 1) store_sys(rred, off[u], wv[u]);
             }
-            store_sys(rred, off, wv);
         }
     } else {
         for (unsigned long long e = (unsigned long long)blockIdx.x * NTX + tid; e < len4; e += (unsigned long long)a.grid * NTX)
             store_sys(rred, (unsigned)(e * 16), *reinterpret_cast<const f32x4 *>(p.dW + base + e * 4));
     }
-    __threadfence_system();
-    __syncthreads();
-    if (tid == 0) {
-        const unsigned old = __hip_atomic_fetch_add(a.ctr, 1u, __ATOMIC_ACQ_REL, __HIP_MEMORY_SCOPE_AGENT);
-        if (old + 1u == (unsigned)a.grid * a.epoch) {
-            __threadfence_system();
-            for (int r = 0; r < n; ++r)
-                __hip_atomic_store(a.pflags[r] + F_DONE + me, a.epoch, __ATOMIC_RELEASE, __HIP_MEMORY_SCOPE_SYSTEM);
-        }
-    }
+    publish_done<FENCES>(a);
     if (n == 1) return;
-    const bool ok2 = wait_all(a, F_DONE, 2);
+    const bool ok2 = wait_all<FENCES>(a, F_DONE, 2);
     float *dst = p.dw_only ? p.dW : p.W;
     for (int d = 1; d < n; ++d) {
         const int q = (me + d) % n;
         const unsigned long long bq = (unsigned long long)q * p.chunkW;
         const unsigned long long lq = bq < p.countW ? (p.countW - bq < p.chunkW ? p.countW - bq : p.chunkW) : 0ull;
-        const unsigned long long lq4 = lq / 4;
-        __amdgpu_buffer_rsrc_t rq = rsrc(a.pred[q], lq4 * 16);
-        const unsigned long long st = (unsigned long long)a.grid * NTX;
-        unsigned long long e = (unsigned long long)blockIdx.x * NTX + tid;
-        if (!ok2) {
-            for (; e < lq4; e += st) *reinterpret_cast<f32x4 *>(dst + bq + e * 4) = (f32x4){qnan, qnan, qnan, qnan};
-            continue;
-        }
-        for (; e + st < lq4; e += 2 * st) {
-            const f32x4 v0 = load_sys(rq, (unsigned)(e * 16)), v1 = load_sys(rq, (unsigned)((e + st) * 16));
-            *reinterpret_cast<f32x4 *>(dst + bq + e * 4) = v0;
-            *reinterpret_cast<f32x4 *>(dst + bq + (e + st) * 4) = v1;
-        }
-        if (e < lq4) *reinterpret_cast<f32x4 *>(dst + bq + e * 4) = load_sys(rq, (unsigned)(e * 16));
+        pull_slice(a.pred[q], dst + bq, lq / 4, st, ok2);
     }
 }
 
@@ -287,12 +367,12 @@
     float *tail_red; unsigned *tail_flag;
 };
 
+template <bool FENCES>
 __global__ __launch_bounds__(NTX) void dbm_exchange_apply_kernel(Args a, DbmApply p) {
     const int tid = threadIdx.x, me = a.rank, n = a.n;
     const float qnan = __builtin_nanf("");
-    if (blockIdx.x == 0 && tid < n)
-        __hip_atomic_store(a.pflags[tid] + F_READY + me, a.epoch, __ATOMIC_RELEASE, __HIP_MEMORY_SCOPE_SYSTEM);
-    const bool ok1 = wait_all(a, F_READY, 1);
+    post_ready<FENCES>(a);
+    const bool ok1 = wait_all<FENCES>(a, F_READY, 1);
     __amdgpu_buffer_rsrc_t rs[MAXR];
 #pragma unroll
     for (int r = 0; r < MAXR; ++r) rs[r] = rsrc(r < n ? a.pbuf[r] : a.buf, r < n ? ((a.count + 3) & ~3ull) * 4 : 0);
@@ -301,35 +381,19 @@
         for (int c4 = tid; c4 < T4; c4 += NTX) {
             const unsigned off = (unsigned)((p.off_sums + 4ull * c4) * 4);
             f32x4 v[MAXR];
-#pragma unroll
-            for (int r = 0; r < MAXR; ++r) if (r < n) v[r] = load_sys(rs[r], off);
-            f32x4 s = v[0];
-#pragma unroll
-            for (int r = 1; r < MAXR; ++r) if (r < n) s = s + v[r];
+            load_ranks(v, rs, off, n, me);
+            f32x4 s = sum_ranks(v, n);
             if (!ok1) s = (f32x4){qnan, qnan, qnan, qnan};
             *reinterpret_cast<f32x4 *>(p.tail_red + 4 * c4) = s;
         }
         __syncthreads();
         for (int v = 0; v <= p.L; ++v)
-            for (int c = tid; c < p.bias[v].n; c += NTX) bm::dbm_bias_update(p.bias[v], c);
-        __threadfence();
-        __syncthreads();
-        if (tid == 0) __hip_atomic_store(p.tail_flag, a.epoch, __ATOMIC_RELEASE, __HIP_MEMORY_SCOPE_AGENT);
-    }
-    bool okp = true;
-    {
-        int bad = 0;
-        if (tid == 0) {
-            const long long t0 = wall_clock64();
-            while ((int)(__hip_atomic_load(p.tail_flag, __ATOMIC_ACQUIRE, __HIP_MEMORY_SCOPE_AGENT) - a.epoch) < 0) {
-                __builtin_amdgcn_s_sleep(2);
-                if (wall_clock64() - t0 > a.timeout_ticks) { bad = 1; break; }
-            }
-            if (bad) __hip_atomic_store(a.flags + F_STATUS, (unsigned)(4 * 16 + me + 1), __ATOMIC_RELAXED, __HIP_MEMORY_SCOPE_SYSTEM);
-        }
-        okp = !__syncthreads_or(bad);
-    }
+            for (int c = tid; c < p.bias[v].n; c += NTX) bm::dbm_bias_update<!FENCES>(p.bias[v], c);
+        post_tail<FENCES>(p.tail_flag, a.epoch);
+    }
+    const bool okp = wait_tail<FENCES>(a, p.tail_flag);
     const bool pow2 = bm::grad_pow2(p.N) && bm::grad_pow2(p.M);
+    const unsigned long long st = (unsigned long long)a.grid * NTX;
     const float invN = 1.0f / p.N, invM = 1.0f / p.M;
     for (int i = 0; i < p.L; ++i) {
         const DbmLayerX &y = p.lay[i];
@@ -337,40 +401,51 @@
         if (c1 <= c0) continue;
         const unsigned w4 = (unsigned)(c1 - c0) / 4u;
         const unsigned long long n4 = (unsigned long long)y.J * w4;
-        for (unsigned long long e = (unsigned long long)blockIdx.x * NTX + tid; e < n4; e += (unsigned long long)a.grid * NTX) {
-            const int j = (int)(e / w4), c = c0 + 4 * (int)(e % w4);
-            const unsigned long long o = (unsigned long long)j * y.ldw + c;
-            const unsigned bp = (unsigned)((y.off_pos + o) * 4), bn = (unsigned)((y.off_neg + o) * 4);
-            f32x4 vp[MAXR], vn[MAXR];
-#pragma unroll
-            for (int r = 0; r < MAXR; ++r) if (r < n) { vp[r] = load_sys(rs[r], bp); vn[r] = load_sys(rs[r], bn); }
-            f32x4 sp = vp[0], sn = vn[0];
-#pragma unroll
-            for (int r = 1; r < MAXR; ++r) if (r < n) { sp = sp + vp[r]; sn = sn + vn[r]; }
-            f32x4 wv = *reinterpret_cast<const f32x4 *>(y.W + o), dv = *reinterpret_cast<const f32x4 *>(y.dW + o);
-            const f32x4 pe = *reinterpret_cast<const f32x4 *>(y.pen + c);
-#pragma unroll
-            for (int q = 0; q < 4; ++q) {
-                const float g = bm::grad_norm2(sp[q], sn[q], p.N, p.M, invN, invM, pow2);
-                float w = wv[q], d = dv[q];
-                bm::apply_w_update(g, pe[q], p.l2, p.lr, p.mom, w, d);
-                wv[q] = w; dv[q] = d;
+        __amdgpu_buffer_rsrc_t rpen = rsrc(y.pen, (unsigned long long)y.I * 4);
+        const unsigned long long wbytes = (unsigned long long)y.J * y.ldw * 4;
+        const __amdgpu_buffer_rsrc_t rW = rsrc(y.W, wbytes), rdW = rsrc(y.dW, wbytes);
+        for (unsigned long long e0 = (unsigned long long)blockIdx.x * NTX + tid; e0 < n4; e0 += DBM_UNROLL * st) {
+            unsigned ow[DBM_UNROLL];
+            f32x4 vp[DBM_UNROLL][MAXR], vn[DBM_UNROLL][MAXR], wv[DBM_UNROLL], dv[DBM_UNROLL], pe[DBM_UNROLL];
+#pragma unroll
+            for (int u = 0; u < DBM_UNROLL; ++u) {
+                const unsigned long long e = e0 + u * st;
+                const bool in = e < n4;
+                const int j = (int)(e / w4), c = c0 + 4 * (int)(e % w4);
+                const unsigned long long o = (unsigned long long)j * y.ldw + c;
+                ow[u] = in ? (unsigned)(o * 4) : OOB;
+                load_ranks(vp[u], rs, in ? (unsigned)((y.off_pos + o) * 4) : OOB, n, me);
+                load_ranks(vn[u], rs, in ? (unsigned)((y.off_neg + o) * 4) : OOB, n, me);
+                wv[u] = load_dev<false>(rW, ow[u]);
+                dv[u] = load_dev<false>(rdW, ow[u]);
+                pe[u] = load_dev<!FENCES>(rpen, in ? (unsigned)c * 4u : OOB);
             }
-            if (!ok1 || !okp) wv = dv = (f32x4){qnan, qnan, qnan, qnan};
-            *reinterpret_cast<f32x4 *>(y.W + o) = wv;
-            *reinterpret_cast<f32x4 *>(y.dW + o) = dv;
-        }
-    }
-}
-
+#pragma unroll
+            for (int u = 0; u < DBM_UNROLL; ++u) {
+                const f32x4 sp = sum_ranks(vp[u], n), sn = sum_ranks(vn[u], n);
+#pragma unroll
+                for (int q = 0; q < 4; ++q) {
+                    const float g = bm::grad_norm2(sp[q], sn[q], p.N, p.M, invN, invM, pow2);
+                    float w = wv[u][q], d = dv[u][q];
+                    bm::apply_w_update(g, pe[u][q], p.l2, p.lr, p.mom, w, d);
+                    wv[u][q] = w; dv[u][q] = d;
+                }
+                if (!ok1 || !okp) wv[u] = dv[u] = (f32x4){qnan, qnan, qnan, qnan};
+                store_dev(rW, ow[u], wv[u]);
+                store_dev(rdW, ow[u], dv[u]);
+            }
+        }
+    }
+}
+
+template <bool FENCES>
 __global__ __launch_bounds__(NTX) void dbm_exchange_gather_kernel(Args a, DbmApply p) {
     __shared__ float t[32][33];
     const int tid = threadIdx.x, me = a.rank, n = a.n;
     const float qnan = __builtin_nanf("");
     if (p.do_ready) {
-        if (blockIdx.x == 0 && tid < n)
-            __hip_atomic_store(a.pflags[tid] + F_READY + me, a.epoch, __ATOMIC_RELEASE, __HIP_MEMORY_SCOPE_SYSTEM);
-        (void)wait_all(a, F_READY, 1);
+        post_ready<FENCES>(a);
+        (void)wait_all<FENCES>(a, F_READY, 1);
     }
     __amdgpu_buffer_rsrc_t rred = rsrc(a.red, a.red_cap * 4);
     for (int i = 0; i < p.L; ++i) {
@@ -390,18 +465,9 @@
                 store_sys(rred, (unsigned)((y.red_off + (unsigned long long)y.J * y.sw + 4 * e) * 4),
                           *reinterpret_cast<const f32x4 *>(y.wnorm + c0 + 4 * e));
     }
-    __threadfence_system();
-    __syncthreads();
-    if (tid == 0) {
-        const unsigned old = __hip_atomic_fetch_add(a.ctr, 1u, __ATOMIC_ACQ_REL, __HIP_MEMORY_SCOPE_AGENT);
-        if (old + 1u == (unsigned)a.grid * a.epoch) {
-            __threadfence_system();
-            for (int r = 0; r < n; ++r)
-                __hip_atomic_store(a.pflags[r] + F_DONE + me, a.epoch, __ATOMIC_RELEASE, __HIP_MEMORY_SCOPE_SYSTEM);
-        }
-    }
+    publish_done<FENCES>(a);
     if (n == 1) return;
-    const bool ok2 = wait_all(a, F_DONE, 2);
+    const bool ok2 = wait_all<FENCES>(a, F_DONE, 2);
     for (int i = 0; i < p.L; ++i) {
         const DbmLayerX &y = p.lay[i];
         float *dst = p.mode ? y.dW : y.W;
@@ -411,14 +477,25 @@
             if (q1 <= q0) continue;
             __amdgpu_buffer_rsrc_t rq = rsrc(a.pred[q], a.red_cap * 4);
             const int tiles_c = (q1 - q0 + 31) / 32, tiles_j = (y.J + 31) / 32;
-            for (int tile = blockIdx.x; tile < tiles_c * tiles_j; tile += a.grid) {
+            const int r = tid >> 3, c4 = tid & 7;
+            for (int tile0 = blockIdx.x; tile0 < tiles_c * tiles_j; tile0 += 4 * a.grid) {
+              f32x4 vt[4];
+#pragma unroll
+              for (int u = 0; u < 4; ++u) {
+                  const int tile = tile0 + u * a.grid;
+                  const int j = (tile / tiles_c) * 32 + r, cb = (tile % tiles_c) * 32;
+                  const bool in = tile < tiles_c * tiles_j && j < y.J && q0 + cb + 4 * c4 < q1;
+                  vt[u] = load_sys(rq, in && ok2 ? (unsigned)((y.red_off + (unsigned long long)j * y.sw + cb + 4 * c4) * 4) : OOB);
+              }
+#pragma unroll
+              for (int u = 0; u < 4; ++u) {
+                const int tile = tile0 + u * a.grid;
+                if (tile >= tiles_c * tiles_j) break;
                 const int cb = (tile % tiles_c) * 32, j0 = (tile / tiles_c) * 32;
-                const int r = tid >> 3, c4 = tid & 7;
                 const int j = j0 + r, c = q0 + cb + 4 * c4;
                 f32x4 v = (f32x4){0.f, 0.f, 0.f, 0.f};
                 if (j < y.J && c < q1) {
-                    v = ok2 ? load_sys(rq, (unsigned)((y.red_off + (unsigned long long)j * y.sw + cb + 4 * c4) * 4))
-                            : (f32x4){qnan, qnan, qnan, qnan};
+                    v = ok2 ? vt[u] : (f32x4){qnan, qnan, qnan, qnan};
                     *reinterpret_cast<f32x4 *>(dst + (unsigned long long)j * y.ldw + c) = v;
                 }
                 if (!p.mode) {
@@ -432,6 +509,7 @@
                     }
                     __syncthreads();
                 }
+              }
             }
             if (!p.mode && blockIdx.x == 0)
                 for (int e = tid; e < (q1 - q0) / 4; e += NTX)
@@ -450,10 +528,9 @@
     unsigned epoch;
     long long timeout_ticks;
 };
-__global__ __launch_bounds__(64) void max1_kernel(MaxArgs a) {
+__device__ __forceinline__ float exchange_max1(const MaxArgs &a, float mine) {
     const int tid = threadIdx.x;
     const unsigned par = a.epoch & 1u;
-    const float mine = *a.val;
     float got = 0.f;
     if (tid < a.n) {
         const unsigned long long word = ((unsigned long long)a.epoch << 32) | (unsigned long long)__float_as_uint(mine);
@@ -470,7 +547,11 @@
     }
 #pragma unroll
     for (int off = 32; off > 0; off >>= 1) got = fmaxf(got, __shfl_xor(got, off));
-    if (tid == 0) *a.val = got;
+    return got;
+}
+__global__ __launch_bounds__(64) void max1_kernel(MaxArgs a) {
+    const float got = exchange_max1(a, *a.val);
+    if (threadIdx.x == 0) *a.val = got;
 }
 
 __global__ __launch_bounds__(256) void mf_ctl_max1_kernel(MaxArgs a, bm::MfCtl *c, float *blk, int nblk, float tol, int init) {
@@ -489,24 +570,7 @@
     }
     __syncthreads();
     if (tid >= 64) return;
-    const unsigned par = a.epoch & 1u;
-    const float mine = s_resid;
-    float got = 0.f;
-    if (tid < a.n) {
-        const unsigned long long word = ((unsigned long long)a.epoch << 32) | (unsigned long long)__float_as_uint(mine);
-        __hip_atomic_store(a.pslots[tid] + par * MAXR + a.rank, word, __ATOMIC_RELAXED, __HIP_MEMORY_SCOPE_SYSTEM);
-        const long long t0 = wall_clock64();
-        unsigned long long w;
-        bool ok = true;
-        while ((unsigned)((w = __hip_atomic_load(a.slots + par * MAXR + tid, __ATOMIC_RELAXED, __HIP_MEMORY_SCOPE_SYSTEM)) >> 32) != a.epoch) {
-            __builtin_amdgcn_s_sleep(2);
-            if (wall_clock64() - t0 > a.timeout_ticks) { ok = false; break; }
-        }
-        if (ok) got = __uint_as_float((unsigned)w);
-        else __hip_atomic_store(a.flags + F_STATUS, (unsigned)(3 * 16 + tid + 1), __ATOMIC_RELAXED, __HIP_MEMORY_SCOPE_SYSTEM);
-    }
-#pragma unroll
-    for (int off = 32; off > 0; off >>= 1) got = fmaxf(got, __shfl_xor(got, off));
+    const float got = exchange_max1(a, s_resid);
     if (tid != 0) return;
     c->resid = got;
     if (init) {
@@ -518,6 +582,28 @@
     }
 }
 
+}
+
+static bool xchg_fences() {
+    static const bool on = bm::dbg("xchg_fences") && atoi(bm::dbg("xchg_fences")) != 0;
+    return on;
+}
+#define BMX_LAUNCH(kern, grid, stream, ...)                                                                        \
+    do {                                                                                                           \
+        if (xchg_fences()) hipLaunchKernelGGL((bmx::kern<true>), dim3(grid), dim3(bmx::NTX), 0, stream, __VA_ARGS__);  \
+        else hipLaunchKernelGGL((bmx::kern<false>), dim3(grid), dim3(bmx::NTX), 0, stream, __VA_ARGS__);               \
+    } while (0)
+
+template <bool FENCES>
+static int xchg_min_occupancy() {
+    int m = 1 << 30, k = 0;
+    const void *kern[4] = {(const void *)bmx::allreduce_kernel<FENCES>, (const void *)bmx::exchange_apply_kernel<FENCES>,
+                           (const void *)bmx::dbm_exchange_apply_kernel<FENCES>, (const void *)bmx::dbm_exchange_gather_kernel<FENCES>};
+    for (const void *f : kern) {
+        if (hipOccupancyMaxActiveBlocksPerMultiprocessor(&k, f, bmx::NTX, 0) != hipSuccess) { (void)hipGetLastError(); return 0; }
+        if (k < m) m = k;
+    }
+    return m;
 }
 
 struct bm_xchg {
@@ -600,7 +686,7 @@
     {
         hipDeviceProp_t pr;
         if (hipGetDeviceProperties(&pr, x->device) == hipSuccess) ncu = pr.multiProcessorCount;
-        if (hipOccupancyMaxActiveBlocksPerMultiprocessor(&per_cu, bmx::dbm_exchange_gather_kernel, bmx::NTX, 0) != hipSuccess) { (void)hipGetLastError(); per_cu = 0; }
+        per_cu = xchg_fences() ? xchg_min_occupancy<true>() : xchg_min_occupancy<false>();
     }
     if (ncu < 1 || per_cu < 1) { bm::set_error("bm_xchg_create: cannot establish a co-resident launch width (CUs %d, workgroups per CU %d)", ncu, per_cu); return fail(); }
     const size_t f4 = (x->chunk / 4 + bmx::NTX - 1) / bmx::NTX;
@@ -682,7 +768,7 @@
     a.rank = x->rank; a.n = x->nranks; a.epoch = ++x->epoch;
     for (int r = 0; r < bmx::MAXR; ++r) { a.pbuf[r] = x->pbuf[r]; a.pred[r] = x->pred[r]; a.pflags[r] = x->pflags[r]; }
     a.flags = x->flags; a.ctr = x->ctr; a.grid = x->grid; a.timeout_ticks = x->timeout_ticks;
-    hipLaunchKernelGGL(bmx::allreduce_kernel, dim3(x->grid), dim3(bmx::NTX), 0, (hipStream_t)stream, a);
+    BMX_LAUNCH(allreduce_kernel, x->grid, (hipStream_t)stream, a);
     BM_HIP(hipGetLastError());
     return 0;
 }
@@ -765,7 +851,7 @@
     q.damping = h->cfg.sparsity_damping; q.cost = h->cfg.sparsity_cost; q.target = h->cfg.sparsity_target;
     q.vb = h->vb.p; q.dvb = h->dvb.p; q.hb = h->hb.p; q.dhb = h->dhb.p; q.q = h->q.p; q.pen = h->pen.p;
     q.tail_red = x->tail_red; q.tail_flag = x->tail_flag; q.dw_only = dw_only;
-    hipLaunchKernelGGL(bmx::exchange_apply_kernel, dim3(x->grid), dim3(bmx::NTX), 0, h->stream, a, q);
+    BMX_LAUNCH(exchange_apply_kernel, x->grid, h->stream, a, q);
     BM_HIP(hipGetLastError());
     h->xchg_used = x; x->user = &h->xchg_used;
     return 0;
@@ -882,13 +968,13 @@
             c.damping = h->cfg.sparsity_damping; c.cost = h->cfg.sparsity_cost[i]; c.target = h->cfg.sparsity_target[i];
         }
     }
-    hipLaunchKernelGGL(bmx::dbm_exchange_apply_kernel, dim3(x->grid), dim3(bmx::NTX), 0, h->stream, a, q);
+    BMX_LAUNCH(dbm_exchange_apply_kernel, x->grid, h->stream, a, q);
     for (int i = 0; i < h->L; ++i) {
         const int c0 = x->rank * q.lay[i].sw;
         const int c1 = c0 + q.lay[i].sw < q.lay[i].I ? c0 + q.lay[i].sw : q.lay[i].I;
         launch_dbm_maxnorm(h, i, c0, c1 > c0 ? c1 : c0);
     }
-    hipLaunchKernelGGL(bmx::dbm_exchange_gather_kernel, dim3(x->grid), dim3(bmx::NTX), 0, h->stream, a, q);
+    BMX_LAUNCH(dbm_exchange_gather_kernel, x->grid, h->stream, a, q);
     BM_HIP(hipGetLastError());
     h->xchg_used = x; x->user = &h->xchg_used;
     x->dw_stale = x->nranks > 1;
@@ -904,7 +990,7 @@
     bmx::Args a; bmx::DbmApply q;
     BM_TRY(dbm_fill_exchange(h, x, a, q, true));
     q.mode = 1; q.do_ready = 1;
-    hipLaunchKernelGGL(bmx::dbm_exchange_gather_kernel, dim3(x->grid), dim3(bmx::NTX), 0, h->stream, a, q);
+    BMX_LAUNCH(dbm_exchange_gather_kernel, x->grid, h->stream, a, q);
     BM_HIP(hipGetLastError());
     h->xchg_used = x; x->user = &h->xchg_used;
     x->dw_stale = false;
@@ -921,7 +1007,7 @@
     a.rank = x->rank; a.n = x->nranks; a.epoch = ++x->epoch;
     for (int r = 0; r < bmx::MAXR; ++r) { a.pbuf[r] = x->pbuf[r]; a.pred[r] = x->pred[r]; a.pflags[r] = x->pflags[r]; }
     a.flags = x->flags; a.ctr = x->ctr; a.grid = x->grid; a.timeout_ticks = x->timeout_ticks;
-    hipLaunchKernelGGL(bmx::allreduce_kernel, dim3(x->grid), dim3(bmx::NTX), 0, stream, a);
+    BMX_LAUNCH(allreduce_kernel, x->grid, stream, a);
     BM_HIP(hipGetLastError());
     return 0;
 }
```

Result: slower. 15670 (-1.3%).
